# ofsouzap/DistributedMandelbrot

Hardware: AMD Instinct MI355X
Metric: G pixel-iterations/s on 4096^2 tile, max_iter=1000 fp64 (higher is better)
Workload: dtype f64

## Files before the change

distributedmandelbrot_amd/_lib.py:

```python
from __future__ import annotations

import ctypes as C
import importlib.util
import os
import sys

HERE = os.path.dirname(os.path.abspath(__file__))
SO_PATH = os.path.join(HERE, "libmbk_hip.so")

MBK_OK, MBK_ERR_INVALID, MBK_ERR_NO_DEVICE, MBK_ERR_HIP, MBK_ERR_NOMEM, MBK_ERR_NET = range(6)
MBK_WANT_COUNTS = 0x1
MBK_WANT_BYTES = 0x2
MBK_KERNEL_DEFAULT = 0x000
MBK_KERNEL_SIMPLE = 0x100
MBK_KERNEL_ASM = 0x200
MBK_KERNEL_REFILL = 0x300
MBK_KERNEL_GROUP = 0x400
MBK_KERNEL_SCAN = 0x500
KERNELS = {"default": MBK_KERNEL_DEFAULT, "simple": MBK_KERNEL_SIMPLE, "asm": MBK_KERNEL_ASM,
           "refill": MBK_KERNEL_REFILL, "group": MBK_KERNEL_GROUP, "scan": MBK_KERNEL_SCAN}
OPTIONS = {name: i for i, name in enumerate(
    ["order", "waves_per_wg", "group_steps", "exact_steps", "probe_steps", "scan_waves", "scan_xcd_map", "scan_col_period", "heavy_share",
     "rf_livemin", "rf_patience", "rf_batch", "rf_waves", "cycle_detect", "probe_mid", "prepass_overlap", "exact_long", "scan_inline", "wave_limit", "units_min_light", "xcd_balance", "m_late", "h_settled", "classify_wg", "scan_strip", "cycle_window", "spill_first", "spill_lanes", "spill_min_mrd", "spill_min_blocks", "spill_cyc_shift"])}
MBK_PRECISION_F32 = 0x1000
MBK_LAZY_UNIFORM = 0x2000
MBK_DEEP_BLA = 0x8000
MBK_DEEP_XBLA = 0x10000
PRECISIONS = {"f64": 0, "f32": MBK_PRECISION_F32}
MBK_SLOTS = 4
MBK_WORKER_DEPTH = 3
MBK_INFO_SCAN_WG_PER_CU = 100
MBK_INFO_XCD_SHARE = 110
MBK_INFO_SPILL = 130
MBK_CODEC_RAW = 0x00
MBK_CODEC_RLE = 0x01
MBK_CHUNK_DEFINITION = 4096
MBK_CHUNK_BYTES = 4096 * 4096
MBK_ABI_VERSION = 5
MBK_RENDER_BYTES = 0
MBK_RENDER_SMOOTH = 1
MBK_RENDER_DISTANCE = 3
MBK_RENDER_DISTANCE_REL = 4
MBK_RENDER_EQUALIZED = 5
RENDER_SOURCES = {"bytes": MBK_RENDER_BYTES, "smooth": MBK_RENDER_SMOOTH, "distance": MBK_RENDER_DISTANCE,
                  "distance_rel": MBK_RENDER_DISTANCE_REL, "equalized": MBK_RENDER_EQUALIZED}
MBK_HISTOGRAM_MAX_MRD = 1 << 20
RENDER_SUPERSAMPLES = (1, 2, 3, 4, 8)
MBK_RENDER_BAND_BYTES = 256 << 20
MBK_STREAM_OK, MBK_STREAM_BAD_CODEC, MBK_STREAM_BAD_SIZE, MBK_STREAM_ZERO_RUN, MBK_STREAM_TOO_LONG, MBK_STREAM_TOO_SHORT = range(6)
STREAM_REASONS = {MBK_STREAM_OK: "MBK_STREAM_OK", MBK_STREAM_BAD_CODEC: "MBK_STREAM_BAD_CODEC", MBK_STREAM_BAD_SIZE: "MBK_STREAM_BAD_SIZE",
                  MBK_STREAM_ZERO_RUN: "MBK_STREAM_ZERO_RUN", MBK_STREAM_TOO_LONG: "MBK_STREAM_TOO_LONG",
                  MBK_STREAM_TOO_SHORT: "MBK_STREAM_TOO_SHORT"}
CHUNK_SCALES = (1, 2, 4, 8, 16, 32, 64)
MBK_DENSITY_MAX_CELLS = 1 << 28
MBK_DENSITY_LINEAR = 0
MBK_DENSITY_SQRT = 1
DENSITY_MODES = {"linear": MBK_DENSITY_LINEAR, "sqrt": MBK_DENSITY_SQRT}
DENSITY_FACTORS = (1, 2, 4, 8)


class mbk_view(C.Structure):
    _fields_ = [("start_r", C.c_double), ("start_i", C.c_double),
                ("range_r", C.c_double), ("range_i", C.c_double),
                ("width", C.c_uint32), ("height", C.c_uint32),
                ("col0", C.c_uint32), ("row0", C.c_uint32),
                ("ncols", C.c_uint32), ("nrows", C.c_uint32)]


class mbk_deep_view(C.Structure):
    _fields_ = [("range_r", C.c_double), ("range_i", C.c_double),
                ("width", C.c_uint32), ("height", C.c_uint32),
                ("col0", C.c_uint32), ("row0", C.c_uint32),
                ("ncols", C.c_uint32), ("nrows", C.c_uint32)]


class mbk_deep_xview(C.Structure):
    _fields_ = [("range_r", C.c_double), ("range_i", C.c_double), ("exp2", C.c_int32),
                ("width", C.c_uint32), ("height", C.c_uint32),
                ("col0", C.c_uint32), ("row0", C.c_uint32),
                ("ncols", C.c_uint32), ("nrows", C.c_uint32)]


class mbk_render_spec(C.Structure):
    _fields_ = [("source", C.c_uint32), ("supersample", C.c_uint32), ("palette", C.c_void_p),
                ("palette_len", C.c_uint32), ("inside", C.c_uint8 * 4),
                ("scale", C.c_double), ("offset", C.c_double), ("max_band_rows", C.c_uint32)]


class mbk_chunk_spec(C.Structure):
    _fields_ = [("palette", C.c_void_p), ("scale", C.c_uint32)]


class mbk_interior_render_spec(C.Structure):
    _fields_ = [("supersample", C.c_uint32), ("palette", C.c_void_p), ("palette_len", C.c_uint32),
                ("unknown", C.c_uint8 * 4), ("outside", C.c_uint8 * 4), ("scale", C.c_double), ("max_band_rows", C.c_uint32)]


class mbk_density_target(C.Structure):
    _fields_ = [("start_r", C.c_double), ("start_i", C.c_double), ("range_r", C.c_double), ("range_i", C.c_double),
                ("width", C.c_uint32), ("height", C.c_uint32)]


class mbk_density_stats(C.Structure):
    _fields_ = [("deposits", C.c_uint64), ("dropped", C.c_uint64)]


class mbk_density_render_spec(C.Structure):
    _fields_ = [("mode", C.c_uint32), ("factor", C.c_uint32), ("palette", C.c_void_p), ("palette_len", C.c_uint32),
                ("scale", C.c_double), ("offset", C.c_double)]


class mbk_stats(C.Structure):
    _fields_ = [("kernel_ms", C.c_float), ("d2h_ms", C.c_float),
                ("pixel_iterations", C.c_uint64), ("never_pixels", C.c_uint64),
                ("all_bytes_zero", C.c_uint32), ("all_bytes_one", C.c_uint32),
                ("rle_runs", C.c_uint64)]


class mbk_device_info(C.Structure):
    _fields_ = [("name", C.c_char * 128), ("arch", C.c_char * 64),
                ("compute_units", C.c_int), ("clock_mhz", C.c_int),
                ("wavefront_size", C.c_int), ("total_mem", C.c_uint64)]


class mbk_worker_report(C.Structure):
    _fields_ = [("leased", C.c_uint64), ("accepted", C.c_uint64), ("rejected", C.c_uint64), ("resets", C.c_uint64),
                ("uniform_tiles", C.c_uint64), ("pixel_iterations", C.c_uint64),
                ("kernel_ms_sum", C.c_double), ("seconds", C.c_double), ("net_retries", C.c_uint64)]


NET_OPTIONS = {name: i for i, name in enumerate(
    ["max_connections", "connect_timeout_ms", "io_timeout_ms", "retries", "backoff_ms", "stop", "peak_connections", "feeder_slots"])}


FEEDER_SUBMIT = C.CFUNCTYPE(C.c_int, C.c_void_p, C.c_int, C.c_uint32, C.c_uint32, C.c_uint32, C.c_uint32, C.c_void_p)
FEEDER_WAIT = C.CFUNCTYPE(C.c_int, C.c_void_p, C.c_int, C.POINTER(mbk_stats))
FEEDER_ALLOC = C.CFUNCTYPE(C.c_void_p, C.c_void_p, C.c_uint64)
FEEDER_RELEASE = C.CFUNCTYPE(None, C.c_void_p, C.c_void_p)
FEEDER_ON_TILE = C.CFUNCTYPE(None, C.c_void_p, C.POINTER(C.c_uint32 * 4), C.POINTER(mbk_stats), C.c_int)


class mbk_feeder_ops(C.Structure):
    _fields_ = [("user", C.c_void_p), ("submit", FEEDER_SUBMIT), ("wait", FEEDER_WAIT), ("alloc", FEEDER_ALLOC),
                ("release", FEEDER_RELEASE), ("on_tile", FEEDER_ON_TILE)]


SIGNATURES = {
    "mbk_abi_version": (C.c_int, []),
    "mbk_device_count": (C.c_int, [C.POINTER(C.c_int)]),
    "mbk_create": (C.c_int, [C.c_int, C.POINTER(C.c_void_p)]),
    "mbk_destroy": (None, [C.c_void_p]),
    "mbk_last_error": (C.c_char_p, [C.c_void_p]),
    "mbk_get_device_info": (C.c_int, [C.c_void_p, C.POINTER(mbk_device_info)]),
    "mbk_device_pci_bus_id": (C.c_int, [C.c_void_p, C.c_char_p, C.c_int]),
    "mbk_host_alloc": (C.c_int, [C.c_void_p, C.c_uint64, C.POINTER(C.c_void_p)]),
    "mbk_host_free": (C.c_int, [C.c_void_p, C.c_void_p]),
    "mbk_datachunk_geometry": (C.c_int, [C.c_uint32, C.c_uint32, C.c_uint32,
                                         C.POINTER(C.c_double), C.POINTER(C.c_double),
                                         C.POINTER(C.c_double)]),
    "mbk_view_outside_circle": (C.c_int, [C.POINTER(mbk_view), C.c_uint32, C.POINTER(C.c_int)]),
    "mbk_view_needs_literal_doubling": (C.c_int, [C.POINTER(mbk_view), C.c_uint32, C.POINTER(C.c_int)]),
    "mbk_view_launch": (C.c_int, [C.c_void_p, C.POINTER(mbk_view), C.c_uint32, C.c_uint32,
                                  C.c_void_p, C.c_void_p, C.c_void_p]),
    "mbk_view_compute": (C.c_int, [C.c_void_p, C.POINTER(mbk_view), C.c_uint32, C.c_uint32,
                                   C.c_void_p, C.c_void_p, C.POINTER(mbk_stats)]),
    "mbk_datachunk": (C.c_int, [C.c_void_p, C.c_uint32, C.c_uint32, C.c_uint32, C.c_uint32,
                                C.c_void_p, C.c_void_p, C.POINTER(mbk_stats)]),
    "mbk_view_launch_smooth": (C.c_int, [C.c_void_p, C.POINTER(mbk_view), C.c_uint32, C.c_uint32,
                                         C.c_void_p, C.c_void_p, C.c_void_p]),
    "mbk_view_compute_smooth": (C.c_int, [C.c_void_p, C.POINTER(mbk_view), C.c_uint32, C.c_uint32,
                                          C.c_void_p, C.c_void_p, C.POINTER(mbk_stats)]),
    "mbk_view_launch_distance": (C.c_int, [C.c_void_p, C.POINTER(mbk_view), C.c_uint32, C.c_uint32,
                                           C.c_void_p, C.c_void_p, C.c_void_p]),
    "mbk_view_compute_distance": (C.c_int, [C.c_void_p, C.POINTER(mbk_view), C.c_uint32, C.c_uint32,
                                            C.c_void_p, C.c_void_p, C.POINTER(mbk_stats)]),
    "mbk_distance_value_host": (C.c_double, [C.c_double, C.c_double, C.c_int32]),
    "mbk_datachunk_submit": (C.c_int, [C.c_void_p, C.c_int, C.c_uint32, C.c_uint32, C.c_uint32, C.c_uint32,
                                       C.c_void_p, C.c_void_p]),
    "mbk_datachunk_submit_ex": (C.c_int, [C.c_void_p, C.c_int, C.c_uint32, C.c_uint32, C.c_uint32, C.c_uint32,
                                          C.c_void_p, C.c_void_p, C.c_uint32]),
    "mbk_view_submit": (C.c_int, [C.c_void_p, C.c_int, C.POINTER(mbk_view), C.c_uint32, C.c_uint32,
                                  C.c_void_p, C.c_void_p]),
    "mbk_wait": (C.c_int, [C.c_void_p, C.c_int, C.POINTER(mbk_stats)]),
    "mbk_serialize_last": (C.c_int, [C.c_void_p, C.c_void_p, C.c_uint64, C.POINTER(C.c_uint64),
                                     C.POINTER(C.c_uint32)]),
    "mbk_set_option": (C.c_int, [C.c_void_p, C.c_int, C.c_uint32]),
# ... 226 lines not shown
```

distributedmandelbrot_amd/csrc/mbk_api.hip:

```cpp
#include "../../include/mbk.h"

#include <hip/hip_runtime.h>

#include <cmath>
#include <cstdio>
#include <cstdlib>
#include <algorithm>
#include <cstring>
#include <new>
#include <string>
#include <vector>

#include "mbk_kernels.h"
#include "mbk_refill.h"
#include "mbk_persist.h"
#include "mbk_scan.h"
#include "mbk_units.h"
#include "mbk_spill.h"
#include "mbk_feeder.h"
#include "mbk_deep_orbit.h"
#include "mbk_deep.h"
#include "mbk_deep_bla.h"
#include "mbk_deep_wide.h"
#include "mbk_deep_wide_bla.h"
#include "mbk_histogram.h"
#include "mbk_render.h"
#include "mbk_chunks.h"
#include "mbk_distance.h"
#include "mbk_interior.h"
#include "mbk_deep_distance.h"
#include "mbk_deep_distance_bla.h"
#include "mbk_deep_wide_distance.h"
#include "mbk_julia.h"
#include "mbk_density.h"

using mbk::Axis;
using mbk::ReduceOut;
using mbk::ReduceSlot;
using mbk::TileArgs;
using mbk::WorkQueues;

static const int kOrderRing = 3;

struct OrderRing {
    uint32_t *d_order[kOrderRing] = {};
    uint32_t *d_ctl = nullptr;
    bool ctl_dirty = true;
    size_t order_cap = 0;
    unsigned order_turn = 0;
    hipStream_t aux = nullptr;
    uint32_t aux_prio = 0;
    int pp_last = -1;
    hipEvent_t ev_cls[kOrderRing] = {};
    hipEvent_t ev_done[kOrderRing] = {};
    bool done_valid[kOrderRing] = {};

    void drop_lists()
    {
        for (int k = 0; k < kOrderRing; ++k) {
            if (d_order[k]) (void)hipFree(d_order[k]);
            d_order[k] = nullptr;
            done_valid[k] = false;
        }
        order_cap = 0;
    }
    void drop_aux()
    {
        if (aux) (void)hipStreamDestroy(aux);
        aux = nullptr;
        for (int k = 0; k < kOrderRing; ++k) {
            if (ev_cls[k]) (void)hipEventDestroy(ev_cls[k]);
            if (ev_done[k]) (void)hipEventDestroy(ev_done[k]);
            ev_cls[k] = ev_done[k] = nullptr;
            done_valid[k] = false;
        }
    }
    void release()
    {
        if (aux) (void)hipStreamSynchronize(aux);
        drop_lists();
        drop_aux();
        if (d_ctl) (void)hipFree(d_ctl);
        *this = OrderRing();
    }
};

struct SpillBuffers {
    void *d_z = nullptr;
    uint32_t *d_meta = nullptr, *d_cnt = nullptr, *d_chunks = nullptr, *d_src = nullptr;
    unsigned long long *d_total = nullptr;
    size_t cap_slots = 0, cap_blocks = 0;

    void release()
    {
        for (void *q : {d_z, (void *)d_meta, (void *)d_cnt, (void *)d_chunks, (void *)d_src, (void *)d_total})
            if (q) (void)hipFree(q);
        *this = SpillBuffers();
    }
};

struct StreamScratch {
    hipStream_t stream = nullptr;
    OrderRing ring;
    WorkQueues *d_queues = nullptr;
    mbk::ScanCursors *d_cursors = nullptr;
    uint32_t *d_entries = nullptr;
    size_t scan_cap_blocks = 0;
    unsigned scan_turn = 0;
    bool cursors_dirty = false;
    uint32_t *h_hint = nullptr;
    SpillBuffers spill;
    ReduceSlot *d_red = nullptr;
    ReduceSlot *h_red = nullptr;
    unsigned long long *h_stamps = nullptr;
    double xcd_f[8] = {0.125, 0.125, 0.125, 0.125, 0.125, 0.125, 0.125, 0.125};
    uint32_t xcd_issued = 0, xcd_consumed = 0;
    struct SharesUsed { uint32_t seq, switches; float f[8]; } xcd_ring[64] = {};
    void *d_render = nullptr;
    size_t render_cap = 0;
    uint32_t *d_palette = nullptr;
    std::vector<uint32_t> palette;
    uint8_t *d_chunk = nullptr;
    size_t chunk_cap_n = 0;
    uint8_t *d_chunk_bytes = nullptr;
    uint32_t *h_chunk_status = nullptr;
    int32_t *d_dist_counts = nullptr;
    size_t dist_cap_px = 0;
    double *d_lut = nullptr;
    size_t lut_cap = 0;
    std::vector<double> lut;
    uint32_t *d_density_bands = nullptr;
    mbk::DensityMax *d_density_max = nullptr;
};
static const size_t kMaxStreamScratch = 64;
static const uint32_t kStampSlots = 16, kShareRing = 64;

struct Slot {
    hipStream_t stream = nullptr;
    hipEvent_t ev_k0 = nullptr, ev_k1 = nullptr, ev_c0 = nullptr, ev_c1 = nullptr;
    int32_t *d_counts = nullptr;
    uint8_t *d_bytes = nullptr;
    size_t cap_px = 0;
    ReduceSlot *d_red = nullptr;
    ReduceSlot *h_red = nullptr;
    bool busy = false;
    bool with_bytes = false;
    uint8_t *lazy_h_bytes = nullptr;
    size_t lazy_px = 0;
    bool immediate = false;
    mbk_stats imm = {};
};

struct mbk_ctx {
    int device = -1;
    Slot s[MBK_SLOTS];
    std::vector<StreamScratch> scratch;
    size_t last_px = 0;
    double *d_smooth = nullptr;
    size_t smooth_cap_px = 0;
    uint32_t *d_rgba = nullptr;
    size_t rgba_cap_px = 0;
    unsigned long long *d_hist = nullptr;
    size_t hist_cap = 0;
    uint32_t *d_density = nullptr;
    size_t density_cap = 0;
    unsigned long long *d_density_stat = nullptr;
    uint8_t *d_rle = nullptr;
    size_t rle_cap_px = 0;
    uint32_t opt[MBK_OPT_COUNT_];
    hipStream_t last_tile_stream = nullptr;
    uint32_t stream_switches = 0;
    int scan_occ[2][2] = {{0, 0}, {0, 0}};
    int scan_occ_inline[2] = {0, 0};
    uint32_t wave_limit_lds[8] = {0, 0, 0, 0, 0, 0, 0, 0};
    uint32_t spill_launches = 0;
    hipStream_t last_spill_stream = nullptr;
    struct ProbeKey { Axis re, im; uint32_t col0, row0, ncols, nrows; } probe_key = {};
    double probe_share = 0.0;
    bool probe_valid = false;
    struct DeepCopy {
        uint64_t id;
        double4 *d;
        mbk::WideEntry *d_wide;
        bool has_bla;
        uint64_t dcmax_bits;
        double *d_rc;
        double4 *d_ab;
        uint32_t levels;
        uint32_t off[mbk::kBlaMaxLevels];
        bool has_xbla;
        uint64_t xdcmax_bits;
        int32_t xdcmax_exp;
        int32_t *d_xke;
        mbk::WideBlaEntry *d_xab;
        uint32_t xlevels;
        uint32_t xoff[mbk::kBlaMaxLevels];
    };
    std::vector<DeepCopy> deep;
    hipDeviceProp_t prop;
    std::string err;
};

struct mbk_deep_orbit {
    mbk::DeepOrbit o;
};

static thread_local std::string g_err;

static int fail(mbk_ctx *ctx, int code, const std::string &msg)
{
    if (ctx) ctx->err = msg;
    g_err = msg;
    return code;
}

#define MBK_HIP(ctx, call)                                                                  \
    do {                                                                                    \
        hipError_t e_ = (call);                                                             \
        if (e_ != hipSuccess) {                                                             \
            return fail((ctx), MBK_ERR_HIP,                                                 \
                        std::string(#call) + ": " + hipGetErrorString(e_));                 \
        }                                                                                   \
    } while (0)


static Axis make_axis(double start, double range, uint32_t n)
{
    Axis a;
    std::memset(&a, 0, sizeof(a));
    a.start = start;
    a.n = n;
    volatile double stop = start + range;
    if (n <= 1) {
        a.last = start;
        a.div = 1.0;
        return a;
    }
    volatile double delta = stop - start;
    volatile double div = (double)(n - 1);
    volatile double step = delta / div;
    a.last = stop;
    a.delta = delta;
    a.div = div;
    a.step = step;
    a.step_is_zero = (step == 0.0) ? 1u : 0u;
    return a;
}

static double axis_value_host(const Axis &a, uint32_t k)
{
    if (k + 1u == a.n) return a.last;
    volatile double y;
    if (a.step_is_zero) {
        volatile double q = (double)k / a.div;
        y = q * a.delta;
    } else {
        y = (double)k * a.step;
    }
    volatile double v = y + a.start;
    return v;
}

static bool axis_end_is_regular(const Axis &a)
{
    if (a.n <= 1 || a.step_is_zero) return false;
    volatile double y = (double)(a.n - 1u) * a.step;
    volatile double v = y + a.start;
    return v == a.last;
}

static const double kMaxCoord = 0x1p500;
static const double kSafeImagMin = 0x1p-900;

static uint32_t coprime_multiplier(uint32_t n)
{
    if (n < 4) return 1u;
    uint64_t m = (uint64_t)((double)n * 0.6180339887498949);
    if (m < 1) m = 1;
    for (;; ++m) {
        uint64_t a = m, b = n;
        while (b) {
            const uint64_t t = a % b;
            a = b;
            b = t;
        }
        if (a == 1) return (uint32_t)(m % n);
    }
}

static bool axis_has_tiny_nonzero(const Axis &a, uint32_t k0, uint32_t cnt, bool f32)
{
    const double thr = f32 ? 0x1p-100 : kSafeImagMin;
    auto value = [&](uint32_t k) { const double y = axis_value_host(a, k); return f32 ? (double)(float)y : y; };
    auto tiny = [&](double y) { return y != 0.0 && std::fabs(y) < thr; };
    if (cnt == 0) return false;
    uint32_t end = k0 + cnt;
    if (a.n >= 1u && end == a.n) {
        if (tiny(value(a.n - 1u))) return true;
        if (--end == k0) return false;
    }
    const double first = value(k0), last = value(end - 1u);
    if (tiny(first) || tiny(last)) return true;
    if ((first > 0.0 && last > 0.0) || (first < 0.0 && last < 0.0) || first == last) return false;
    const double s = last > first ? 1.0 : -1.0;
    auto lower = [&](bool strict) {
        uint32_t lo = k0, hi = end;
        while (lo < hi) {
            const uint32_t mid = lo + (hi - lo) / 2u;
            const double y = s * value(mid);
            if (strict ? y > 0.0 : y >= 0.0) hi = mid;
            else lo = mid + 1u;
        }
        return lo;
    };
    const uint32_t ge = lower(false), gt = lower(true);
    if (ge > k0 && tiny(value(ge - 1u))) return true;
    if (gt < end && tiny(value(gt))) return true;
    return false;
}

static int validate_view(mbk_ctx *ctx, const mbk_view *v, bool *safe_doubling, bool f32 = false)
{
    if (!v) return fail(ctx, MBK_ERR_INVALID, "view is NULL");
    if (v->width == 0 || v->height == 0) return fail(ctx, MBK_ERR_INVALID, "empty view");
    if (v->ncols == 0 || v->nrows == 0) return fail(ctx, MBK_ERR_INVALID, "empty window");
    if ((uint64_t)v->col0 + v->ncols > v->width || (uint64_t)v->row0 + v->nrows > v->height)
        return fail(ctx, MBK_ERR_INVALID, "window exceeds the view");
    if ((uint64_t)v->ncols * v->nrows > (1ull << 31))
        return fail(ctx, MBK_ERR_INVALID, "window larger than 2^31 pixels");
    const double vals[6] = {v->start_r, v->start_i, v->range_r, v->range_i,
                            v->start_r + v->range_r, v->start_i + v->range_i};
    const double max_coord = f32 ? 0x1p60 : kMaxCoord;
    for (double x : vals)
        if (!std::isfinite(x) || std::fabs(x) > max_coord)
            return fail(ctx, MBK_ERR_INVALID, f32 ? "view coordinates must be finite and |x| <= 2^60 (fp32)"
                                                  : "view coordinates must be finite and |x| <= 2^500");
    *safe_doubling = axis_has_tiny_nonzero(make_axis(v->start_i, v->range_i, v->height), v->row0, v->nrows, f32);
    return MBK_OK;
}

static void free_deep_copy(mbk_ctx::DeepCopy &c)
{
    if (c.d) (void)hipFree(c.d);
    if (c.d_rc) (void)hipFree(c.d_rc);
    if (c.d_ab) (void)hipFree(c.d_ab);
    if (c.d_wide) (void)hipFree(c.d_wide);
    if (c.d_xke) (void)hipFree(c.d_xke);
    if (c.d_xab) (void)hipFree(c.d_xab);
    c = mbk_ctx::DeepCopy();
}

static void free_scratch(StreamScratch &sc)
{
    sc.ring.release();
    sc.spill.release();
    if (sc.d_queues) (void)hipFree(sc.d_queues);
    if (sc.d_cursors) (void)hipFree(sc.d_cursors);
    if (sc.d_entries) (void)hipFree(sc.d_entries);
    if (sc.h_hint) (void)hipHostFree(sc.h_hint);
    if (sc.h_stamps) (void)hipHostFree(sc.h_stamps);
    if (sc.d_red) (void)hipFree(sc.d_red);
    if (sc.h_red) (void)hipHostFree(sc.h_red);
    if (sc.d_render) (void)hipFree(sc.d_render);
    if (sc.d_palette) (void)hipFree(sc.d_palette);
    if (sc.d_chunk) (void)hipFree(sc.d_chunk);
    if (sc.d_chunk_bytes) (void)hipFree(sc.d_chunk_bytes);
    if (sc.h_chunk_status) (void)hipHostFree(sc.h_chunk_status);
    if (sc.d_dist_counts) (void)hipFree(sc.d_dist_counts);
    if (sc.d_lut) (void)hipFree(sc.d_lut);
    if (sc.d_density_bands) (void)hipFree(sc.d_density_bands);
    if (sc.d_density_max) (void)hipFree(sc.d_density_max);
    sc = StreamScratch();
}

static int get_scratch(mbk_ctx *ctx, hipStream_t stream, StreamScratch **out)
{
    for (StreamScratch &sc : ctx->scratch)
        if (sc.stream == stream) {
            *out = &sc;
            return MBK_OK;
        }
    if (ctx->scratch.size() >= kMaxStreamScratch) {
        MBK_HIP(ctx, hipDeviceSynchronize());
        for (StreamScratch &sc : ctx->scratch) free_scratch(sc);
        ctx->scratch.clear();
    }
    ctx->scratch.emplace_back();
    StreamScratch &sc = ctx->scratch.back();
    sc.stream = stream;
    *out = &sc;
    MBK_HIP(ctx, hipHostMalloc((void **)&sc.h_hint, 2 * sizeof(uint32_t), hipHostMallocDefault));
    sc.h_hint[0] = sc.h_hint[1] = 0xffffffffu;
    return MBK_OK;
}

static void set_window_facts(TileArgs &a, bool f32);
static void shares_from_fractions(const double *f, uint32_t *cum);
static double window_heavy_share(const TileArgs &a);
static double window_heavy_share(mbk_ctx *ctx, const TileArgs &a);

static void xcd_shares_update(const mbk_ctx *ctx, StreamScratch &sc)
{
    const unsigned long long kMask = 0xffffffffffffull;
    uint32_t first = sc.xcd_issued >= kStampSlots ? sc.xcd_issued - kStampSlots + 1u : 1u;
    first = std::max(first, sc.xcd_consumed + 1u);
    for (uint32_t c = first; c <= sc.xcd_issued; ++c) {
        const volatile unsigned long long *st = sc.h_stamps + (size_t)(c % kStampSlots) * mbk::kStampWords;
        const StreamScratch::SharesUsed &used = sc.xcd_ring[c % kShareRing];
        if (used.seq != c) continue;
        const StreamScratch::SharesUsed &before = sc.xcd_ring[(c - 1u) % kShareRing], &after = sc.xcd_ring[(c + 1u) % kShareRing];
        const bool alone = c > 1u && before.seq == c - 1u && before.switches == used.switches &&
                           (c == sc.xcd_issued ? ctx->stream_switches == used.switches : after.seq == c + 1u && after.switches == used.switches);
        unsigned long long v[mbk::kStampWords];
        bool whole = true;
        for (uint32_t i = 0; i < mbk::kStampWords; ++i) {
            v[i] = st[i];
            whole = whole && (v[i] >> 48) == (c & 0xffffu);
        }
        if (!whole) continue;
        unsigned long long start = v[0] & kMask;
        for (uint32_t x = 1; x < 8u; ++x)
            if ((((v[x] & kMask) - start) & kMask) >> 47) start = v[x] & kMask;
        double T[8], tmin = 1e300, tmax = 0.0, speed[8], sum = 0.0;
        for (uint32_t x = 0; x < 8u; ++x) {
            unsigned long long last = 0;
            for (uint32_t t = 0; t < mbk::kStampTail; ++t)
                last = std::max(last, ((v[8u + x * mbk::kStampTail + t] & kMask) - start) & kMask);
            T[x] = (double)last;
            tmin = std::min(tmin, T[x]);
            tmax = std::max(tmax, T[x]);
        }
        sc.xcd_consumed = c;
        if (!alone || tmin < 1000.0 || tmax > 1.25 * tmin) continue;
        for (uint32_t x = 0; x < 8u; ++x) {
            speed[x] = (double)used.f[x] / T[x];
            sum += speed[x];
        }
        double fs = 0.0;
        for (uint32_t x = 0; x < 8u; ++x) {
            const double f = 0.7 * sc.xcd_f[x] + 0.3 * speed[x] / sum;
            sc.xcd_f[x] = std::min(0.14, std::max(0.11, f));
            fs += sc.xcd_f[x];
        }
        for (uint32_t x = 0; x < 8u; ++x) sc.xcd_f[x] /= fs;
    }
}

struct FuseStats { ReduceSlot *slots; bool counts_unwanted; bool fused; };

static uint32_t quant_table4(int32_t mrd, bool want_bytes)
{
    uint32_t qtab = 0u;
    if (want_bytes && mrd > 0)
        for (uint32_t c = 1; c <= 4u; ++c)
            qtab |= (uint32_t)(((uint64_t)c * 256u + (uint32_t)mrd - 1u) / (uint32_t)mrd & 0xffu) << (8u * (c - 1u));
    return qtab;
}

struct BlockLaunchPlan {
    uint32_t wpw, by;
    dim3 grid, block;
    uint32_t order_mode, probe_steps;
    bool cyc, units, ordered;
    double unit_share;
};

static BlockLaunchPlan block_launch_plan(mbk_ctx *ctx, TileArgs &a, uint32_t kernel, bool safe, bool f32)
{
    BlockLaunchPlan p;
    p.wpw = ctx->opt[MBK_OPT_WAVES_PER_WG];
    a.blocks_x = (a.ncols + 8u * p.wpw - 1u) / (8u * p.wpw);
    p.by = (a.nrows + 7u) / 8u;
    set_window_facts(a, f32);
    p.cyc = ctx->opt[MBK_OPT_CYCLE_DETECT] != 0u;
    p.grid = dim3(a.blocks_x * p.by);
    p.block = dim3(64u * p.wpw);
    p.order_mode = ctx->opt[MBK_OPT_ORDER];
    p.probe_steps = ctx->opt[MBK_OPT_PROBE_STEPS];
    a.perm_mul = p.order_mode == 1 ? coprime_multiplier(p.grid.x) : 1u;
    a.order = nullptr;
    p.units = p.order_mode == 3 && p.wpw == 1u && kernel == MBK_KERNEL_GROUP && !safe && a.smooth == nullptr &&
              (a.counts || a.bytes) && !(a.bytes && a.quant_wide) && a.blocks_x % 8u == 0u && a.blocks_x <= 2048u &&
              a.fast_bx_end > 0u && a.fast_by_end > 0u && (f32 || ctx->opt[MBK_OPT_GROUP_STEPS] == 16u) &&
              p.grid.x >= 16384u && (uint32_t)a.mrd > 2u * p.probe_steps && p.by <= 0xffffu;
    p.unit_share = 0.0;
    if (p.units) {
        p.unit_share = window_heavy_share(ctx, a);
        p.units = (1.0 - p.unit_share) * 65536.0 >= (double)ctx->opt[MBK_OPT_UNITS_MIN_LIGHT];
    }
    p.ordered = p.order_mode >= 2 && p.grid.x >= 16384u && (uint32_t)a.mrd > 2u * p.probe_steps && a.blocks_x <= 0xffffu && p.by <= 0xffffu;
    return p;
}

struct OrderList {
    StreamScratch *sc = nullptr;
    unsigned k = 0;
    uint32_t *list = nullptr;
    hipStream_t pre = nullptr;
    bool overlap = false;
    bool whole = false;
    ~OrderList() { if (sc && !whole) sc->ring.ctl_dirty = true; }
};

static int acquire_order_list(mbk_ctx *ctx, hipStream_t stream, uint32_t nblocks, OrderList *out)
{
    StreamScratch *sc = nullptr;
    int rc = get_scratch(ctx, stream, &sc);
    if (rc != MBK_OK) return rc;
    OrderRing &ring = sc->ring;
    const uint32_t pp_mode = ctx->opt[MBK_OPT_PREPASS_OVERLAP];
    const bool overlap = pp_mode != 0u;
    const uint32_t want_prio = pp_mode == 2u ? 2u : 1u;
    if (ring.pp_last != (int)pp_mode) {
        if (ring.pp_last >= 0) {
            MBK_HIP(ctx, hipStreamSynchronize(stream));
            if (ring.aux) MBK_HIP(ctx, hipStreamSynchronize(ring.aux));
        }
        for (int k = 0; k < kOrderRing; ++k) ring.done_valid[k] = false;
        ring.pp_last = (int)pp_mode;
    }
    if (overlap && ring.aux && ring.aux_prio != want_prio) {
        MBK_HIP(ctx, hipStreamSynchronize(stream));
        MBK_HIP(ctx, hipStreamSynchronize(ring.aux));
        ring.drop_aux();
    }
    if (overlap && !ring.aux) {
        if (want_prio == 2u) {
            int least = 0, greatest = 0;
            MBK_HIP(ctx, hipDeviceGetStreamPriorityRange(&least, &greatest));
            MBK_HIP(ctx, hipStreamCreateWithPriority(&ring.aux, hipStreamNonBlocking, greatest));
        } else {
            MBK_HIP(ctx, hipStreamCreateWithFlags(&ring.aux, hipStreamNonBlocking));
        }
        ring.aux_prio = want_prio;
        for (int k = 0; k < kOrderRing; ++k) {
            MBK_HIP(ctx, hipEventCreateWithFlags(&ring.ev_cls[k], hipEventDisableTiming));
            MBK_HIP(ctx, hipEventCreateWithFlags(&ring.ev_done[k], hipEventDisableTiming));
        }
    }
    if (nblocks > ring.order_cap) {
        MBK_HIP(ctx, hipStreamSynchronize(stream));
        if (ring.aux) MBK_HIP(ctx, hipStreamSynchronize(ring.aux));
        ring.drop_lists();
        for (int k = 0; k < kOrderRing; ++k)
            MBK_HIP(ctx, hipMalloc((void **)&ring.d_order[k], mbk::units_list_words(nblocks) * sizeof(uint32_t)));
        ring.order_cap = nblocks;
    }
    const unsigned k = ring.order_turn++ % (unsigned)kOrderRing;
    if (overlap && ring.done_valid[k]) MBK_HIP(ctx, hipStreamWaitEvent(ring.aux, ring.ev_done[k], 0));
    out->k = k;
    out->list = ring.d_order[k];
    out->pre = overlap ? ring.aux : stream;
    out->overlap = overlap;
    out->sc = sc;
    return MBK_OK;
}

static int enqueue_units_prepass(mbk_ctx *ctx, TileArgs &a, const BlockLaunchPlan &p, const OrderList &ol, hipStream_t stream)
{
    StreamScratch *sc = ol.sc;
    OrderRing &ring = sc->ring;
    const uint32_t hs = p.cyc ? ctx->opt[MBK_OPT_H_SETTLED] : 0u;
    const double settle_thr = hs ? std::pow(10.0, -(double)hs) : 0.0;
    if (!ring.d_ctl) {
        MBK_HIP(ctx, hipMalloc((void **)&ring.d_ctl, (size_t)kOrderRing * 8u * sizeof(uint32_t)));
        ring.ctl_dirty = true;
    }
    if (ring.ctl_dirty) {
        if (ring.aux) MBK_HIP(ctx, hipStreamSynchronize(ring.aux));
        MBK_HIP(ctx, hipStreamSynchronize(stream));
        MBK_HIP(ctx, hipMemsetAsync(ring.d_ctl, 0, (size_t)kOrderRing * 8u * sizeof(uint32_t), ol.pre));
        ring.ctl_dirty = false;
    }
    uint32_t *ctl = ring.d_ctl + 8u * ol.k;
    const uint32_t balance = ctx->opt[MBK_OPT_XCD_BALANCE] == 1u && (p.cyc || ctx->prop.multiProcessorCount != 256)
                                 ? 0u : ctx->opt[MBK_OPT_XCD_BALANCE];
    static const double kUneven[8] = {0.110, 0.140, 0.125, 0.120, 0.130, 0.125, 0.115, 0.135};
    if (balance == 1u && !sc->h_stamps) {
        MBK_HIP(ctx, hipHostMalloc((void **)&sc->h_stamps, (size_t)kStampSlots * mbk::kStampWords * sizeof(unsigned long long),
                                   hipHostMallocDefault));
        std::memset(sc->h_stamps, 0xff, (size_t)kStampSlots * mbk::kStampWords * sizeof(unsigned long long));
    }
    if (balance == 1u) xcd_shares_update(ctx, *sc);
    mbk::XcdShares w;
    double f[8];
    const uint32_t seq = ++sc->xcd_issued;
    StreamScratch::SharesUsed &used = sc->xcd_ring[seq % kShareRing];
    used.seq = seq;
    used.switches = ctx->stream_switches;
    for (uint32_t x = 0; x < 8u; ++x) {
        f[x] = balance == 1u ? sc->xcd_f[x] : (balance == 2u ? kUneven[x] : 0.125);
        used.f[x] = (float)f[x];
    }
    shares_from_fractions(f, w.cum);
    a.plan = ol.list + ((2u * (size_t)p.grid.x + 5u + 15u) & ~(size_t)15u);
    a.stamps = balance == 1u ? sc->h_stamps + (size_t)(seq % kStampSlots) * mbk::kStampWords : nullptr;
    a.stamp_tag = seq & 0xffffu;
    const uint32_t cwg = ctx->opt[MBK_OPT_CLASSIFY_WG];
    hipLaunchKernelGGL(mbk::classify_units_kernel, dim3((p.grid.x + cwg - 1u) / cwg), dim3(cwg), 0, ol.pre, a, p.grid.x,
                       (int32_t)p.probe_steps, ol.list, ctl, (int32_t)ctx->opt[MBK_OPT_M_LATE], settle_thr, ctl + 3, (uint32_t *)a.plan, w,
                       a.stamps ? 1u : 0u);
    return MBK_OK;
}

static int enqueue_classify_prepass(mbk_ctx *ctx, const TileArgs &a, const BlockLaunchPlan &p, const OrderList &ol, bool *mid_first)
{
    const uint32_t nblocks = p.grid.x;
    uint32_t *cursors = ol.list + nblocks;
    MBK_HIP(ctx, hipMemsetAsync(cursors, 0, 3 * sizeof(uint32_t), ol.pre));
    *mid_first = p.order_mode == 3 && ctx->opt[MBK_OPT_PROBE_MID] > p.probe_steps && ctx->opt[MBK_OPT_M_LATE] >= 2u &&
                 ctx->opt[MBK_OPT_M_LATE] <= p.probe_steps;
    hipLaunchKernelGGL(mbk::classify_blocks_kernel, dim3((nblocks + 1023u) / 1024u), dim3(1024), 0, ol.pre, a,
                       nblocks, 8u * p.wpw, (int32_t)p.probe_steps, (int32_t)(*mid_first ? ctx->opt[MBK_OPT_M_LATE] : ctx->opt[MBK_OPT_PROBE_MID]),
                       ol.list, cursors);
    return MBK_OK;
}

static bool spill_wanted(const mbk_ctx *ctx, const TileArgs &a, const BlockLaunchPlan &p, uint32_t kernel, bool safe, bool f32)
{
    const uint32_t spill_first = ctx->opt[MBK_OPT_SPILL_FIRST], spill_lanes = ctx->opt[MBK_OPT_SPILL_LANES];
    return !p.units && a.order != nullptr && p.order_mode >= 2u && kernel == MBK_KERNEL_GROUP && !safe && a.smooth == nullptr && p.wpw == 1u &&
           (a.counts || a.bytes) && spill_first != 0u && (f32 || ctx->opt[MBK_OPT_GROUP_STEPS] == 16u) &&
           (uint32_t)a.mrd >= ctx->opt[MBK_OPT_SPILL_MIN_MRD] && (uint32_t)a.mrd < (1u << 26) &&
           ((uint64_t)p.grid.x >> ctx->opt[MBK_OPT_SPILL_MIN_BLOCKS]) != 0ull &&
           (uint64_t)a.mrd > (uint64_t)ctx->opt[MBK_OPT_EXACT_STEPS] + spill_first + 66u &&
           (uint64_t)p.grid.x * spill_lanes < (1ull << 32) && a.fast_bx_end > 0u && a.fast_by_end > 0u;
}

static int acquire_spill(mbk_ctx *ctx, StreamScratch *sc, hipStream_t stream, TileArgs &a, uint32_t nblocks, SpillBuffers **out)
{
    SpillBuffers &sp = sc->spill;
    const uint32_t spill_lanes = ctx->opt[MBK_OPT_SPILL_LANES];
    const size_t slots = (size_t)nblocks * spill_lanes, nchunks = (nblocks + mbk::kSpillChunk - 1u) / mbk::kSpillChunk;
    *out = nullptr;
    if (slots > sp.cap_slots || nblocks > sp.cap_blocks) {
        MBK_HIP(ctx, hipStreamSynchronize(stream));
        sp.release();
        const bool got = hipMalloc(&sp.d_z, slots * 16u) == hipSuccess &&
                         hipMalloc((void **)&sp.d_meta, slots * sizeof(uint32_t)) == hipSuccess &&
                         hipMalloc((void **)&sp.d_src, slots * sizeof(uint32_t)) == hipSuccess &&
                         hipMalloc((void **)&sp.d_cnt, (size_t)nblocks * sizeof(uint32_t)) == hipSuccess &&
                         hipMalloc((void **)&sp.d_chunks, (nchunks * mbk::kSpillLevels + 1u) * sizeof(uint32_t)) == hipSuccess &&
                         hipMalloc((void **)&sp.d_total, sizeof(unsigned long long)) == hipSuccess;
        if (got) {
            sp.cap_slots = slots;
            sp.cap_blocks = nblocks;
        } else {
            (void)hipGetLastError();
            sp.release();
        }
    }
    if (sp.cap_slots >= slots && sp.cap_blocks >= nblocks && sp.d_z) {
        a.spill_first = ctx->opt[MBK_OPT_SPILL_FIRST];
        a.spill_lanes = spill_lanes;
        a.spill_win_shift = ctx->opt[MBK_OPT_SPILL_CYC_SHIFT];
        a.spill_z = sp.d_z;
        a.spill_meta = sp.d_meta;
        a.spill_cnt = sp.d_cnt;
        MBK_HIP(ctx, hipMemsetAsync(sp.d_cnt, 0, (size_t)nblocks * sizeof(uint32_t), stream));
        *out = &sp;
    }
    return MBK_OK;
}

typedef void (*UnitsKernel)(TileArgs, uint32_t);
typedef void (*BlockKernel)(TileArgs);
typedef void (*SpillKernel)(TileArgs, const uint32_t *, const unsigned long long *, uint32_t);

static UnitsKernel pick_units_kernel(bool f32, bool cyc, bool stats, bool counts, bool bytes)
{
    static const UnitsKernel forms[4][4] = {
        {mbk::tile_units_kernel<float, 8, true, false, true, true>, mbk::tile_units_kernel<float, 8, true, true, true>,
         mbk::tile_units_kernel<float, 8, true, false, true>, mbk::tile_units_kernel<float, 8, true, true, false>},
        {mbk::tile_units_kernel<float, 8, false, false, true, true>, mbk::tile_units_kernel<float, 8, false, true, true>,
         mbk::tile_units_kernel<float, 8, false, false, true>, mbk::tile_units_kernel<float, 8, false, true, false>},
        {mbk::tile_units_kernel<double, 16, true, false, true, true>, mbk::tile_units_kernel<double, 16, true, true, true>,
         mbk::tile_units_kernel<double, 16, true, false, true>, mbk::tile_units_kernel<double, 16, true, true, false>},
        {mbk::tile_units_kernel<double, 16, false, false, true, true>, mbk::tile_units_kernel<double, 16, false, true, true>,
         mbk::tile_units_kernel<double, 16, false, false, true>, mbk::tile_units_kernel<double, 16, false, true, false>},
    };
    return forms[(f32 ? 0 : 2) + (cyc ? 0 : 1)][stats ? 0 : (counts && bytes) ? 1 : bytes ? 2 : 3];
}

static BlockKernel pick_block_kernel(uint32_t kernel, bool safe, bool f32, bool cyc, uint32_t group_steps, bool spill)
{
    if (spill && f32 && cyc) return mbk::tile_asm_kernel<float, true, 8, true, true>;
    if (spill && f32) return mbk::tile_asm_kernel<float, true, 8, false, true>;
    if (spill && cyc) return mbk::tile_asm_kernel<double, true, 16, true, true>;
    if (spill) return mbk::tile_asm_kernel<double, true, 16, false, true>;
    if (f32 && safe) return mbk::tile_asm_kernel<float, false, 0>;
    if (f32 && kernel == MBK_KERNEL_ASM) return mbk::tile_asm_kernel<float, true, 0>;
    if (f32 && cyc) return mbk::tile_asm_kernel<float, true, 8, true>;
    if (f32) return mbk::tile_asm_kernel<float, true, 8>;
    if (safe) return mbk::tile_asm_kernel<double, false, 0>;
    if (kernel == MBK_KERNEL_ASM) return mbk::tile_asm_kernel<double, true, 0>;
    if (group_steps == 32 && !cyc) return mbk::tile_asm_kernel<double, true, 32>;
    if (group_steps >= 16 && cyc) return mbk::tile_asm_kernel<double, true, 16, true>;
    if (group_steps >= 16) return mbk::tile_asm_kernel<double, true, 16>;
    if (group_steps == 8 && cyc) return mbk::tile_asm_kernel<double, true, 8, true>;
    if (group_steps == 8) return mbk::tile_asm_kernel<double, true, 8>;
    return mbk::tile_asm_kernel<double, true, 4>;
}

static SpillKernel pick_spill_kernels(bool f32, bool cyc)
{
    if (f32 && cyc) return mbk::tile_spill_kernel<float, true>;
    if (f32) return mbk::tile_spill_kernel<float, false>;
    if (cyc) return mbk::tile_spill_kernel<double, true>;
    return mbk::tile_spill_kernel<double, false>;
}

static void enqueue_units_tile(mbk_ctx *ctx, TileArgs &a, const BlockLaunchPlan &p, bool f32, uint32_t lds, hipStream_t stream, FuseStats *fuse)
{
    const double est = (double)p.grid.x * (p.unit_share + (1.0 - p.unit_share) / 8.0);
    const uint32_t cus = (uint32_t)ctx->prop.multiProcessorCount;
    uint32_t g = (uint32_t)std::min<double>((double)p.grid.x, est * 1.15 + 2048.0);
    g = (std::max(std::max(g, std::min(p.grid.x, cus * 64u)), 16384u) + 7u) & ~7u;
    a.unit_stride = g;
    const bool stats = fuse != nullptr && fuse->slots != nullptr && fuse->counts_unwanted && a.bytes != nullptr;
    if (stats) {
        a.stats = fuse->slots;
        a.counts = nullptr;
        fuse->fused = true;
    }
    hipLaunchKernelGGL(pick_units_kernel(f32, p.cyc, stats, a.counts != nullptr, a.bytes != nullptr), dim3(g), dim3(64), lds, stream, a,
                       quant_table4(a.mrd, a.bytes != nullptr));
}

static int enqueue_spill_second_pass(mbk_ctx *ctx, const TileArgs &a, const SpillBuffers &sp, uint32_t nblocks, bool f32, bool cyc, hipStream_t stream)
{
    const uint32_t nchunks = (nblocks + mbk::kSpillChunk - 1u) / mbk::kSpillChunk;
    hipLaunchKernelGGL(mbk::spill_count_kernel, dim3(nchunks), dim3(mbk::kSpillChunk), 0, stream, sp.d_cnt, nblocks, nchunks, sp.d_chunks);
    hipLaunchKernelGGL(mbk::rle_scan_kernel, dim3(1), dim3(1024), 0, stream, sp.d_chunks, nchunks * mbk::kSpillLevels, sp.d_total);
    hipLaunchKernelGGL(mbk::spill_expand_kernel, dim3(nchunks), dim3(mbk::kSpillChunk), 0, stream, sp.d_cnt, nblocks, nchunks,
                       sp.d_chunks, a.spill_lanes, sp.d_src);
    const uint32_t nwg = (uint32_t)std::min<uint64_t>(((uint64_t)nblocks * a.spill_lanes + 63u) / 64u, 16384u);
    const uint32_t lds2 = 0u;
    hipLaunchKernelGGL(pick_spill_kernels(f32, cyc), dim3(nwg), dim3(64), lds2, stream, a, sp.d_src, sp.d_total, nwg);
    MBK_HIP(ctx, hipGetLastError());
    ++ctx->spill_launches;
    ctx->last_spill_stream = stream;
    return MBK_OK;
}

static int launch_blocks(mbk_ctx *ctx, TileArgs a, uint32_t kernel, bool safe, bool f32, hipStream_t stream, FuseStats *fuse = nullptr)
{
    const BlockLaunchPlan p = block_launch_plan(ctx, a, kernel, safe, f32);
    OrderList ol;
    if (p.ordered) {
        int rc = acquire_order_list(ctx, stream, p.grid.x, &ol);
        if (rc != MBK_OK) return rc;
        OrderRing &ring = ol.sc->ring;
        bool mid_first = false;
        rc = p.units ? enqueue_units_prepass(ctx, a, p, ol, stream) : enqueue_classify_prepass(ctx, a, p, ol, &mid_first);
        if (rc != MBK_OK) return rc;
        if (ol.overlap) {
            MBK_HIP(ctx, hipEventRecord(ring.ev_cls[ol.k], ring.aux));
            MBK_HIP(ctx, hipStreamWaitEvent(stream, ring.ev_cls[ol.k], 0));
        }
        a.order = ol.list;
        a.ngrid = p.grid.x;
        a.order_mid = mid_first ? 2u : (ctx->opt[MBK_OPT_PROBE_MID] <= p.probe_steps ? 1u : 0u);
    }
    SpillBuffers *spill = nullptr;
    if (spill_wanted(ctx, a, p, kernel, safe, f32)) {
        const int rc = acquire_spill(ctx, ol.sc, stream, a, p.grid.x, &spill);
        if (rc != MBK_OK) return rc;
    }
    const uint32_t lds = p.wpw == 1u ? ctx->wave_limit_lds[ctx->opt[MBK_OPT_WAVE_LIMIT] & 7u] : 0u;
    if (p.units && a.order)
        enqueue_units_tile(ctx, a, p, f32, lds, stream, fuse);
    else
        hipLaunchKernelGGL(pick_block_kernel(kernel, safe, f32, p.cyc, ctx->opt[MBK_OPT_GROUP_STEPS], spill != nullptr), p.grid, p.block, lds, stream, a);
    const hipError_t e = hipGetLastError();
    if (e != hipSuccess) return fail(ctx, MBK_ERR_HIP, std::string("tile launch: ") + hipGetErrorString(e));
    if (ol.overlap) {
        MBK_HIP(ctx, hipEventRecord(ol.sc->ring.ev_done[ol.k], stream));
        ol.sc->ring.done_valid[ol.k] = true;
    }
    if (spill) {
        const int rc = enqueue_spill_second_pass(ctx, a, *spill, p.grid.x, f32, p.cyc, stream);
        if (rc != MBK_OK) return rc;
    }
    ol.whole = true;
    return MBK_OK;
}

static bool window_may_touch_ring(const TileArgs &a, double margin = 1e-6)
{
    const double x0 = axis_value_host(a.re, a.col0), x1 = axis_value_host(a.re, a.col0 + a.ncols - 1u);
    const double y0 = axis_value_host(a.im, a.row0), y1 = axis_value_host(a.im, a.row0 + a.nrows - 1u);
    const double xlo = std::fmin(x0, x1), xhi = std::fmax(x0, x1), ylo = std::fmin(y0, y1), yhi = std::fmax(y0, y1);
    const double dx = (xlo <= 0.0 && 0.0 <= xhi) ? 0.0 : std::fmin(std::fabs(xlo), std::fabs(xhi));
    const double dy = (ylo <= 0.0 && 0.0 <= yhi) ? 0.0 : std::fmin(std::fabs(ylo), std::fabs(yhi));
    const double fx = std::fmax(std::fabs(xlo), std::fabs(xhi)), fy = std::fmax(std::fabs(ylo), std::fabs(yhi));
    const double rmin2 = dx * dx + dy * dy, rmax2 = fx * fx + fy * fy;
    return !(rmax2 < 4.0 - margin || rmin2 > 4.0 + margin);
}

static void set_window_facts(TileArgs &a, bool f32)
{
    a.ring_possible = window_may_touch_ring(a, f32 ? 2e-3 : 1e-6) ? 1u : 0u;
    a.fast_bx_end = a.fast_by_end = 0u;
    if (a.re.step_is_zero || a.im.step_is_zero) return;
    const uint64_t re_n = (uint64_t)a.re.n - (axis_end_is_regular(a.re) ? 0u : 1u), im_n = (uint64_t)a.im.n - (axis_end_is_regular(a.im) ? 0u : 1u);
    const uint64_t cols_ok = std::min<uint64_t>(a.ncols, re_n - std::min<uint64_t>(a.col0, re_n));
    const uint64_t rows_ok = std::min<uint64_t>(a.nrows, im_n - std::min<uint64_t>(a.row0, im_n));
    a.fast_bx_end = (uint32_t)(cols_ok / 8u);
    a.fast_by_end = (uint32_t)(rows_ok / 8u);
}

static int launch_refill(mbk_ctx *ctx, const TileArgs &a, bool safe, hipStream_t stream)
{
    const bool eligible = !safe && a.mrd >= 2 && a.counts != nullptr && !a.re.step_is_zero &&
                          !a.im.step_is_zero && !window_may_touch_ring(a, 1e-6);
    const uint32_t cols_ok = a.re.n > 0 ? std::min<uint64_t>(a.ncols, (uint64_t)(a.re.n - 1u) - std::min<uint64_t>(a.col0, a.re.n - 1u)) : 0u;
    const uint32_t rows_ok = a.im.n > 0 ? std::min<uint64_t>(a.nrows, (uint64_t)(a.im.n - 1u) - std::min<uint64_t>(a.row0, a.im.n - 1u)) : 0u;
    const uint32_t icols = eligible ? (cols_ok / 8u) * 8u : 0u, irows = eligible ? (rows_ok / 8u) * 8u : 0u;
    if (icols == 0 || irows == 0) return launch_blocks(ctx, a, MBK_KERNEL_GROUP, safe, false, stream);

    mbk::PersistArgs q;
    std::memset(&q, 0, sizeof(q));
    q.re_start = a.re.start;
    q.re_step = a.re.step;
    q.im_start = a.im.start;
    q.im_step = a.im.step;
    q.col0 = a.col0;
    q.row0 = a.row0;
    q.pitch = a.out_pitch;
    q.bxn = icols / 8u;
    q.nblocks = q.bxn * (irows / 8u);
    q.total = (uint32_t)a.mrd - 1u;
    q.livemin = ctx->opt[MBK_OPT_RF_LIVEMIN];
    q.patience = ctx->opt[MBK_OPT_RF_PATIENCE];
    q.batch = ctx->opt[MBK_OPT_RF_BATCH];
    q.counts = a.counts;
    StreamScratch *sc = nullptr;
    int rcs = get_scratch(ctx, stream, &sc);
    if (rcs != MBK_OK) return rcs;
    if (!sc->d_queues) MBK_HIP(ctx, hipMalloc((void **)&sc->d_queues, sizeof(WorkQueues)));
    WorkQueues *wq = sc->d_queues;
    hipLaunchKernelGGL(mbk::init_queues_kernel, dim3(1), dim3(64), 0, stream, wq, q.nblocks);
    uint32_t waves = (uint32_t)ctx->prop.multiProcessorCount * 4u * ctx->opt[MBK_OPT_RF_WAVES];
    if (waves > q.nblocks) waves = q.nblocks;
    hipLaunchKernelGGL(mbk::tile_persist_kernel, dim3((waves + 3u) / 4u), dim3(256), 0, stream, q, wq);
    MBK_HIP(ctx, hipGetLastError());
    TileArgs e = a;
    e.bytes = nullptr;
    if (icols < a.ncols) {
        e.col0 = a.col0 + icols;
        e.ncols = a.ncols - icols;
        e.out_col0 = a.out_col0 + icols;
        int rc = launch_blocks(ctx, e, MBK_KERNEL_GROUP, safe, false, stream);
        if (rc != MBK_OK) return rc;
    }
    if (irows < a.nrows) {
        e = a;
        e.bytes = nullptr;
        e.ncols = icols;
        e.row0 = a.row0 + irows;
        e.nrows = a.nrows - irows;
        e.out_row0 = a.out_row0 + irows;
        int rc = launch_blocks(ctx, e, MBK_KERNEL_GROUP, safe, false, stream);
        if (rc != MBK_OK) return rc;
    }
    if (a.bytes) {
        const uint64_t npx = (uint64_t)a.ncols * a.nrows;
        hipLaunchKernelGGL(mbk::quantise_kernel, dim3(2048), dim3(256), 0, stream, a.counts, a.bytes, npx, a.mrd,
                           a.quant_wide, a.quant_rcp);
        MBK_HIP(ctx, hipGetLastError());
    }
    return MBK_OK;
}

static double window_heavy_share(const TileArgs &a)
{
    const uint32_t k = 16;
    uint32_t inside = 0;
    for (uint32_t j = 0; j < k; ++j) {
        const double ci = axis_value_host(a.im, a.row0 + (uint32_t)(((uint64_t)(2u * j + 1u) * a.nrows) / (2u * k)));
        for (uint32_t i = 0; i < k; ++i) {
            const double cr = axis_value_host(a.re, a.col0 + (uint32_t)(((uint64_t)(2u * i + 1u) * a.ncols) / (2u * k)));
            double zr = cr, zi = ci;
            bool in = true;
            for (int n = 0; n < 4 && in; ++n) {
                const double t = zr * zr - zi * zi + cr;
                zi = 2.0 * zr * zi + ci;
                zr = t;
                in = zr * zr + zi * zi < 4.0;
            }
            inside += in ? 1u : 0u;
        }
    }
    return (double)inside / (double)(k * k);
}

static double window_heavy_share(mbk_ctx *ctx, const TileArgs &a)
{
    mbk_ctx::ProbeKey k;
    std::memset(&k, 0, sizeof(k));
    k.re = a.re;
// ... 473 lines not shown
        case Target::kDeep: set_geometry(p.deep, p.g); break;
        case Target::kJulia:
        case Target::kPlain: set_geometry(p.view, p.g); break;
    }
    return p;
}

struct BandPlan {
    uint32_t ncols, nrows, tile_cols, band_rows;
    size_t cap_px() const { return (size_t)tile_cols * band_rows; }
};

static BandPlan band_plan(uint32_t ncols, uint32_t nrows, uint64_t bytes_per_px, uint32_t max_rows = 0u)
{
    const uint64_t budget = MBK_RENDER_BAND_BYTES - 1024u;
    BandPlan p = {ncols, nrows, ncols, 1u};
    if ((uint64_t)ncols * bytes_per_px <= budget)
        p.band_rows = (uint32_t)std::min<uint64_t>(nrows, budget / ((uint64_t)ncols * bytes_per_px));
    else
        p.tile_cols = (uint32_t)(budget / bytes_per_px);
    if (max_rows) p.band_rows = std::min(p.band_rows, max_rows);
    return p;
}

template <typename Piece>
static int for_each_band(mbk_ctx *ctx, const BandPlan &p, const int32_t *d_counts, uint64_t samples_per_px, uint32_t mrd,
                         hipStream_t stream, Slot *stat, Piece piece)
{
    for (uint32_t r = 0; r < p.nrows; r += p.band_rows) {
        const uint32_t nr = std::min(p.band_rows, p.nrows - r);
        for (uint32_t c = 0; c < p.ncols; c += p.tile_cols) {
            const uint32_t nc = std::min(p.tile_cols, p.ncols - c);
            const bool is_last = r + nr == p.nrows && c + nc == p.ncols;
            int rc = piece(r, c, nr, nc, is_last);
            if (rc != MBK_OK) return rc;
            if (stat) {
                if (is_last) MBK_HIP(ctx, hipEventRecord(stat->ev_k1, stream));
                rc = launch_reduce(ctx, stat->d_red, stat->h_red, d_counts, nullptr, (uint64_t)nc * nr * samples_per_px, mrd, stream, false);
                if (rc != MBK_OK) return rc;
            }
        }
    }
    return MBK_OK;
}


static double deep_step(double range, uint32_t n)
{
    if (n <= 1u) return 0.0;
    volatile double s = range / (double)(n - 1u);
    return s;
}

static double deep_dc(uint32_t k, uint32_t n, double range)
{
    volatile double dc = ((double)k - (double)(n - 1u) * 0.5) * deep_step(range, n);
    return dc;
}

template <typename V>
static bool deep_ranges_within(const V *v, double lo)
{
    for (double r : {v->range_r, v->range_i})
        if (!std::isfinite(r) || !(r >= lo) || !(r <= 4.0)) return false;
    return true;
}

template <typename V, typename FlagRules, typename RangeRules>
static int validate_deep_view(mbk_ctx *ctx, const mbk_deep_orbit *orbit, const V *v, uint32_t mrd, uint32_t flags, FlagRules flag_rules,
                              RangeRules range_rules)
{
    if (!orbit) return fail(ctx, MBK_ERR_INVALID, "orbit is NULL");
    if (!v) return fail(ctx, MBK_ERR_INVALID, "view is NULL");
    int rc = flag_rules();
    if (rc != MBK_OK) return rc;
    if (v->width == 0 || v->height == 0) return fail(ctx, MBK_ERR_INVALID, "empty view");
    if (v->ncols == 0 || v->nrows == 0) return fail(ctx, MBK_ERR_INVALID, "empty window");
    if ((uint64_t)v->col0 + v->ncols > v->width || (uint64_t)v->row0 + v->nrows > v->height)
        return fail(ctx, MBK_ERR_INVALID, "window exceeds the view");
    if ((uint64_t)v->ncols * v->nrows > (1ull << 31)) return fail(ctx, MBK_ERR_INVALID, "window larger than 2^31 pixels");
    rc = range_rules();
    if (rc != MBK_OK) return rc;
    if (mrd > orbit->o.mrd) return fail(ctx, MBK_ERR_INVALID, "mrd exceeds the mrd the reference orbit was computed for");
    if ((flags & MBK_WANT_BYTES) && mrd == 0) return fail(ctx, MBK_ERR_INVALID, "mrd == 0 has no quantised form (division by zero)");
    return MBK_OK;
}

template <typename Args, typename V>
static void fill_deep_window(Args &a, const V *v, uint32_t mrd)
{
    a.half_r = (double)(v->width - 1u) * 0.5;
    a.half_i = (double)(v->height - 1u) * 0.5;
    a.step_r = deep_step(v->range_r, v->width);
    a.step_i = deep_step(v->range_i, v->height);
    a.col0 = v->col0;
    a.row0 = v->row0;
    a.ncols = v->ncols;
    a.nrows = v->nrows;
    a.blocks_x = (v->ncols + 7u) / 8u;
    a.mrd = (int32_t)mrd;
}

template <typename Args>
static void fill_outputs(Args &a, uint32_t mrd, int32_t *d_counts, uint8_t *d_bytes, double *d_smooth)
{
    a.quant_wide = (mrd >= (1u << 23)) ? 1u : 0u;
    a.quant_rcp = mrd ? 1.0 / (double)mrd : 0.0;
    a.counts = d_counts;
    a.bytes = d_bytes;
    a.smooth = d_smooth;
}

template <typename Args>
static dim3 block_grid(const Args &a) { return dim3(a.blocks_x * ((a.nrows + 7u) / 8u)); }


extern "C" {

int mbk_abi_version(void) { return MBK_ABI_VERSION; }

int mbk_device_count(int *count)
{
    if (!count) return fail(nullptr, MBK_ERR_INVALID, "count is NULL");
    int n = 0;
    hipError_t e = hipGetDeviceCount(&n);
    if (e != hipSuccess) {
        *count = 0;
        return fail(nullptr, MBK_ERR_NO_DEVICE, std::string("hipGetDeviceCount: ") + hipGetErrorString(e));
    }
    *count = n;
    return MBK_OK;
}

int mbk_create(int device, mbk_ctx **out)
{
    if (!out) return fail(nullptr, MBK_ERR_INVALID, "out is NULL");
    *out = nullptr;
    int n = 0;
    hipError_t e = hipGetDeviceCount(&n);
    if (e != hipSuccess || n <= 0)
        return fail(nullptr, MBK_ERR_NO_DEVICE,
                    std::string("no HIP device visible (") + hipGetErrorString(e) +
                        "); libmbk_hip has no CPU fallback");
    if (device < 0 || device >= n) return fail(nullptr, MBK_ERR_NO_DEVICE, "device index out of range");
    mbk_ctx *ctx = new (std::nothrow) mbk_ctx();
    if (!ctx) return fail(nullptr, MBK_ERR_NOMEM, "out of host memory");
    ctx->device = device;
    static const uint32_t kDefaults[MBK_OPT_COUNT_] = {
         3u,  1u,  16u,  8u,  32u,
         8u,  1u,  4u,  655u,
         48u,  256u,  1u,  8u,  1u,
         65537u,  1u,  0u,  1u,  0u,
         32768u,  0u,  8u,  6u,  1024u,
         1u,  32u,  256u,  16u,  2048u,  19u,  5u};
    std::memcpy(ctx->opt, kDefaults, sizeof(kDefaults));
#define MBK_CREATE_HIP(call)                                                        \
    do {                                                                            \
        hipError_t e2_ = (call);                                                    \
        if (e2_ != hipSuccess) {                                                    \
            fail(nullptr, MBK_ERR_HIP, std::string(#call) + ": " + hipGetErrorString(e2_)); \
            mbk_destroy(ctx);                                                       \
            return MBK_ERR_HIP;                                                     \
        }                                                                           \
    } while (0)
    MBK_CREATE_HIP(hipSetDevice(device));
    MBK_CREATE_HIP(hipGetDeviceProperties(&ctx->prop, device));
    if (std::strncmp(ctx->prop.gcnArchName, "gfx950", 6) != 0) {
        fail(nullptr, MBK_ERR_NO_DEVICE,
             std::string("device is ") + ctx->prop.gcnArchName + ", this library is built for gfx950 only");
        mbk_destroy(ctx);
        return MBK_ERR_NO_DEVICE;
    }
    for (Slot &sl : ctx->s) {
        MBK_CREATE_HIP(hipStreamCreateWithFlags(&sl.stream, hipStreamNonBlocking));
        MBK_CREATE_HIP(hipEventCreate(&sl.ev_k0));
        MBK_CREATE_HIP(hipEventCreate(&sl.ev_k1));
        MBK_CREATE_HIP(hipEventCreate(&sl.ev_c0));
        MBK_CREATE_HIP(hipEventCreate(&sl.ev_c1));
        MBK_CREATE_HIP(hipMalloc((void **)&sl.d_red, sizeof(ReduceSlot) * mbk::kReduceSlots));
        MBK_CREATE_HIP(hipHostMalloc((void **)&sl.h_red, sizeof(ReduceSlot) * mbk::kReduceSlots, hipHostMallocDefault));
    }
    {
        const void *fns[2][2] = {{(const void *)mbk::tile_light_kernel<double, true, true>, (const void *)mbk::tile_todo_kernel<double>},
                                 {(const void *)mbk::tile_light_kernel<float, true, true>, (const void *)mbk::tile_todo_kernel<float>}};
        for (int f = 0; f < 2; ++f)
            for (int k = 0; k < 2; ++k) {
                int n = 0;
                MBK_CREATE_HIP(hipOccupancyMaxActiveBlocksPerMultiprocessor(&n, fns[f][k], 64, 0));
                ctx->scan_occ[f][k] = n > 0 ? n : 1;
            }
        const void *fi[2][6] = {{(const void *)mbk::tile_light_kernel<double, true, true, 2>, (const void *)mbk::tile_light_kernel<double, true, true, 1>,
                                 (const void *)mbk::tile_light_kernel<double, true, true, 2, true>, (const void *)mbk::tile_light_kernel<double, false, true, 2, true>,
                                 (const void *)mbk::tile_light_kernel<double, true, false, 2, true>, (const void *)mbk::tile_light_kernel<double, true, false, 1>},
                                {(const void *)mbk::tile_light_kernel<float, true, true, 2>, (const void *)mbk::tile_light_kernel<float, true, true, 1>,
                                 (const void *)mbk::tile_light_kernel<float, true, true, 2, true>, (const void *)mbk::tile_light_kernel<float, false, true, 2, true>,
                                 (const void *)mbk::tile_light_kernel<float, true, false, 2, true>, (const void *)mbk::tile_light_kernel<float, true, false, 1>}};
        for (int f = 0; f < 2; ++f) {
            int least = 0;
            for (int k = 0; k < 6; ++k) {
                int n = 0;
                MBK_CREATE_HIP(hipOccupancyMaxActiveBlocksPerMultiprocessor(&n, fi[f][k], 64, 0));
                n = n > 0 ? n : 1;
                least = (k == 0 || n < least) ? n : least;
            }
            ctx->scan_occ_inline[f] = least;
        }
    }
    {
        const void *fn = (const void *)mbk::tile_asm_kernel<double, true, 16, false>;
        for (int k = 1; k <= 7; ++k) {
            uint32_t lo = 0, hi = 65536;
            int n = 0;
            MBK_CREATE_HIP(hipOccupancyMaxActiveBlocksPerMultiprocessor(&n, fn, 64, hi));
            if (n > 4 * k) {
                ctx->wave_limit_lds[k] = hi;
                continue;
            }
            while (hi - lo > 64) {
                const uint32_t mid = (lo + hi) / 2;
                MBK_CREATE_HIP(hipOccupancyMaxActiveBlocksPerMultiprocessor(&n, fn, 64, mid));
                if (n > 4 * k) lo = mid;
                else hi = mid;
            }
            ctx->wave_limit_lds[k] = hi;
        }
    }
#undef MBK_CREATE_HIP
    *out = ctx;
    return MBK_OK;
}

void mbk_destroy(mbk_ctx *ctx)
{
    if (!ctx) return;
    if (ctx->device >= 0) (void)hipSetDevice(ctx->device);
    for (Slot &sl : ctx->s) {
        if (sl.stream) (void)hipStreamSynchronize(sl.stream);
        if (sl.d_counts) (void)hipFree(sl.d_counts);
        if (sl.d_bytes) (void)hipFree(sl.d_bytes);
        if (sl.d_red) (void)hipFree(sl.d_red);
        if (sl.h_red) (void)hipHostFree(sl.h_red);
        if (sl.ev_k0) (void)hipEventDestroy(sl.ev_k0);
        if (sl.ev_k1) (void)hipEventDestroy(sl.ev_k1);
        if (sl.ev_c0) (void)hipEventDestroy(sl.ev_c0);
        if (sl.ev_c1) (void)hipEventDestroy(sl.ev_c1);
        if (sl.stream) (void)hipStreamDestroy(sl.stream);
    }
    if (!ctx->scratch.empty() || !ctx->deep.empty()) (void)hipDeviceSynchronize();
    for (StreamScratch &sc : ctx->scratch) free_scratch(sc);
    for (mbk_ctx::DeepCopy &c : ctx->deep) free_deep_copy(c);
    if (ctx->d_rle) (void)hipFree(ctx->d_rle);
    if (ctx->d_smooth) (void)hipFree(ctx->d_smooth);
    if (ctx->d_rgba) (void)hipFree(ctx->d_rgba);
    if (ctx->d_hist) (void)hipFree(ctx->d_hist);
    if (ctx->d_density) (void)hipFree(ctx->d_density);
    if (ctx->d_density_stat) (void)hipFree(ctx->d_density_stat);
    delete ctx;
}

const char *mbk_last_error(const mbk_ctx *ctx) { return ctx ? ctx->err.c_str() : g_err.c_str(); }

int mbk_get_device_info(mbk_ctx *ctx, mbk_device_info *info)
{
    if (!ctx || !info) return fail(ctx, MBK_ERR_INVALID, "NULL argument");
    std::memset(info, 0, sizeof(*info));
    std::snprintf(info->name, sizeof(info->name), "%s", ctx->prop.name);
    std::snprintf(info->arch, sizeof(info->arch), "%s", ctx->prop.gcnArchName);
    info->compute_units = ctx->prop.multiProcessorCount;
    info->clock_mhz = ctx->prop.clockRate / 1000;
    info->wavefront_size = ctx->prop.warpSize;
    info->total_mem = ctx->prop.totalGlobalMem;
    return MBK_OK;
}

int mbk_device_pci_bus_id(mbk_ctx *ctx, char *buf, int len)
{
    if (!ctx || !buf || len < 16) return fail(ctx, MBK_ERR_INVALID, "buffer of at least 16 bytes needed");
    MBK_HIP(ctx, hipDeviceGetPCIBusId(buf, len, ctx->device));
    return MBK_OK;
}

int mbk_host_alloc(mbk_ctx *ctx, uint64_t bytes, void **out)
{
    if (!ctx || !out || bytes == 0) return fail(ctx, MBK_ERR_INVALID, "bad argument");
    MBK_HIP(ctx, hipSetDevice(ctx->device));
    MBK_HIP(ctx, hipHostMalloc(out, bytes, hipHostMallocDefault));
    return MBK_OK;
}

int mbk_host_free(mbk_ctx *ctx, void *ptr)
{
    if (!ctx) return fail(ctx, MBK_ERR_INVALID, "ctx is NULL");
    if (!ptr) return MBK_OK;
    MBK_HIP(ctx, hipSetDevice(ctx->device));
    MBK_HIP(ctx, hipHostFree(ptr));
    return MBK_OK;
}

int mbk_datachunk_geometry(uint32_t level, uint32_t index_real, uint32_t index_imag,
                           double *start_r, double *start_i, double *range)
{
    if (!start_r || !start_i || !range) return fail(nullptr, MBK_ERR_INVALID, "NULL output pointer");
    if (level == 0) return fail(nullptr, MBK_ERR_INVALID, "level must be > 0 (DataChunk.cs:99-100)");
    if (index_real >= level || index_imag >= level)
        return fail(nullptr, MBK_ERR_INVALID, "chunk index must be < level (DataChunk.cs:102-106)");
    volatile double chunk_range = (2.0 - (-2.0)) / (double)level;
    volatile double pr = chunk_range * (double)index_real;
// ... 328 lines not shown
static int launch_interior(mbk_ctx *ctx, const mbk_view *v, uint32_t mrd, uint32_t flags, bool safe, int32_t *d_counts,
                           int32_t *d_period, double *d_distance, hipStream_t stream)
{
    const size_t px = (size_t)v->ncols * v->nrows;
    if (!d_counts) {
        StreamScratch *sc = nullptr;
        int rc = get_scratch(ctx, stream, &sc);
        if (rc == MBK_OK) rc = grow(ctx, sc->d_dist_counts, sc->dist_cap_px, px, px * sizeof(int32_t));
        if (rc != MBK_OK) return rc;
        d_counts = sc->d_dist_counts;
    }
    int rc = launch_tile(ctx, v, mrd, (flags & MBK_KERNEL_MASK) | MBK_WANT_COUNTS, d_counts, nullptr, stream);
    if (rc != MBK_OK) return rc;
    mbk::InteriorArgs a;
    std::memset(&a, 0, sizeof(a));
    fill_window(a, v);
    a.blocks_x = (v->ncols + 7u) / 8u;
    a.mrd = (int32_t)mrd;
    a.counts_in = d_counts;
    a.period = d_period;
    a.distance = d_distance;
    const dim3 grid(a.blocks_x * ((v->nrows + 7u) / 8u)), block(64);
    if (safe) hipLaunchKernelGGL(mbk::interior_kernel<false>, grid, block, 0, stream, a);
    else hipLaunchKernelGGL(mbk::interior_kernel<true>, grid, block, 0, stream, a);
    MBK_HIP(ctx, hipGetLastError());
    return MBK_OK;
}

int mbk_view_interior_launch(mbk_ctx *ctx, const mbk_view *view, uint32_t mrd, uint32_t flags, int32_t *d_counts,
                             int32_t *d_period, double *d_distance, void *hip_stream)
{
    if (!ctx || (!d_period && !d_distance)) return fail(ctx, MBK_ERR_INVALID, "NULL argument");
    bool safe = false;
    int rc = interior_check(ctx, view, mrd, flags, &safe);
    if (rc != MBK_OK) return rc;
    MBK_HIP(ctx, hipSetDevice(ctx->device));
    return launch_interior(ctx, view, mrd, flags, safe, d_counts, d_period, d_distance, (hipStream_t)hip_stream);
}

int mbk_view_interior_compute(mbk_ctx *ctx, const mbk_view *view, uint32_t mrd, uint32_t flags, int32_t *h_counts,
                              int32_t *h_period, double *h_distance, mbk_stats *stats)
{
    if (!ctx || !view || (!h_period && !h_distance)) return fail(ctx, MBK_ERR_INVALID, "NULL argument");
    bool safe = false;
    int rc = interior_check(ctx, view, mrd, flags, &safe);
    if (rc != MBK_OK) return rc;
    rc = sync_begin(ctx);
    if (rc != MBK_OK) return rc;
    const size_t px = (size_t)view->ncols * view->nrows;
    return compute_values(ctx, px, mrd, h_counts, h_distance, stats,
                          [&](int32_t *d_counts, double *d_distance, hipStream_t stream) {
                              return launch_interior(ctx, view, mrd, flags, safe, d_counts, h_period ? (int32_t *)(d_distance + px) : nullptr,
                                                     h_distance ? d_distance : nullptr, stream);
                          },
                          true, h_period);
}

int mbk_interior_host(double c_r, double c_i, uint32_t mrd, int32_t *count, int32_t *period, int32_t *cycle_len, double *de)
{
    if (!count) return fail(nullptr, MBK_ERR_INVALID, "count is NULL");
    if (mrd > 0x7fffffffu) return fail(nullptr, MBK_ERR_INVALID, "mrd must fit int32 (calc_mb_value returns int32)");
    double mag = 0.0, d = 0.0;
    int32_t L = 0, p = 0;
    *count = mbk::julia_count<false>(c_r, c_i, c_r, c_i, (int32_t)mrd, &mag);
    mbk::interior_pixel<false>(c_r, c_i, (int32_t)mrd, *count, L, p, d);
    if (period) *period = p;
    if (cycle_len) *cycle_len = L;
    if (de) *de = d;
    return MBK_OK;
}

int mbk_serialize_last(mbk_ctx *ctx, uint8_t *h_out, uint64_t cap, uint64_t *size, uint32_t *codec)
{
    if (!ctx || !h_out || !size || !codec) return fail(ctx, MBK_ERR_INVALID, "NULL argument");
    int rc = sync_begin(ctx);
    if (rc != MBK_OK) return rc;
    const size_t n = ctx->last_px;
    if (n == 0) return fail(ctx, MBK_ERR_INVALID, "no tile with quantised bytes has been computed on this ctx");
    const uint32_t nblocks = (uint32_t)((n + mbk::kRleBlock - 1) / mbk::kRleBlock);
    auto align = [](size_t x) { return (x + 255) & ~(size_t)255; };
    const size_t max_runs = n / 5 + 1;
    const size_t off_cnt = 0, off_tot = align(off_cnt + (size_t)nblocks * 4), off_start = align(off_tot + 8),
                 off_val = align(off_start + max_runs * 4), off_out = align(off_val + max_runs),
                 total_bytes = off_out + 1 + n;
    rc = grow(ctx, ctx->d_rle, ctx->rle_cap_px, n, total_bytes);
    if (rc != MBK_OK) return rc;
    uint32_t *d_cnt = (uint32_t *)(ctx->d_rle + off_cnt);
    unsigned long long *d_tot = (unsigned long long *)(ctx->d_rle + off_tot);
    uint32_t *d_start = (uint32_t *)(ctx->d_rle + off_start);
    uint8_t *d_val = ctx->d_rle + off_val, *d_out = ctx->d_rle + off_out;
    hipStream_t s = ctx->s[0].stream;
    hipLaunchKernelGGL(mbk::rle_count_kernel, dim3(nblocks), dim3(mbk::kRleBlock), 0, s, ctx->s[0].d_bytes, (uint64_t)n, d_cnt);
    hipLaunchKernelGGL(mbk::rle_scan_kernel, dim3(1), dim3(1024), 0, s, d_cnt, nblocks, d_tot);
    MBK_HIP(ctx, hipGetLastError());
    unsigned long long runs = 0;
    MBK_HIP(ctx, hipMemcpyAsync(&runs, d_tot, sizeof(runs), hipMemcpyDeviceToHost, s));
    MBK_HIP(ctx, hipStreamSynchronize(s));
    const uint64_t raw_size = 1 + (uint64_t)n, rle_size = 1 + 5 * (uint64_t)runs;
    const bool use_rle = rle_size < raw_size;
    *codec = use_rle ? MBK_CODEC_RLE : MBK_CODEC_RAW;
    *size = use_rle ? rle_size : raw_size;
    if (cap < *size) return fail(ctx, MBK_ERR_INVALID, "output buffer too small for the serialised chunk");
    if (use_rle) {
        hipLaunchKernelGGL(mbk::rle_scatter_kernel, dim3(nblocks), dim3(mbk::kRleBlock), 0, s, ctx->s[0].d_bytes,
                           (uint64_t)n, d_cnt, d_start, d_val);
        hipLaunchKernelGGL(mbk::rle_emit_kernel, dim3((uint32_t)((runs + 255) / 256)), dim3(256), 0, s, d_start,
                           d_val, (uint64_t)runs, (uint64_t)n, d_out);
        MBK_HIP(ctx, hipGetLastError());
        MBK_HIP(ctx, hipMemcpyAsync(h_out, d_out, rle_size, hipMemcpyDeviceToHost, s));
    } else {
        h_out[0] = MBK_CODEC_RAW;
        MBK_HIP(ctx, hipMemcpyAsync(h_out + 1, ctx->s[0].d_bytes, n, hipMemcpyDeviceToHost, s));
    }
    MBK_HIP(ctx, hipStreamSynchronize(s));
    return MBK_OK;
}

int mbk_set_option(mbk_ctx *ctx, int option, uint32_t value)
{
    if (!ctx) return fail(ctx, MBK_ERR_INVALID, "ctx is NULL");
    bool ok = false;
    switch (option) {
        case MBK_OPT_ORDER: ok = value <= 3u; break;
        case MBK_OPT_WAVES_PER_WG: ok = value == 1u || value == 2u || value == 4u; break;
        case MBK_OPT_GROUP_STEPS: ok = value == 4u || value == 8u || value == 16u || value == 32u; break;
        case MBK_OPT_EXACT_STEPS: ok = value <= 4096u; break;
        case MBK_OPT_PROBE_STEPS: ok = value >= 2u && value <= 65536u; break;
        case MBK_OPT_SCAN_WAVES: ok = value >= 1u && value <= 8u; break;
        case MBK_OPT_SCAN_XCD_MAP: ok = value <= 1u; break;
        case MBK_OPT_SCAN_COL_PERIOD: ok = value <= 65536u; break;
        case MBK_OPT_HEAVY_SHARE: ok = value <= 65536u; break;
        case MBK_OPT_RF_LIVEMIN: ok = value <= 63u; break;
        case MBK_OPT_RF_PATIENCE: ok = value >= 16u && value <= (1u << 20); break;
        case MBK_OPT_RF_BATCH: ok = value >= 1u && value <= 64u; break;
        case MBK_OPT_RF_WAVES: ok = value >= 1u && value <= 8u; break;
        case MBK_OPT_CYCLE_DETECT: ok = value <= 1u; break;
        case MBK_OPT_PROBE_MID: ok = value >= 2u && value <= 65537u; break;
        case MBK_OPT_PREPASS_OVERLAP: ok = value <= 2u; break;
        case MBK_OPT_CLASSIFY_WG: ok = value >= 64u && value <= 1024u && value % 64u == 0u; break;
        case MBK_OPT_SCAN_STRIP: ok = value <= 1u; break;
        case MBK_OPT_CYCLE_WINDOW: ok = value <= 65536u; break;
        case MBK_OPT_EXACT_LONG: ok = value <= 4096u; break;
        case MBK_OPT_SCAN_INLINE: ok = value <= 1u; break;
        case MBK_OPT_WAVE_LIMIT: ok = value <= 7u; break;
        case MBK_OPT_UNITS_MIN_LIGHT: ok = value <= 65536u; break;
        case MBK_OPT_XCD_BALANCE: ok = value <= 2u; break;
        case MBK_OPT_M_LATE: ok = value <= 65536u; break;
        case MBK_OPT_H_SETTLED: ok = value <= 30u; break;
        case MBK_OPT_SPILL_FIRST: ok = value <= 65536u && value % 32u == 0u; break;
        case MBK_OPT_SPILL_LANES: ok = value >= 1u && value <= 32u; break;
        case MBK_OPT_SPILL_MIN_MRD: ok = true; break;
        case MBK_OPT_SPILL_MIN_BLOCKS: ok = value <= 31u; break;
        case MBK_OPT_SPILL_CYC_SHIFT: ok = value <= 31u; break;
        default: return fail(ctx, MBK_ERR_INVALID, "unknown MBK_OPT_* selector");
    }
    if (!ok) return fail(ctx, MBK_ERR_INVALID, "option value out of range");
    ctx->opt[option] = value;
    return MBK_OK;
}

int mbk_get_option(mbk_ctx *ctx, int option, uint32_t *value)
{
    if (!ctx || !value) return fail(ctx, MBK_ERR_INVALID, "NULL argument");
    if (option >= MBK_INFO_SCAN_WG_PER_CU && option < MBK_INFO_SCAN_WG_PER_CU + 4) {
        const int k = option - MBK_INFO_SCAN_WG_PER_CU;
        *value = (uint32_t)ctx->scan_occ[k >> 1][k & 1];
        return MBK_OK;
    }
    if (option >= MBK_INFO_XCD_SHARE && option < MBK_INFO_XCD_SHARE + 10) {
        const StreamScratch *best = nullptr;
        for (const StreamScratch &sc : ctx->scratch)
            if (!best || sc.xcd_consumed > best->xcd_consumed) best = &sc;
        const int k = option - MBK_INFO_XCD_SHARE;
        *value = !best ? 0u : k < 8 ? (uint32_t)std::lround(best->xcd_f[k] * 1048576.0) : k == 8 ? best->xcd_consumed : best->xcd_issued;
        return MBK_OK;
    }
    if (option == MBK_INFO_SPILL || option == MBK_INFO_SPILL + 1) {
        *value = ctx->spill_launches;
        if (option == MBK_INFO_SPILL) {
            *value = 0u;
            for (const StreamScratch &sc : ctx->scratch)
                if (sc.stream == ctx->last_spill_stream && sc.spill.d_total && ctx->spill_launches) {
                    unsigned long long t = 0;
                    MBK_HIP(ctx, hipSetDevice(ctx->device));
                    MBK_HIP(ctx, hipStreamSynchronize(sc.stream));
                    MBK_HIP(ctx, hipMemcpy(&t, sc.spill.d_total, sizeof(t), hipMemcpyDeviceToHost));
                    *value = (uint32_t)std::min<unsigned long long>(t, 0xffffffffull);
                }
        }
        return MBK_OK;
    }
    if (option < 0 || option >= MBK_OPT_COUNT_) return fail(ctx, MBK_ERR_INVALID, "unknown MBK_OPT_* selector");
    *value = ctx->opt[option];
    return MBK_OK;
}

static void shares_from_fractions(const double *f, uint32_t *cum)
{
    double c = 0.0;
    for (uint32_t x = 0; x < 8u; ++x) {
        c += f[x];
        cum[x] = x == 7u ? (1u << 24) : (uint32_t)std::lround(std::min(1.0, std::max(0.0, c)) * (double)(1u << 24));
    }
}

int mbk_units_plan(uint32_t n_h, uint32_t n_v, uint32_t n_m, const double *fractions, uint32_t *plan)
{
    if (!fractions || !plan) return MBK_ERR_INVALID;
    if ((uint64_t)n_h + n_v + n_m > 0x7fffffffull) return MBK_ERR_INVALID;
    uint32_t cum[8];
    shares_from_fractions(fractions, cum);
    mbk::units_plan(n_h, n_v, n_m, cum, 0u, plan, 0u, 0u);
    return MBK_OK;
}

int mbk_units_lookup(const uint32_t *plan, uint32_t id, uint32_t *list, uint32_t *index)
{
    if (!plan || !list || !index) return MBK_ERR_INVALID;
    const uint32_t x = id & 7u;
    bool is_h = false;
    uint32_t i = 0;
    *list = 0u;
    *index = 0u;
    if (id >= plan[2] || !mbk::units_lookup(id, plan[3], plan[4], plan[8u + x], plan[16u + x], plan[24u + x], plan[32u + x], is_h, i))
        return MBK_OK;
    *list = is_h ? 1u : (i < plan[1] ? 2u : 3u);
    *index = is_h ? i : (i < plan[1] ? i : i - plan[1]);
    return MBK_OK;
}

int mbk_quantise_counts(mbk_ctx *ctx, const int32_t *h_counts, uint64_t n, uint32_t mrd, uint8_t *h_bytes)
{
    if (!ctx || !h_counts || !h_bytes) return fail(ctx, MBK_ERR_INVALID, "NULL argument");
    if (mrd == 0 || mrd > 0x7fffffffu) return fail(ctx, MBK_ERR_INVALID, "mrd must be in [1, 2^31)");
    if (n == 0) return MBK_OK;
    if (n > (1ull << 31)) return fail(ctx, MBK_ERR_INVALID, "more than 2^31 counts");
    int rc = sync_begin(ctx);
    if (rc != MBK_OK) return rc;
    Slot &sl = ctx->s[0];
    rc = ensure_buffers(ctx, sl, (size_t)n);
    if (rc != MBK_OK) return rc;
    MBK_HIP(ctx, hipMemcpyAsync(sl.d_counts, h_counts, n * sizeof(int32_t), hipMemcpyHostToDevice, sl.stream));
    hipLaunchKernelGGL(mbk::quantise_kernel, dim3(2048), dim3(256), 0, sl.stream, sl.d_counts, sl.d_bytes, n,
                       (int32_t)mrd, mrd >= (1u << 23) ? 1u : 0u, 1.0 / (double)mrd);
    MBK_HIP(ctx, hipGetLastError());
    MBK_HIP(ctx, hipMemcpyAsync(h_bytes, sl.d_bytes, n, hipMemcpyDeviceToHost, sl.stream));
    MBK_HIP(ctx, hipStreamSynchronize(sl.stream));
    ctx->last_px = 0;
    return MBK_OK;
}

int mbk_reduce_counts(mbk_ctx *ctx, const int32_t *d_counts, uint64_t n, uint32_t mrd,
                      void *hip_stream, mbk_stats *stats)
{
    if (!ctx || !d_counts || !stats) return fail(ctx, MBK_ERR_INVALID, "NULL argument");
    MBK_HIP(ctx, hipSetDevice(ctx->device));
    hipStream_t s = (hipStream_t)hip_stream;
    StreamScratch *sc = nullptr;
    int rc = get_scratch(ctx, s, &sc);
    if (rc != MBK_OK) return rc;
    if (!sc->d_red) {
        MBK_HIP(ctx, hipMalloc((void **)&sc->d_red, sizeof(ReduceSlot) * mbk::kReduceSlots));
        MBK_HIP(ctx, hipHostMalloc((void **)&sc->h_red, sizeof(ReduceSlot) * mbk::kReduceSlots, hipHostMallocDefault));
    }
    rc = launch_reduce(ctx, sc->d_red, sc->h_red, d_counts, nullptr, n, mrd, s);
    if (rc != MBK_OK) return rc;
    MBK_HIP(ctx, hipStreamSynchronize(s));
    std::memset(stats, 0, sizeof(*stats));
    fill_stats_from_reduce(sc->h_red, stats, false);
    return MBK_OK;
}


int mbk_deep_orbit_create(const char *center_r, const char *center_i, uint32_t precision_bits, uint32_t mrd,
                          mbk_deep_orbit **out)
{
    if (!out) return fail(nullptr, MBK_ERR_INVALID, "out is NULL");
    *out = nullptr;
    mbk_deep_orbit *o = new (std::nothrow) mbk_deep_orbit();
    if (!o) return fail(nullptr, MBK_ERR_NOMEM, "out of host memory");
    std::string why;
    bool ok = false;
    try {
        ok = mbk::build_deep_orbit(center_r, center_i, precision_bits, mrd, &o->o, &why);
    } catch (const std::bad_alloc &) {
        delete o;
        return fail(nullptr, MBK_ERR_NOMEM, "out of host memory for the reference orbit");
    }
    if (!ok) {
        delete o;
        return fail(nullptr, MBK_ERR_INVALID, why);
    }
    *out = o;
    return MBK_OK;
}

void mbk_deep_orbit_destroy(mbk_deep_orbit *orbit) { delete orbit; }

int mbk_deep_orbit_info(const mbk_deep_orbit *orbit, uint32_t *length, uint32_t *escaped, uint32_t *precision_bits,
                        uint32_t *mrd)
{
    if (!orbit) return fail(nullptr, MBK_ERR_INVALID, "orbit is NULL");
    if (length) *length = orbit->o.length;
    if (escaped) *escaped = orbit->o.escaped;
    if (precision_bits) *precision_bits = orbit->o.precision_bits;
    if (mrd) *mrd = orbit->o.mrd;
    return MBK_OK;
}

int mbk_deep_orbit_read(const mbk_deep_orbit *orbit, double *zr, double *zi, uint64_t n)
{
    if (!orbit || !zr || !zi) return fail(nullptr, MBK_ERR_INVALID, "NULL argument");
    const uint64_t entries = (uint64_t)orbit->o.length + 1u;
    if (n < entries) return fail(nullptr, MBK_ERR_INVALID, "the output holds fewer than length + 1 entries");
    for (uint64_t k = 0; k < entries; ++k) {
        zr[k] = orbit->o.table[4 * k];
        zi[k] = orbit->o.table[4 * k + 1];
    }
    return MBK_OK;
}

int mbk_deep_orbit_read_wide(const mbk_deep_orbit *orbit, double *xr, double *xi, int32_t *xe, uint64_t n)
{
    if (!orbit || !xr || !xi || !xe) return fail(nullptr, MBK_ERR_INVALID, "NULL argument");
    const uint64_t entries = (uint64_t)orbit->o.length + 1u;
    if (n < entries) return fail(nullptr, MBK_ERR_INVALID, "the output holds fewer than length + 1 entries");
    for (uint64_t k = 0; k < entries; ++k) {
        xr[k] = orbit->o.wide[k].xr;
        xi[k] = orbit->o.wide[k].xi;
        xe[k] = orbit->o.wide[k].xe;
    }
    return MBK_OK;
}

static const size_t kMaxDeepCopies = 8;

static int deep_copy(mbk_ctx *ctx, const mbk_deep_orbit *orbit, mbk_ctx::DeepCopy **out)
{
    for (mbk_ctx::DeepCopy &c : ctx->deep)
        if (c.id == orbit->o.id) {
            *out = &c;
// ... 2287 lines not shown
```

distributedmandelbrot_amd/csrc/mbk_kernels.h:

```cpp
#pragma once

#include <hip/hip_runtime.h>
#include <stdint.h>

namespace mbk {

struct Axis {
    double start;
    double step;
    double last;
    double delta;
    double div;
    uint32_t n;
    uint32_t step_is_zero;
};

struct ReduceSlot;

constexpr uint32_t kSpillLevels = 12;

struct TileArgs {
    Axis re, im;
    uint32_t col0, row0, ncols, nrows;
    uint32_t blocks_x;
// ... 28 lines not shown

__device__ __forceinline__ double axis_value(const Axis &a, uint32_t k)
{
    double y;
    if (a.step_is_zero) {
        double q = (double)k / a.div;
        y = q * a.delta;
    } else {
        y = (double)k * a.step;
    }
    double v = y + a.start;
    return (k + 1u == a.n) ? a.last : v;
}

__device__ __forceinline__ uint8_t quantise(int32_t count, int32_t mrd, uint32_t wide, double rcp)
{
    if (wide) {
        uint64_t x = (uint64_t)(uint32_t)count * 256ull + (uint64_t)(uint32_t)mrd - 1ull;
        return (uint8_t)(x / (uint64_t)(uint32_t)mrd);
    }
    const uint32_t x = (uint32_t)count * 256u + (uint32_t)mrd - 1u;
    return (uint8_t)(uint32_t)__builtin_fma((double)x, rcp, 0x1p-30);
}
__device__ __forceinline__ uint8_t quantise(int32_t count, const TileArgs &p)
{
    return quantise(count, p.mrd, p.quant_wide, p.quant_rcp);
}

__device__ __forceinline__ double smooth_value(int32_t count, double m)
{
    return count > 0 ? (double)count + 1.0 - log2(0.5 * log(m)) : 0.0;
}

template <bool kFmaDouble>
__device__ __forceinline__ int32_t escape_count(double cr, double ci, int32_t mrd)
{
    double zr = cr, zi = ci;
    double a = zr * zr, b = zi * zi;
    int32_t result = 0;
    for (int32_t n = 1; n < mrd; ++n) {
        double t = a - b;
        double zi_new;
        if (kFmaDouble) {
            double p = zr * zi;
            zi_new = __builtin_fma(2.0, p, ci);
        } else {
            double w = 2.0 * zr;
            double u = w * zi;
            zi_new = u + ci;
        }
        zr = t + cr;
        zi = zi_new;
        a = zr * zr;
        b = zi * zi;
        double m = a + b;
        if (m >= 4.0) {
            result = n;
            break;
        }
    }
    return result;
}

template <bool kFmaDouble>
__global__ __launch_bounds__(256) void tile_simple_kernel(TileArgs p)
{
    const uint32_t lane = threadIdx.x & 63u;
    const uint32_t wave = threadIdx.x >> 6;
    const uint32_t by = blockIdx.x / p.blocks_x, bx = blockIdx.x - by * p.blocks_x;
    const uint32_t lc = bx * 32u + wave * 8u + (lane & 7u);
    const uint32_t lr = by * 8u + (lane >> 3);
    if (lc >= p.ncols || lr >= p.nrows) return;
    const double cr = axis_value(p.re, p.col0 + lc);
    const double ci = axis_value(p.im, p.row0 + lr);
    const int32_t count = escape_count<kFmaDouble>(cr, ci, p.mrd);
    const size_t o = (size_t)lr * p.ncols + lc;
    if (p.counts) p.counts[o] = count;
    if (p.bytes) p.bytes[o] = quantise(count, p);
}

#define MBK_T double
#define MBK_F "f64"
#define MBK_CI_FROM_T64 "v_add_f64 %[ci], %[t64], %[start]\n"
#define MBK_CR_FROM_T64 "v_add_f64 %[cr], %[t64], %[start]\n"
#define MBK_CYC_BITS "u64"
#define MBK_CYC_MOV "b64"
#include "mbk_loops.inc"
#undef MBK_T
#undef MBK_F
#undef MBK_CI_FROM_T64
#undef MBK_CR_FROM_T64
#undef MBK_CYC_BITS
#undef MBK_CYC_MOV
#define MBK_T float
#define MBK_F "f32"
#define MBK_CI_FROM_T64 "v_add_f64 %[t64], %[t64], %[start]\nv_cvt_f32_f64 %[ci], %[t64]\n"
#define MBK_CR_FROM_T64 "v_add_f64 %[t64], %[t64], %[start]\nv_cvt_f32_f64 %[cr], %[t64]\n"
#define MBK_CYC_BITS "u32"
#define MBK_CYC_MOV "b32"
#include "mbk_loops.inc"
#undef MBK_T
#undef MBK_F
#undef MBK_CI_FROM_T64
#undef MBK_CR_FROM_T64
#undef MBK_CYC_BITS
#undef MBK_CYC_MOV


template <typename T, bool kFmaDouble, int kGroup, bool kCycle = false>
__device__ __forceinline__ int32_t block_pixel(const TileArgs &p, uint32_t ucol, uint32_t urow, uint32_t lx, uint32_t ly,
                                               bool long_groups, bool interior = false)
{
    const uint32_t lc = ucol + lx, lr = urow + ly;
    T cr, ci;
    bool ring_test = kGroup != 0 && kFmaDouble;
    if (interior) {
        cr = (T)((double)(p.col0 + lc) * p.re.step + p.re.start);
        ci = (T)((double)(p.row0 + lr) * p.im.step + p.im.start);
        ring_test = ring_test && p.ring_possible != 0u;
    } else {
        if (lc >= p.ncols || lr >= p.nrows) return -1;
        cr = (T)axis_value(p.re, p.col0 + lc);
        ci = (T)axis_value(p.im, p.row0 + lr);
    }
    int32_t count;
    T m = 0;
    if (kGroup != 0 && kFmaDouble) {
        bool risky = false;
        if (ring_test) {
            const T c2 = cr * cr + ci * ci;
            const T margin = sizeof(T) == 8 ? (T)1e-9 : (T)1e-3;
            risky = __ballot(__builtin_fabs((double)(c2 - (T)4)) < (double)margin) != 0ull;
        }
        if (risky) {
            count = escape_count_asm<true>(cr, ci, p.mrd, &m);
        } else if (kGroup == 32) {
            count = long_groups ? escape_count_group<32, false>(cr, ci, p.mrd, &m, p.exact_steps_long)
                                : escape_count_group<8, false>(cr, ci, p.mrd, &m, p.exact_steps);
        } else if (kGroup == 16) {
            count = long_groups ? escape_count_group<16, kCycle>(cr, ci, p.mrd, &m, p.exact_steps_long, p.cyc_window)
                                : escape_count_group<8, kCycle>(cr, ci, p.mrd, &m, p.exact_steps, p.cyc_window);
        } else {
            count = escape_count_group<kGroup == 8 ? 8 : 4, kCycle>(cr, ci, p.mrd, &m, p.exact_steps, p.cyc_window);
        }
    } else {
        count = escape_count_asm<kFmaDouble>(cr, ci, p.mrd, &m);
    }
    const size_t ubase = (size_t)(urow + p.out_row0) * p.out_pitch + ucol + p.out_col0;
    const uint32_t loff = ly * p.out_pitch + lx;
    if (p.counts) (p.counts + ubase)[loff] = count;
    if (p.bytes) (p.bytes + ubase)[loff] = quantise(count, p);
    if (p.smooth) (p.smooth + ubase)[loff] = smooth_value(count, (double)m);
    return count;
}

template <typename T> struct SpillPair;
template <> struct SpillPair<double> { using type = double2; };
template <> struct SpillPair<float> { using type = float2; };
constexpr int32_t kSpilled = -2;

template <typename T, int kGroup, bool kCycle>
__device__ __forceinline__ void block_pixel_spill(const TileArgs &p, uint32_t ucol, uint32_t urow, uint32_t lx, uint32_t ly,
                                                  bool long_groups, uint32_t block_index)
{
    const uint32_t lc = ucol + lx, lr = urow + ly;
    const T cr = (T)((double)(p.col0 + lc) * p.re.step + p.re.start);
    const T ci = (T)((double)(p.row0 + lr) * p.im.step + p.im.start);
    bool risky = false;
    if (p.ring_possible != 0u) {
        const T c2 = cr * cr + ci * ci;
        const T margin = sizeof(T) == 8 ? (T)1e-9 : (T)1e-3;
        risky = __ballot(__builtin_fabs((double)(c2 - (T)4)) < (double)margin) != 0ull;
    }
    int32_t count;
    if (risky) {
        count = escape_count_asm<true>(cr, ci, p.mrd);
    } else {
        T zr = cr, zi = ci, a = zr * zr, b = zi * zi, m = 0;
        int32_t cnt = 0;
        const uint32_t total = p.mrd > 1 ? (uint32_t)p.mrd - 1u : 0u;
        const uint32_t ex = (kGroup >= 16 && long_groups) ? p.exact_steps_long : p.exact_steps;
        const uint32_t first = total < ex ? total : ex;
        escape_steps_asm<true>(cr, ci, zr, zi, a, b, m, cnt, 0u, first);
        uint32_t n = first, seg = p.spill_first, level = 0u;
        bool spilled = false;
        T szr = zr, szi = zi;
        uint32_t cyc_tc = 0u, cyc_win = 1u;
        while (n < total) {
            if (__ballot(cnt == 0) == 0ull) break;
            const uint32_t stop = (total - n > seg + 64u) ? n + seg : total;
            if (cnt == 0) {
                if (kCycle) {
                    if (kGroup >= 16 && long_groups) escape_steps_carry<16>(cr, ci, zr, zi, a, b, m, cnt, n, stop, p.cyc_window, szr, szi, cyc_tc, cyc_win);
                    else escape_steps_carry<8>(cr, ci, zr, zi, a, b, m, cnt, n, stop, p.cyc_window, szr, szi, cyc_tc, cyc_win);
                } else {
                    if (kGroup >= 16 && long_groups) escape_steps_tail<16, false, false>(cr, ci, zr, zi, a, b, m, cnt, n, stop);
                    else escape_steps_tail<8, false, false>(cr, ci, zr, zi, a, b, m, cnt, n, stop);
                }
            }
            if (kCycle) {
                cyc_tc = (uint32_t)__builtin_amdgcn_readfirstlane((int)cyc_tc);
                cyc_win = (uint32_t)__builtin_amdgcn_readfirstlane((int)cyc_win);
            }
            n = stop;
            if (n >= total) break;
            const unsigned long long alive = __ballot(cnt == 0);
            const uint32_t k = (uint32_t)__popcll(alive);
            if (k == 0u) break;
            if (k <= p.spill_lanes) {
                if (cnt == 0) {
                    const uint32_t rank = __builtin_amdgcn_mbcnt_hi((uint32_t)(alive >> 32), __builtin_amdgcn_mbcnt_lo((uint32_t)alive, 0u));
                    const size_t slot = (size_t)block_index * p.spill_lanes + rank;
                    typename SpillPair<T>::type z;
                    z.x = zr;
                    z.y = zi;
                    reinterpret_cast<typename SpillPair<T>::type *>(p.spill_z)[slot] = z;
                    p.spill_meta[slot] = (ly * 8u + lx) | (n << 6);
                    if (rank == 0u) p.spill_cnt[block_index] = k | ((level < kSpillLevels - 1u ? level : kSpillLevels - 1u) << 8);
                    spilled = true;
                }
                break;
            }
            seg = n - first;
            ++level;
        }
        escape_fixup(cr, ci, zr, zi, a, b, m, cnt);
        count = spilled ? kSpilled : ((kCycle && cnt == -1) ? 0 : cnt);
    }
    if (count != kSpilled) {
        const size_t ubase = (size_t)(urow + p.out_row0) * p.out_pitch + ucol + p.out_col0;
        const uint32_t loff = ly * p.out_pitch + lx;
        if (p.counts) (p.counts + ubase)[loff] = count;
        if (p.bytes) (p.bytes + ubase)[loff] = quantise(count, p);
    }
}

template <typename T, bool kFmaDouble, int kGroup = 0, bool kCycle = false, bool kSpill = false>
__global__ __launch_bounds__(256) void tile_asm_kernel(TileArgs p)
{
    const uint32_t lane = threadIdx.x & 63u;
    const uint32_t wave = (uint32_t)__builtin_amdgcn_readfirstlane((int)(threadIdx.x >> 6));
    uint32_t bx, by;
    uint32_t n_heavy = 0u, heavy_lo = 0u;
    if (p.order) {
        const uint32_t j = blockIdx.x;
        uint32_t e;
        if (p.order_mid == 2u) {
            n_heavy = p.order[p.ngrid];
            const uint32_t n_mid = p.order[p.ngrid + 2u];
            e = j < n_mid ? p.order[p.ngrid + 3u + j] : (j < n_mid + n_heavy ? p.order[j - n_mid] : p.order[j]);
            heavy_lo = n_mid;
        } else if (p.order_mid) {
            n_heavy = p.order[p.ngrid];
            const uint32_t n_mid = p.order[p.ngrid + 2u];
            e = (j >= n_heavy && j < n_heavy + n_mid) ? p.order[p.ngrid + 3u + (j - n_heavy)] : p.order[j];
        } else {
            e = p.order[j];
            n_heavy = p.order[p.ngrid];
        }
        by = e >> 16;
        bx = e & 0xffffu;
    } else {
        const uint32_t blk = (uint32_t)(((uint64_t)blockIdx.x * p.perm_mul) % gridDim.x);
        by = blk / p.blocks_x;
        bx = blk - by * p.blocks_x;
    }
    const uint32_t wcol = bx * (blockDim.x >> 6) + wave;
    const bool long_groups = kGroup >= 16 && (!p.order || (blockIdx.x >= heavy_lo && blockIdx.x < heavy_lo + n_heavy));
    const bool interior = wcol < p.fast_bx_end && by < p.fast_by_end;
    if (kSpill && kFmaDouble && kGroup >= 8 && interior)
        block_pixel_spill<T, kGroup, kCycle>(p, wcol * 8u, by * 8u, lane & 7u, lane >> 3, long_groups, by * p.blocks_x + wcol);
    else
    block_pixel<T, kFmaDouble, kGroup, kCycle>(p, wcol * 8u, by * 8u, lane & 7u, lane >> 3, long_groups, interior);
}

__global__ __launch_bounds__(1024) void classify_blocks_kernel(TileArgs p, uint32_t nregions,
                                                                uint32_t region_w, int32_t probe_steps, int32_t mid_min,
                                                                uint32_t *order, uint32_t *counters)
{
    __shared__ uint32_t s_cnt[3][16], s_base[3];
    const uint32_t r = blockIdx.x * blockDim.x + threadIdx.x;
    const uint32_t lane = threadIdx.x & 63u, wave = threadIdx.x >> 6;
    const bool valid = r < nregions;
    uint32_t cls = 1u;
    uint32_t packed = 0;
    if (valid) {
        const uint32_t by = r / p.blocks_x, bx = r - by * p.blocks_x;
        packed = (by << 16) | bx;
        uint32_t lc = bx * region_w + region_w / 2u, lr = by * 8u + 4u;
        lc = lc < p.ncols ? lc : p.ncols - 1u;
        lr = lr < p.nrows ? lr : p.nrows - 1u;
        const double cr = axis_value(p.re, p.col0 + lc), ci = axis_value(p.im, p.row0 + lr);
        const int32_t cap = p.mrd < probe_steps ? p.mrd : probe_steps;
        const int32_t cnt = cap > 1 ? escape_count<true>(cr, ci, cap) : 1;
        cls = cnt == 0 ? 0u : (cnt >= mid_min ? 2u : 1u);
    }
    unsigned long long m[3];
#pragma unroll
    for (uint32_t k = 0; k < 3u; ++k) {
        m[k] = __ballot(valid && cls == k);
        if (lane == 0) s_cnt[k][wave] = (uint32_t)__popcll(m[k]);
    }
    __syncthreads();
    if (threadIdx.x < 3u) {
        const uint32_t k = threadIdx.x, nw = (blockDim.x + 63u) >> 6;
        uint32_t t = 0;
// ... 237 lines not shown
```

distributedmandelbrot_amd/csrc/mbk_loops.inc:

```
#ifndef MBK_T
#error "define MBK_T and MBK_F before including mbk_loops.inc"
#endif
#define MBK_STEP_HEAD_FMA                                  \
    "v_add_" MBK_F " %[t], %[a], -%[b]\n"                        \
    "v_mul_" MBK_F " %[p], %[zr], %[zi]\n"                       \
    "v_add_" MBK_F " %[zr], %[t], %[cr]\n"                       \
    "v_fma_" MBK_F " %[zi], %[p], 2.0, %[ci]\n"
#define MBK_STEP_HEAD_SAFE                                 \
    "v_add_" MBK_F " %[t], %[a], -%[b]\n"                        \
    "v_add_" MBK_F " %[p], %[zr], %[zr]\n"                       \
    "v_mul_" MBK_F " %[p], %[p], %[zi]\n"                        \
    "v_add_" MBK_F " %[zr], %[t], %[cr]\n"                       \
    "v_add_" MBK_F " %[zi], %[p], %[ci]\n"
#define MBK_STEP_TAIL(ID)                                  \
    "v_mul_" MBK_F " %[a], %[zr], %[zr]\n"                       \
    "v_mul_" MBK_F " %[b], %[zi], %[zi]\n"                       \
    "v_add_" MBK_F " %[m], %[a], %[b]\n"                         \
    "v_cmp_le_" MBK_F " vcc, 4.0, %[m]\n"                        \
    "s_cbranch_vccnz .Lesc" ID "_%=\n"                     \
    ".Lcont" ID "_%=:\n"
#define MBK_ESCAPE(ID, INC)                                \
    ".Lesc" ID "_%=:\n"                                    \
    "s_add_u32 %[k], %[n], " INC "\n"                      \
    "s_and_saveexec_b64 %[tmp], vcc\n"                     \
// ... 134 lines not shown
    MBK_G_GROUP(MBK_G_B2T, MBK_G_T2A, "%[a]", "%[b]", "2")    \
    "s_add_u32 %[n], %[n], 8\n"                            \
    "s_cmp_lt_u32 %[n], %[limit8]\n"                       \
    "s_cbranch_scc1 .Lgmain_%=\n"                          \
    ".Lgtail_%=:\n"                                        \
    "s_cmp_ge_u32 %[n], %[total]\n"                        \
    "s_cbranch_scc1 .Lgdone_%=\n"                          \
    ".Lgtloop_%=:\n"                                       \
    MBK_STEP_HEAD_FMA MBK_STEP_TAIL("GT")                  \
    "s_add_u32 %[n], %[n], 1\n"                            \
    "s_cmp_lt_u32 %[n], %[total]\n"                        \
    "s_cbranch_scc1 .Lgtloop_%=\n"                         \
    "s_branch .Lgdone_%=\n"                                \
    MBK_G_TRIP_A("1", "0")                                 \
    MBK_G_TRIP_B("2", "4")                                 \
    MBK_ESCAPE("GT", "1")                                  \
    ".Ldone_%=:\n"                                         \
    ".Lgdone_%=:\n"                                        \
    "s_mov_b64 exec, %[save]\n"                            \
    MBK_G_FIXUP("4")                                       \
    "s_mov_b64 exec, %[save]\n"

#define MBK_G_GROUP8(FIRST, LAST, AD, BD, ID)              \
    FIRST MBK_G_T2T MBK_G_T2T MBK_G_T2T MBK_G_T2T MBK_G_T2T MBK_G_T2T LAST \
    "v_add_" MBK_F " %[m], " AD ", " BD "\n"                     \
    "v_cmp_ngt_" MBK_F " vcc, 4.0, %[m]\n"                       \
    "s_cbranch_vccnz .Lgrep" ID "_%=\n"                    \
    ".Lgcont" ID "_%=:\n"
#define MBK_G_LOOP8X(INIT, CYC1, CYC2, OOL, FIX)                             \
    "s_mov_b64 %[save], exec\n"                            \
    "s_mov_b32 %[n], %[n0]\n"                              \
    INIT                                                   \
    "s_cmp_ge_u32 %[n], %[limit8]\n"                          \
    "s_cbranch_scc1 .Lgtail_%=\n"                          \
    ".Lgmain_%=:\n"                                        \
    MBK_G_GROUP8(MBK_G_A2T, MBK_G_T2B, "%[a2]", "%[b2]", "1") \
    CYC1                                                   \
    MBK_G_GROUP8(MBK_G_B2T, MBK_G_T2A, "%[a]", "%[b]", "2")   \
    CYC2                                                   \
    "s_add_u32 %[n], %[n], 16\n"                           \
    "s_cmp_lt_u32 %[n], %[limit8]\n"                       \
    "s_cbranch_scc1 .Lgmain_%=\n"                          \
    ".Lgtail_%=:\n"                                        \
    "s_cmp_ge_u32 %[n], %[total]\n"                        \
    "s_cbranch_scc1 .Lgdone_%=\n"                          \
    ".Lgtloop_%=:\n"                                       \
    MBK_STEP_HEAD_FMA MBK_STEP_TAIL("GT")                  \
    "s_add_u32 %[n], %[n], 1\n"                            \
    "s_cmp_lt_u32 %[n], %[total]\n"                        \
    "s_cbranch_scc1 .Lgtloop_%=\n"                         \
    "s_branch .Lgdone_%=\n"                                \
    MBK_G_TRIP_A("1", "0")                                 \
    MBK_G_TRIP_B("2", "8")                                 \
    MBK_ESCAPE("GT", "1")                                  \
    OOL                                                    \
    ".Ldone_%=:\n"                                         \
    ".Lgdone_%=:\n"                                        \
    "s_mov_b64 exec, %[save]\n"                            \
    FIX                                                    \
    "s_mov_b64 exec, %[save]\n"
#define MBK_G_LOOP8 MBK_G_LOOP8X("", "", "", "", MBK_G_FIXUP("8"))
#define MBK_G_LOOP8_NF MBK_G_LOOP8X("", "", "", "", "")

#define MBK_G_T2T4 MBK_G_T2T MBK_G_T2T MBK_G_T2T MBK_G_T2T
#define MBK_G_GROUP16(FIRST, MID, LAST, AD, BD, ID)        \
    FIRST MBK_G_T2T4 MBK_G_T2T MBK_G_T2T MBK_G_T2T MID MBK_G_T2T4 MBK_G_T2T MBK_G_T2T MBK_G_T2T LAST \
    "v_add_" MBK_F " %[m], " AD ", " BD "\n"                     \
    "v_cmp_ngt_" MBK_F " vcc, 4.0, %[m]\n"                       \
    "s_cbranch_vccnz .Lgrep" ID "_%=\n"                    \
    ".Lgcont" ID "_%=:\n"
#define MBK_G_LOOP16X(INIT, MID1, CYC1, MID2, CYC2, OOL, FIX)                      \
    "s_mov_b64 %[save], exec\n"                            \
    "s_mov_b32 %[n], %[n0]\n"                              \
    INIT                                                   \
    "s_cmp_ge_u32 %[n], %[limit8]\n"                       \
    "s_cbranch_scc1 .Lgtail_%=\n"                          \
    ".Lgmain_%=:\n"                                        \
    MBK_G_GROUP16(MBK_G_A2T, MID1, MBK_G_T2B, "%[a2]", "%[b2]", "1") \
    CYC1                                                   \
    MBK_G_GROUP16(MBK_G_B2T, MID2, MBK_G_T2A, "%[a]", "%[b]", "2")   \
    CYC2                                                   \
    "s_add_u32 %[n], %[n], 32\n"                           \
    "s_cmp_lt_u32 %[n], %[limit8]\n"                       \
    "s_cbranch_scc1 .Lgmain_%=\n"                          \
    ".Lgtail_%=:\n"                                        \
    "s_cmp_ge_u32 %[n], %[total]\n"                        \
    "s_cbranch_scc1 .Lgdone_%=\n"                          \
    ".Lgtloop_%=:\n"                                       \
    MBK_STEP_HEAD_FMA MBK_STEP_TAIL("GT")                  \
    "s_add_u32 %[n], %[n], 1\n"                            \
    "s_cmp_lt_u32 %[n], %[total]\n"                        \
    "s_cbranch_scc1 .Lgtloop_%=\n"                         \
    "s_branch .Lgdone_%=\n"                                \
    MBK_G_TRIP_A("1", "0")                                 \
    MBK_G_TRIP_B("2", "16")                                \
    MBK_ESCAPE("GT", "1")                                  \
    OOL                                                    \
    ".Ldone_%=:\n"                                         \
    ".Lgdone_%=:\n"                                        \
    "s_mov_b64 exec, %[save]\n"                            \
    FIX                                                    \
    "s_mov_b64 exec, %[save]\n"
#define MBK_G_LOOP16 MBK_G_LOOP16X("", "", "", "", "", "", MBK_G_FIXUP("16"))
#define MBK_G_LOOP16_NF MBK_G_LOOP16X("", "", "", "", "", "", "")

#define MBK_G_T2T7 MBK_G_T2T4 MBK_G_T2T MBK_G_T2T MBK_G_T2T
#define MBK_G_GROUP32(FIRST, LAST, AD, BD, ID)             \
    FIRST MBK_G_T2T7 MBK_G_T2T4 MBK_G_T2T4 MBK_G_T2T4 MBK_G_T2T4 MBK_G_T2T7 LAST \
    "v_add_" MBK_F " %[m], " AD ", " BD "\n"                     \
    "v_cmp_ngt_" MBK_F " vcc, 4.0, %[m]\n"                       \
    "s_cbranch_vccnz .Lgrep" ID "_%=\n"                    \
    ".Lgcont" ID "_%=:\n"
#define MBK_G_LOOP32                                       \
    "s_mov_b64 %[save], exec\n"                            \
    "s_mov_b32 %[n], %[n0]\n"                              \
    "s_cmp_ge_u32 %[n], %[limit8]\n"                       \
    "s_cbranch_scc1 .Lgtail_%=\n"                          \
    ".Lgmain_%=:\n"                                        \
    MBK_G_GROUP32(MBK_G_A2T, MBK_G_T2B, "%[a2]", "%[b2]", "1") \
    MBK_G_GROUP32(MBK_G_B2T, MBK_G_T2A, "%[a]", "%[b]", "2")   \
    "s_add_u32 %[n], %[n], 64\n"                           \
    "s_cmp_lt_u32 %[n], %[limit8]\n"                       \
    "s_cbranch_scc1 .Lgmain_%=\n"                          \
    ".Lgtail_%=:\n"                                        \
    "s_cmp_ge_u32 %[n], %[total]\n"                        \
    "s_cbranch_scc1 .Lgdone_%=\n"                          \
    ".Lgtloop_%=:\n"                                       \
    MBK_STEP_HEAD_FMA MBK_STEP_TAIL("GT")                  \
    "s_add_u32 %[n], %[n], 1\n"                            \
    "s_cmp_lt_u32 %[n], %[total]\n"                        \
    "s_cbranch_scc1 .Lgtloop_%=\n"                         \
    "s_branch .Lgdone_%=\n"                                \
    MBK_G_TRIP_A("1", "0")                                 \
    MBK_G_TRIP_B("2", "32")                                \
    MBK_ESCAPE("GT", "1")                                  \
    ".Ldone_%=:\n"                                         \
    ".Lgdone_%=:\n"                                        \
    "s_mov_b64 exec, %[save]\n"                            \
    MBK_G_FIXUP("32")                                      \
    "s_mov_b64 exec, %[save]\n"

#define MBK_G_CYC_INIT                                     \
    "v_mov_" MBK_CYC_MOV " %[szr], %[zr]\n"                \
    "v_mov_" MBK_CYC_MOV " %[szi], %[zi]\n"                \
    "s_mov_b32 %[tc], 0\n"                                 \
    "s_mov_b32 %[win], 1\n"
#define MBK_G_CYC_INIT_W                                   \
    "v_mov_" MBK_CYC_MOV " %[szr], %[zr]\n"                \
    "v_mov_" MBK_CYC_MOV " %[szi], %[zi]\n"                \
    "s_mov_b32 %[tc], 0\n"                                 \
    "s_mov_b32 %[win], %[win0]\n"
#define MBK_G_CYC(ZR, ZI, ID)                              \
    "v_cmp_eq_" MBK_CYC_BITS " vcc, " ZR ", %[szr]\n"      \
    "v_cmp_eq_" MBK_CYC_BITS "_e64 %[tmp2], " ZI ", %[szi]\n" \
    "s_and_b64 vcc, vcc, %[tmp2]\n"                        \
    "s_cbranch_vccnz .Lcyc" ID "_%=\n"                     \
    ".Lcyccont" ID "_%=:\n"                                \
    "s_add_u32 %[tc], %[tc], 1\n"                          \
    "s_cmp_ge_u32 %[tc], %[win]\n"                         \
    "s_cbranch_scc1 .Lcycsave" ID "_%=\n"                  \
    ".Lcycsaved" ID "_%=:\n"
#define MBK_G_CYC_OOL(ZR, ZI, ID)                          \
    ".Lcyc" ID "_%=:\n"                                    \
    "s_and_saveexec_b64 %[tmp], vcc\n"                     \
    "v_mov_b32 %[cnt], -1\n"                               \
    "s_andn2_b64 exec, %[tmp], vcc\n"                      \
    "s_cbranch_scc1 .Lcyccont" ID "_%=\n"                  \
    "s_branch .Lgdone_%=\n"                                \
    ".Lcycsave" ID "_%=:\n"                                \
    "v_mov_" MBK_CYC_MOV " %[szr], " ZR "\n"               \
    "v_mov_" MBK_CYC_MOV " %[szi], " ZI "\n"               \
    "s_mov_b32 %[tc], 0\n"                                 \
    "s_lshr_b32 %[k], %[win], 2\n"                         \
    "s_add_u32 %[k], %[k], 1\n"                            \
    "s_cmp_lt_u32 %[win], %[wcap]\n"                       \
    "s_cselect_b32 %[k], %[k], %[win]\n"                   \
    "s_add_u32 %[win], %[win], %[k]\n"                     \
    "s_branch .Lcycsaved" ID "_%=\n"
#define MBK_G_LOOP8CXI(INIT, FIX) MBK_G_LOOP8X(INIT, MBK_G_CYC("%[zr2]", "%[zi2]", "1"), MBK_G_CYC("%[zr]", "%[zi]", "2"), \
                                               MBK_G_CYC_OOL("%[zr2]", "%[zi2]", "1") MBK_G_CYC_OOL("%[zr]", "%[zi]", "2"), FIX)
#define MBK_G_LOOP8CX(FIX) MBK_G_LOOP8CXI(MBK_G_CYC_INIT, FIX)
#define MBK_G_LOOP8C_W MBK_G_LOOP8CXI(MBK_G_CYC_INIT_W, MBK_G_FIXUP("8"))
#define MBK_G_LOOP16CX(FIX) MBK_G_LOOP16X(MBK_G_CYC_INIT, MBK_G_CYC("%[zrt]", "%[zit]", "M1"), MBK_G_CYC("%[zr2]", "%[zi2]", "1"), \
                                          MBK_G_CYC("%[zrt]", "%[zit]", "M2"), MBK_G_CYC("%[zr]", "%[zi]", "2"), \
                                          MBK_G_CYC_OOL("%[zrt]", "%[zit]", "M1") MBK_G_CYC_OOL("%[zr2]", "%[zi2]", "1") \
                                          MBK_G_CYC_OOL("%[zrt]", "%[zit]", "M2") MBK_G_CYC_OOL("%[zr]", "%[zi]", "2"), FIX)
#define MBK_G_LOOP8C MBK_G_LOOP8CX(MBK_G_FIXUP("8"))
#define MBK_G_LOOP16C MBK_G_LOOP16CX(MBK_G_FIXUP("16"))
#define MBK_G_LOOP8C_NF MBK_G_LOOP8CX("")
#define MBK_G_LOOP16C_NF MBK_G_LOOP16CX("")
#define MBK_G_LOOP8C_R MBK_G_LOOP8CXI("", "")
#define MBK_G_LOOP16C_R MBK_G_LOOP16X("", MBK_G_CYC("%[zrt]", "%[zit]", "M1"), MBK_G_CYC("%[zr2]", "%[zi2]", "1"), \
                                      MBK_G_CYC("%[zrt]", "%[zit]", "M2"), MBK_G_CYC("%[zr]", "%[zi]", "2"), \
                                      MBK_G_CYC_OOL("%[zrt]", "%[zit]", "M1") MBK_G_CYC_OOL("%[zr2]", "%[zi2]", "1") \
                                      MBK_G_CYC_OOL("%[zrt]", "%[zit]", "M2") MBK_G_CYC_OOL("%[zr]", "%[zi]", "2"), "")

template <int kGroup = 4, bool kCycle = false, bool kFixup = true, bool kWin0 = false>
__device__ __forceinline__ void escape_steps_group(MBK_T cr, MBK_T ci, MBK_T &zr, MBK_T &zi, MBK_T &a,
                                                   MBK_T &b, MBK_T &m, int32_t &cnt, uint32_t n0, uint32_t total,
                                                   uint32_t cyc_wcap = 32u, uint32_t cyc_win0 = 1u)
{
    static_assert(kFixup || kGroup == 8 || kGroup == 16, "the form without the fix-up exists for 8- and 16-step groups");
    static_assert(!kWin0 || (kGroup == 8 && kCycle && kFixup), "a starting window exists for the 8-step cycle-test loop");
    MBK_T zr2, zi2, a2, b2, zrt, zit, at, bt, t, p;
    const uint32_t limit8 = n0 + ((total - n0) & (kGroup == 32 ? ~63u : kGroup == 16 ? ~31u : kGroup == 8 ? ~15u : ~7u));
    uint32_t n, k;
    unsigned long long save, tmp, tmp2;
#define MBK_G_OUTPUTS                                                                           \
                   [zr] "+&v"(zr), [zi] "+&v"(zi), [a] "+&v"(a), [b] "+&v"(b), [cnt] "+&v"(cnt),  \
                   [zr2] "=&v"(zr2), [zi2] "=&v"(zi2), [a2] "=&v"(a2), [b2] "=&v"(b2),            \
                   [zrt] "=&v"(zrt), [zit] "=&v"(zit), [at] "=&v"(at), [bt] "=&v"(bt),            \
                   [m] "+&v"(m), [t] "=&v"(t), [p] "=&v"(p), [n] "=&s"(n), [k] "=&s"(k),           \
                   [save] "=&s"(save), [tmp] "=&s"(tmp), [tmp2] "=&s"(tmp2)
#define MBK_G_INPUTS [cr] "v"(cr), [ci] "v"(ci), [total] "s"(total), [limit8] "s"(limit8), [n0] "s"(n0)
    if (kCycle && kGroup >= 8) {
        MBK_T szr, szi;
        uint32_t tc, win;
        if (kGroup == 16 && kFixup) {
            asm volatile(MBK_G_LOOP16C
                         : MBK_G_OUTPUTS, [szr] "=&v"(szr), [szi] "=&v"(szi), [tc] "=&s"(tc), [win] "=&s"(win)
                         : MBK_G_INPUTS, [wcap] "s"(cyc_wcap)
                         : "vcc", "scc");
        } else if (kGroup == 16) {
            asm volatile(MBK_G_LOOP16C_NF
                         : MBK_G_OUTPUTS, [szr] "=&v"(szr), [szi] "=&v"(szi), [tc] "=&s"(tc), [win] "=&s"(win)
                         : MBK_G_INPUTS, [wcap] "s"(cyc_wcap)
                         : "vcc", "scc");
        } else if (kWin0) {
            asm volatile(MBK_G_LOOP8C_W
                         : MBK_G_OUTPUTS, [szr] "=&v"(szr), [szi] "=&v"(szi), [tc] "=&s"(tc), [win] "=&s"(win)
                         : MBK_G_INPUTS, [wcap] "s"(cyc_wcap), [win0] "s"(cyc_win0)
                         : "vcc", "scc");
        } else if (kFixup) {
            asm volatile(MBK_G_LOOP8C
                         : MBK_G_OUTPUTS, [szr] "=&v"(szr), [szi] "=&v"(szi), [tc] "=&s"(tc), [win] "=&s"(win)
                         : MBK_G_INPUTS, [wcap] "s"(cyc_wcap)
                         : "vcc", "scc");
        } else {
            asm volatile(MBK_G_LOOP8C_NF
                         : MBK_G_OUTPUTS, [szr] "=&v"(szr), [szi] "=&v"(szi), [tc] "=&s"(tc), [win] "=&s"(win)
                         : MBK_G_INPUTS, [wcap] "s"(cyc_wcap)
                         : "vcc", "scc");
        }
    } else if (kGroup == 32) {
        asm volatile(MBK_G_LOOP32 : MBK_G_OUTPUTS : MBK_G_INPUTS : "vcc", "scc");
    } else if (kGroup == 16 && kFixup) {
        asm volatile(MBK_G_LOOP16 : MBK_G_OUTPUTS : MBK_G_INPUTS : "vcc", "scc");
    } else if (kGroup == 16) {
        asm volatile(MBK_G_LOOP16_NF : MBK_G_OUTPUTS : MBK_G_INPUTS : "vcc", "scc");
    } else if (kGroup == 8 && kFixup) {
        asm volatile(MBK_G_LOOP8 : MBK_G_OUTPUTS : MBK_G_INPUTS : "vcc", "scc");
    } else if (kGroup == 8) {
        asm volatile(MBK_G_LOOP8_NF : MBK_G_OUTPUTS : MBK_G_INPUTS : "vcc", "scc");
    } else {
        asm volatile(MBK_G_LOOP : MBK_G_OUTPUTS : MBK_G_INPUTS : "vcc", "scc");
    }
#undef MBK_G_OUTPUTS
#undef MBK_G_INPUTS
}

template <int kGroup>
__device__ __forceinline__ void escape_steps_carry(MBK_T cr, MBK_T ci, MBK_T &zr, MBK_T &zi, MBK_T &a, MBK_T &b, MBK_T &m, int32_t &cnt,
                                                   uint32_t n0, uint32_t total, uint32_t cyc_wcap, MBK_T &szr, MBK_T &szi, uint32_t &tc, uint32_t &win)
{
    static_assert(kGroup == 8 || kGroup == 16, "8- or 16-step groups");
    MBK_T zr2, zi2, a2, b2, zrt, zit, at, bt, t, p;
    uint32_t n, k;
    unsigned long long save, tmp, tmp2;
#define MBK_G_CARRY_OPERANDS                                                                       \
                 : [zr] "+&v"(zr), [zi] "+&v"(zi), [a] "+&v"(a), [b] "+&v"(b), [cnt] "+&v"(cnt),    \
                   [zr2] "=&v"(zr2), [zi2] "=&v"(zi2), [a2] "=&v"(a2), [b2] "=&v"(b2),              \
                   [zrt] "=&v"(zrt), [zit] "=&v"(zit), [at] "=&v"(at), [bt] "=&v"(bt),              \
                   [m] "+&v"(m), [t] "=&v"(t), [p] "=&v"(p), [n] "=&s"(n), [k] "=&s"(k),             \
                   [save] "=&s"(save), [tmp] "=&s"(tmp), [tmp2] "=&s"(tmp2),                        \
                   [szr] "+&v"(szr), [szi] "+&v"(szi), [tc] "+&s"(tc), [win] "+&s"(win)              \
                 : [cr] "v"(cr), [ci] "v"(ci), [total] "s"(stop), [limit8] "s"(limit8), [n0] "s"(start), [wcap] "s"(cyc_wcap) \
                 : "vcc", "scc"
    uint32_t start = n0;
    if (kGroup == 16) {
        const uint32_t stop = n0 + ((total - n0) & ~31u), limit8 = stop;
        if (stop > start) {
            asm volatile(MBK_G_LOOP16C_R MBK_G_CARRY_OPERANDS);
            tc = (uint32_t)__builtin_amdgcn_readfirstlane((int)tc);
            win = (uint32_t)__builtin_amdgcn_readfirstlane((int)win);
        }
        start = stop;
    }
    if (total > start) {
        const uint32_t stop = total, limit8 = start + ((total - start) & ~15u);
        if (cnt == 0) {
            asm volatile(MBK_G_LOOP8C_R MBK_G_CARRY_OPERANDS);
        }
        tc = (uint32_t)__builtin_amdgcn_readfirstlane((int)tc);
        win = (uint32_t)__builtin_amdgcn_readfirstlane((int)win);
    }
#undef MBK_G_CARRY_OPERANDS
}

__device__ __forceinline__ void escape_fixup(MBK_T cr, MBK_T ci, MBK_T &zr, MBK_T &zi, MBK_T &a, MBK_T &b, MBK_T &m, int32_t &cnt)
{
    MBK_T t, p;
    uint32_t k;
    unsigned long long save, tmp2;
    asm volatile("s_mov_b64 %[save], exec\n"
                 MBK_G_FIXUP("16")
                 "s_mov_b64 exec, %[save]\n"
                 : [zr] "+&v"(zr), [zi] "+&v"(zi), [a] "+&v"(a), [b] "+&v"(b), [cnt] "+&v"(cnt), [m] "+&v"(m), [t] "=&v"(t), [p] "=&v"(p),
                   [k] "=&s"(k), [save] "=&s"(save), [tmp2] "=&s"(tmp2)
                 : [cr] "v"(cr), [ci] "v"(ci)
                 : "vcc", "scc");
}

template <int kGroup, bool kCycle = false, bool kFixup = true>
__device__ __forceinline__ void escape_steps_tail(MBK_T cr, MBK_T ci, MBK_T &zr, MBK_T &zi, MBK_T &a, MBK_T &b,
                                                  MBK_T &m, int32_t &cnt, uint32_t n0, uint32_t total, uint32_t cyc_wcap = 32u)
{
    if (kGroup == 32) {
        static_assert(kGroup != 32 || !kCycle, "32-step groups have no cycle test");
        const uint32_t t64 = n0 + ((total - n0) & ~63u);
        if (t64 > n0) escape_steps_group<32, false>(cr, ci, zr, zi, a, b, m, cnt, n0, t64);
        if (cnt == 0 && total > t64) escape_steps_tail<16, false>(cr, ci, zr, zi, a, b, m, cnt, t64, total);
    } else if (kGroup == 16) {
        const uint32_t t32 = n0 + ((total - n0) & ~31u);
        if (t32 > n0) escape_steps_group<16, kCycle, kFixup>(cr, ci, zr, zi, a, b, m, cnt, n0, t32, cyc_wcap);
        if (cnt == 0 && total > t32) escape_steps_group<8, kCycle, kFixup>(cr, ci, zr, zi, a, b, m, cnt, t32, total, cyc_wcap);
    } else {
        escape_steps_group<kGroup, kCycle, kFixup>(cr, ci, zr, zi, a, b, m, cnt, n0, total, cyc_wcap);
    }
}

template <int kGroup = 4, bool kCycle = false>
__device__ __forceinline__ int32_t escape_count_group(MBK_T cr, MBK_T ci, int32_t mrd, MBK_T *m_out = nullptr,
                                                      uint32_t kExactSteps = 8, uint32_t cyc_wcap = 32u)
{
    MBK_T zr = cr, zi = ci;
    MBK_T a = zr * zr, b = zi * zi, m = 0;
    int32_t cnt = 0;
    const uint32_t total = mrd > 1 ? (uint32_t)mrd - 1u : 0u;
    const uint32_t first = total < kExactSteps ? total : kExactSteps;
    escape_steps_asm<true>(cr, ci, zr, zi, a, b, m, cnt, 0u, first);
    if (cnt == 0 && total > first) escape_steps_tail<kGroup, kCycle>(cr, ci, zr, zi, a, b, m, cnt, first, total, cyc_wcap);
    if (m_out) *m_out = m;
    return kCycle && cnt < 0 ? 0 : cnt;
}

template <bool kFmaDouble>
__device__ __forceinline__ int32_t escape_count_asm_from(MBK_T z0r, MBK_T z0i, MBK_T cr, MBK_T ci, int32_t mrd, MBK_T *m_out = nullptr)
{
    MBK_T zr = z0r, zi = z0i;
    MBK_T a = zr * zr, b = zi * zi, m = 0;
    int32_t cnt = 0;
    escape_steps_asm<kFmaDouble>(cr, ci, zr, zi, a, b, m, cnt, 0u, mrd > 1 ? (uint32_t)mrd - 1u : 0u);
    if (m_out) *m_out = m;
    return cnt;
}

template <int kGroup = 8, bool kCycle = false>
__device__ __forceinline__ int32_t escape_count_group_from(MBK_T z0r, MBK_T z0i, MBK_T cr, MBK_T ci, int32_t mrd, MBK_T *m_out = nullptr,
                                                           uint32_t kExactSteps = 8, uint32_t cyc_wcap = 32u)
{
    MBK_T zr = z0r, zi = z0i;
    MBK_T a = zr * zr, b = zi * zi, m = 0;
    int32_t cnt = 0;
    const uint32_t total = mrd > 1 ? (uint32_t)mrd - 1u : 0u;
    const uint32_t first = total < kExactSteps ? total : kExactSteps;
    escape_steps_asm<true>(cr, ci, zr, zi, a, b, m, cnt, 0u, first);
    if (cnt == 0 && total > first) escape_steps_tail<kGroup, kCycle>(cr, ci, zr, zi, a, b, m, cnt, first, total, cyc_wcap);
    if (m_out) *m_out = m;
    return kCycle && cnt < 0 ? 0 : cnt;
}

#define MBK_LR_TEST                                        \
    "v_mul_" MBK_F " %[a], %[zr], %[zr]\n"                 \
    "v_mul_" MBK_F " %[b], %[zi], %[zi]\n"                 \
    "v_add_" MBK_F " %[m], %[a], %[b]\n"                   \
    "v_cmp_gt_" MBK_F " vcc, 4.0, %[m]\n"                  \
    "v_addc_co_u32_e64 %[cnt], %[tmp], %[cnt], 0, vcc\n"   \
    "s_mov_b64 exec, vcc\n"                                \
    "s_cbranch_execz .Llrdone_%=\n"
#define MBK_LR_BODY(STORES)                                \
    "s_mov_b64 %[save], exec\n"                            \
    ".Llrblk_%=:\n"                                        \
    "v_cvt_f64_u32 %[t64], %[row]\n"                       \
    "v_mul_f64 %[t64], %[t64], %[step]\n"                  \
    MBK_CI_FROM_T64                                        \
    "v_mov_b32 %[cnt], 1\n"                                \
    "v_mul_" MBK_F " %[b], %[ci], %[ci]\n"                 \
    "v_add_" MBK_F " %[t], %[a0], -%[b]\n"                 \
    "v_mul_" MBK_F " %[p], %[cr], %[ci]\n"                 \
    "v_add_" MBK_F " %[zr], %[t], %[cr]\n"                 \
    "v_fma_" MBK_F " %[zi], %[p], 2.0, %[ci]\n"            \
    MBK_LR_TEST                                            \
    MBK_STEP_HEAD_FMA MBK_LR_TEST                          \
    MBK_STEP_HEAD_FMA MBK_LR_TEST                          \
    MBK_STEP_HEAD_FMA MBK_LR_TEST                          \
    "s_mov_b64 exec, %[save]\n"                            \
    "s_mov_b32 %[flag], 1\n"                               \
    "s_branch .Llrend_%=\n"                                \
    ".Llrdone_%=:\n"                                       \
    "s_mov_b64 exec, %[save]\n"                            \
    STORES                                                 \
    "v_add_u32 %[row], %[rowinc], %[row]\n"                \
    "v_add_u32 %[off], %[einc], %[off]\n"                  \
    "s_sub_u32 %[n], %[n], 1\n"                            \
    "s_cmp_lg_u32 %[n], 0\n"                               \
    "s_cbranch_scc1 .Llrblk_%=\n"                          \
    "s_mov_b32 %[flag], 0\n"                               \
    ".Llrend_%=:\n"
#define MBK_LR_ST_COUNTS "global_store_dword %[off], %[cnt], %[cbase]\n"
#define MBK_LR_ST_BYTES_Q                                  \
    "v_lshl_add_u32 %[q], %[cnt], 3, -8\n"                 \
    "v_lshrrev_b32_e64 %[q], %[q], %[qtab]\n"
#define MBK_LR_ST_BYTES_ONLY MBK_LR_ST_BYTES_Q "global_store_byte %[off], %[q], %[bbase]\n"
#define MBK_LR_ST_BOTH MBK_LR_ST_COUNTS MBK_LR_ST_BYTES_Q "v_lshrrev_b32 %[o2], 2, %[off]\nglobal_store_byte %[o2], %[q], %[bbase]\n"
template <bool kCounts, bool kBytes, bool kAcc = false>
__device__ __forceinline__ uint32_t escape_light_run(MBK_T cr, MBK_T a0, uint32_t &row, uint32_t rowinc, double im_step,
                                                     double im_start, int32_t &cnt, int32_t *cbase, uint8_t *bbase,
                                                     uint32_t &off, uint32_t einc, uint32_t qtab, uint32_t &n,
                                                     uint32_t *acc_io = nullptr)
{
    MBK_T ci, zr, zi, a, b, t, p, m;
    double t64;
    uint32_t q, o2, flag;
    unsigned long long tmp, save;
    const unsigned long long step_bits = (unsigned long long)__double_as_longlong(im_step);
    const unsigned long long start_bits = (unsigned long long)__double_as_longlong(im_start);
    uint32_t acc = kAcc ? *acc_io : 0u;
#define MBK_LR_OPERANDS                                                                                    \
        : [row] "+v"(row), [off] "+v"(off), [cnt] "=&v"(cnt), [n] "+s"(n), [acc] "+v"(acc), [ci] "=&v"(ci), [zr] "=&v"(zr), \
          [zi] "=&v"(zi), [a] "=&v"(a), [b] "=&v"(b), [m] "=&v"(m), [t] "=&v"(t), [p] "=&v"(p),            \
          [t64] "=&v"(t64), [q] "=&v"(q), [o2] "=&v"(o2), [tmp] "=&s"(tmp), [save] "=&s"(save),            \
          [flag] "=&s"(flag)                                                                               \
        : [cr] "v"(cr), [a0] "v"(a0), [step] "s"(step_bits), [start] "s"(start_bits), [cbase] "s"(cbase),  \
          [bbase] "s"(bbase), [qtab] "s"(qtab), [rowinc] "s"(rowinc), [einc] "s"(einc)                     \
        : "vcc", "scc", "memory"
#define MBK_LR_ACC "v_add_u32 %[acc], %[acc], %[cnt]\n"
    if (kAcc) {
        if (kCounts && kBytes) {
            asm volatile(MBK_LR_BODY(MBK_LR_ACC MBK_LR_ST_BOTH) MBK_LR_OPERANDS);
        } else if (kCounts) {
            asm volatile(MBK_LR_BODY(MBK_LR_ACC MBK_LR_ST_COUNTS) MBK_LR_OPERANDS);
        } else {
            asm volatile(MBK_LR_BODY(MBK_LR_ACC MBK_LR_ST_BYTES_ONLY) MBK_LR_OPERANDS);
        }
        *acc_io = acc;
    } else if (kCounts && kBytes) {
        asm volatile(MBK_LR_BODY(MBK_LR_ST_BOTH) MBK_LR_OPERANDS);
    } else if (kCounts) {
        asm volatile(MBK_LR_BODY(MBK_LR_ST_COUNTS) MBK_LR_OPERANDS);
    } else {
        asm volatile(MBK_LR_BODY(MBK_LR_ST_BYTES_ONLY) MBK_LR_OPERANDS);
    }
#undef MBK_LR_ACC
#undef MBK_LR_OPERANDS
    n = (uint32_t)__builtin_amdgcn_readfirstlane((int)n);
    return (uint32_t)__builtin_amdgcn_readfirstlane((int)flag);
}
#define MBK_LW_TEST                                        \
    "v_mul_" MBK_F " %[a], %[zr], %[zr]\n"                 \
    "v_mul_" MBK_F " %[b], %[zi], %[zi]\n"                 \
    "v_add_" MBK_F " %[m], %[a], %[b]\n"                   \
    "v_cmp_gt_" MBK_F " vcc, 4.0, %[m]\n"                  \
    "v_addc_co_u32_e64 %[cnt], %[tmp], %[cnt], 0, vcc\n"   \
    "s_mov_b64 exec, vcc\n"                                \
    "s_cbranch_execz .Llwdone_%=\n"
#define MBK_LW_BODY(STORES)                                \
    "s_mov_b64 %[save], exec\n"                            \
    ".Llwblk_%=:\n"                                        \
    "s_bitcmp1_b32 %[mask], %[k]\n"                        \
    "s_cbranch_scc0 .Llwnext_%=\n"                         \
    "s_lshl_b32 %[kk], %[k], 3\n"                          \
    "v_add_u32 %[c], %[kk], %[col]\n"                      \
    "v_cvt_f64_u32 %[t64], %[c]\n"                         \
    "v_mul_f64 %[t64], %[t64], %[step]\n"                  \
    MBK_CR_FROM_T64                                        \
    "v_mov_b32 %[cnt], 1\n"                                \
    "v_mul_" MBK_F " %[a], %[cr], %[cr]\n"                 \
    "v_add_" MBK_F " %[t], %[a], -%[b0]\n"                 \
    "v_mul_" MBK_F " %[p], %[cr], %[ci]\n"                 \
    "v_add_" MBK_F " %[zr], %[t], %[cr]\n"                 \
    "v_fma_" MBK_F " %[zi], %[p], 2.0, %[ci]\n"            \
    MBK_LW_TEST                                            \
    MBK_STEP_HEAD_FMA MBK_LW_TEST                          \
    MBK_STEP_HEAD_FMA MBK_LW_TEST                          \
    MBK_STEP_HEAD_FMA MBK_LW_TEST                          \
    "s_mov_b64 exec, %[save]\n"                            \
    "s_mov_b32 %[flag], 1\n"                               \
    "s_branch .Llwend_%=\n"                                \
    ".Llwdone_%=:\n"                                       \
    "s_mov_b64 exec, %[save]\n"                            \
    "s_mul_i32 %[kk], %[k], %[einc]\n"                     \
    "v_add_u32 %[o], %[kk], %[off]\n"                      \
    STORES                                                 \
    ".Llwnext_%=:\n"                                       \
    "s_add_u32 %[k], %[k], 1\n"                            \
    "s_cmp_lt_u32 %[k], 8\n"                               \
    "s_cbranch_scc1 .Llwblk_%=\n"                          \
    "s_mov_b32 %[flag], 0\n"                               \
// ... 94 lines not shown
```

distributedmandelbrot_amd/csrc/mbk_units.h:

```cpp
#pragma once

#include "mbk_refill.h"

namespace mbk {

__host__ __device__ inline size_t units_settled_base(size_t n) { return 2u * n + 64u; }
__host__ __device__ inline size_t units_list_words(size_t n) { return 3u * n + 64u; }

struct XcdShares { uint32_t cum[8]; };
__host__ __device__ inline void units_plan(uint32_t n_h, uint32_t n_v, uint32_t n_m, const uint32_t *cum, uint32_t stamps, uint32_t *plan,
                                           uint32_t n_ml, uint32_t n_hs);

__device__ __forceinline__ int32_t probe_settling(double cr, double ci, int32_t cap, double *delta)
{
    double zr = cr, zi = ci;
    int32_t n = 1;
    for (; n < cap - 9; ++n) {
        const double t = zr * zr - zi * zi;
        zi = __builtin_fma(2.0, zr * zi, ci);
        zr = t + cr;
        if (zr * zr + zi * zi >= 4.0) { *delta = 1e300; return n; }
    }
    double hr[9], hi[9];
#pragma unroll
    for (int k = 0; k < 9; ++k) hr[k] = hi[k] = 1e150;
    for (; n < cap; ++n) {
        const double t = zr * zr - zi * zi;
        zi = __builtin_fma(2.0, zr * zi, ci);
        zr = t + cr;
        if (zr * zr + zi * zi >= 4.0) { *delta = 1e300; return n; }
#pragma unroll
        for (int k = 8; k > 0; --k) { hr[k] = hr[k - 1]; hi[k] = hi[k - 1]; }
        hr[0] = zr;
        hi[0] = zi;
    }
    double d = 1e300;
#pragma unroll
    for (int k = 1; k <= 8; ++k) {
        if (k == 7) continue;
        const double dr = hr[0] - hr[k], di = hi[0] - hi[k], q = dr * dr + di * di;
        d = q < d ? q : d;
    }
    *delta = d;
    return 0;
}

__global__ __launch_bounds__(1024) void classify_units_kernel(TileArgs p, uint32_t nregions, int32_t probe_steps,
                                                              uint32_t *order, uint32_t *counters, int32_t m_late, double settle_thr,
                                                              uint32_t *extra, uint32_t *plan, XcdShares shares, uint32_t stamps)
{
    __shared__ uint32_t s_last;
    __shared__ uint32_t s_cnt[5][16], s_base[5];
    const uint32_t r = blockIdx.x * blockDim.x + threadIdx.x;
    const uint32_t lane = threadIdx.x & 63u, wave = threadIdx.x >> 6;
    const bool valid = r < nregions;
    uint32_t cls = 5u;
    uint32_t by = 0, bx = 0;
    if (valid) {
        by = r / p.blocks_x;
        bx = r - by * p.blocks_x;
        uint32_t lc = bx * 8u + 4u, lr = by * 8u + 4u;
        lc = lc < p.ncols ? lc : p.ncols - 1u;
        lr = lr < p.nrows ? lr : p.nrows - 1u;
        const double cr = axis_value(p.re, p.col0 + lc), ci = axis_value(p.im, p.row0 + lr);
        const int32_t cap = p.mrd < probe_steps ? p.mrd : probe_steps;
        double delta = 1e300;
        const int32_t cnt = cap > 1 ? (settle_thr > 0.0 ? probe_settling(cr, ci, cap, &delta) : escape_count<true>(cr, ci, cap)) : 1;
        const bool regular = bx < p.fast_bx_end && by < p.fast_by_end;
        cls = cnt == 0 ? (delta <= settle_thr ? 4u : 0u) : (cnt <= 3 && regular ? 1u : (m_late > 0 && cnt >= m_late ? 3u : 2u));
    }
    const unsigned long long vmask = __ballot(cls == 1u);
    const uint32_t seg = (uint32_t)(vmask >> (lane & ~7u)) & 0xffu;
    const bool emit[5] = {cls == 0u, (lane & 7u) == 0u && seg != 0u, cls == 2u, cls == 3u, cls == 4u};
    unsigned long long m[5];
#pragma unroll
    for (uint32_t k = 0; k < 5u; ++k) {
        m[k] = __ballot(emit[k]);
        if (lane == 0) s_cnt[k][wave] = (uint32_t)__popcll(m[k]);
    }
    __syncthreads();
    if (threadIdx.x < 5u) {
        const uint32_t k = threadIdx.x, nw = (blockDim.x + 63u) >> 6;
        uint32_t t = 0;
        for (uint32_t w = 0; w < nw; ++w) {
            const uint32_t c = s_cnt[k][w];
            s_cnt[k][w] = t;
            t += c;
        }
        s_base[k] = t ? atomicAdd(k < 3u ? &counters[k] : &extra[k - 3u], t) : 0u;
    }
    __syncthreads();
    const unsigned long long below = (1ull << lane) - 1ull;
    if (emit[0]) order[s_base[0] + s_cnt[0][wave] + (uint32_t)__popcll(m[0] & below)] = (by << 16) | bx;
    if (emit[1]) order[nregions - 1u - (s_base[1] + s_cnt[1][wave] + (uint32_t)__popcll(m[1] & below))] = (by << 16) | ((bx >> 3) << 8) | seg;
    if (emit[2]) order[nregions + 3u + s_base[2] + s_cnt[2][wave] + (uint32_t)__popcll(m[2] & below)] = (by << 16) | bx;
    if (emit[3]) order[2u * nregions + 2u - (s_base[3] + s_cnt[3][wave] + (uint32_t)__popcll(m[3] & below))] = (by << 16) | bx;
    if (emit[4]) order[units_settled_base(nregions) + s_base[4] + s_cnt[4][wave] + (uint32_t)__popcll(m[4] & below)] = (by << 16) | bx;
    if (plan == nullptr) return;
    __syncthreads();
    if (threadIdx.x == 0) {
        __threadfence();
        s_last = atomicAdd(&extra[2], 1u) == gridDim.x - 1u ? 1u : 0u;
    }
    __syncthreads();
    if (s_last != 0u && threadIdx.x == 0) {
        __threadfence();
        const uint32_t n_h = atomicExch(&counters[0], 0u), n_v = atomicExch(&counters[1], 0u), n_m = atomicExch(&counters[2], 0u);
        const uint32_t n_ml = atomicExch(&extra[0], 0u), n_hs = atomicExch(&extra[1], 0u);
        atomicExch(&extra[2], 0u);
        units_plan(n_h + n_ml + n_hs, n_v, n_m, shares.cum, stamps, plan, n_ml, n_hs);
    }
}

constexpr uint32_t kStampTail = 8;
constexpr uint32_t kStampWords = 8u + 8u * kStampTail;
constexpr uint32_t kPlanWords = 40;

__host__ __device__ inline void units_plan(uint32_t n_h, uint32_t n_v, uint32_t n_m, const uint32_t *cum, uint32_t stamps, uint32_t *plan,
                                           uint32_t n_ml, uint32_t n_hs)
{
    const uint32_t n_l = n_m + n_v, total = n_h + n_l;
    uint32_t h[8], l[8], prev = 0, slots = (total + 7u) >> 3;
    for (uint32_t x = 0; x < 8u; ++x) {
        uint32_t c = x == 7u ? n_h : (uint32_t)(((unsigned long long)n_h * cum[x]) >> 24);
        c = c < prev ? prev : (c > n_h ? n_h : c);
        h[x] = c - prev;
        prev = c;
        slots = slots > h[x] ? slots : h[x];
    }
    uint32_t left = n_l, hmin = 0xffffffffu, lmin = 0xffffffffu;
    for (uint32_t x = 0; x < 8u; ++x) {
        const uint32_t room = slots - h[x];
        l[x] = room < left ? room : left;
        left -= l[x];
        hmin = hmin < h[x] ? hmin : h[x];
        lmin = lmin < l[x] ? lmin : l[x];
    }
    plan[0] = n_h; plan[1] = n_m; plan[2] = slots * 8u; plan[3] = hmin; plan[4] = lmin; plan[5] = stamps; plan[6] = n_ml < n_h ? n_ml : n_h; plan[7] = n_hs < n_h ? n_h - n_hs : 0u;
    uint32_t hb = 8u * hmin, lb = 8u * lmin;
    for (uint32_t x = 0; x < 8u; ++x) {
        plan[8u + x] = h[x];
        plan[16u + x] = l[x];
        plan[24u + x] = hb - hmin;
        plan[32u + x] = lb - lmin;
        hb += h[x] - hmin;
        lb += l[x] - lmin;
    }
}

__host__ __device__ __forceinline__ bool units_lookup(uint32_t u, uint32_t hmin, uint32_t lmin, uint32_t h_x, uint32_t l_x,
                                                      uint32_t hbase_x, uint32_t lbase_x, bool &is_h, uint32_t &i)
{
    const uint32_t x = u & 7u, j = u >> 3, k = j - h_x;
    is_h = j < h_x;
    if (!is_h && k >= l_x) return false;
    i = is_h ? (j < hmin ? u : hbase_x + j) : (k < lmin ? 8u * k + x : lbase_x + k);
    return true;
}

__device__ __forceinline__ void load_shares(const uint32_t *plan, uint32_t x, uint32_t &n_m, uint32_t &total, uint32_t &hmin,
                                            uint32_t &lmin, uint32_t &stamps, uint32_t &n_ml, uint32_t &hs0, uint32_t &h_x, uint32_t &l_x,
                                            uint32_t &hbase_x, uint32_t &lbase_x)
{
    const uint32_t *pl = plan, *px = plan + x;
    asm volatile("s_load_dword %0, %11, 0x4\n\t"
                 "s_load_dword %1, %11, 0x8\n\t"
                 "s_load_dword %2, %11, 0xc\n\t"
                 "s_load_dword %3, %11, 0x10\n\t"
                 "s_load_dword %4, %11, 0x14\n\t"
                 "s_load_dword %5, %11, 0x18\n\t"
                 "s_load_dword %6, %11, 0x1c\n\t"
                 "s_load_dword %7, %12, 0x20\n\t"
                 "s_load_dword %8, %12, 0x40\n\t"
                 "s_load_dword %9, %12, 0x60\n\t"
                 "s_load_dword %10, %12, 0x80\n\t"
                 "s_waitcnt lgkmcnt(0)"
                 : "=&s"(n_m), "=&s"(total), "=&s"(hmin), "=&s"(lmin), "=&s"(stamps), "=&s"(n_ml), "=&s"(hs0), "=&s"(h_x), "=&s"(l_x),
                   "=&s"(hbase_x), "=&s"(lbase_x)
                 : "s"(pl), "s"(px)
                 : "memory");
}

__device__ __forceinline__ void leave_stamp(uint32_t slot)
{
    unsigned long long base;
    uint32_t tag;
    asm volatile("s_load_dwordx2 %0, %2, %3\n\t"
                 "s_load_dword %1, %2, %4\n\t"
                 "s_waitcnt lgkmcnt(0)"
                 : "=&s"(base), "=&s"(tag)
                 : "s"(__builtin_amdgcn_kernarg_segment_ptr()), "n"(offsetof(TileArgs, stamps)), "n"(offsetof(TileArgs, stamp_tag))
                 : "memory");
    if (__lane_id() == 0)
        reinterpret_cast<unsigned long long *>(base)[slot] = (wall_clock64() & 0xffffffffffffull) | ((unsigned long long)tag << 48);
}

template <typename T, int kGroup, bool kCycle, bool kCounts, bool kBytes, bool kStats = false>
__global__ __launch_bounds__(64) __attribute__((amdgpu_waves_per_eu(8, 8))) void tile_units_kernel(TileArgs args, uint32_t qtab)
{
    static_assert(!kStats || (!kCounts && kBytes), "fused statistics exist for the bytes-only instantiation");
    unsigned long long heavy = 0;
    uint32_t acc = 0;
    const uint32_t never_cap = args.mrd > 1 ? (uint32_t)args.mrd - 1u : 0u;
    TileArgs p = args;
    p.smooth = nullptr;
    p.stats = nullptr;
    p.quant_wide = 0u;
    p.re.step_is_zero = p.im.step_is_zero = 0u;
    if (!kCounts) p.counts = nullptr;
    if (!kBytes) p.bytes = nullptr;
    const uint32_t lane = threadIdx.x;
    const uint32_t lx = lane & 7u, ly = lane >> 3;
    const uint32_t n = p.ngrid;
    const uint32_t x = blockIdx.x & 7u;
    const uint32_t oscale = kCounts ? 4u : 1u;
    for (uint32_t u = blockIdx.x;; u += p.unit_stride) {
        uint32_t n_m, total, hmin, lmin, stamps, n_ml, hs0, h_x, l_x, hbase_x, lbase_x;
        load_shares(args.plan, x, n_m, total, hmin, lmin, stamps, n_ml, hs0, h_x, l_x, hbase_x, lbase_x);
        if (stamps && u < p.unit_stride) {
            const uint32_t j0 = u >> 3, slots = total >> 3;
            if (j0 == 0u) leave_stamp(x);
            if (j0 < slots && j0 + kStampTail >= slots) leave_stamp(8u + x * kStampTail + (j0 + kStampTail - slots));
        }
        if (u >= total) break;
        bool is_h;
        uint32_t i;
        if (!units_lookup(u, hmin, lmin, h_x, l_x, hbase_x, lbase_x, is_h, i)) break;
        if (is_h || i < n_m) {
            const bool late = is_h && i < n_ml;
            const uint32_t e = scalar_load_u32(p.order, is_h ? (late ? 2u * n + 2u - i : (i < hs0 ? i - n_ml : (uint32_t)units_settled_base(n) + (i - hs0)))
                                                              : n + 3u + i);
            const uint32_t by = e >> 16, bx = e & 0xffffu;
            const int32_t c = block_pixel<T, true, kGroup, kCycle>(p, bx * 8u, by * 8u, lx, ly, kGroup >= 16 && is_h && !late,
                                                                   bx < p.fast_bx_end && by < p.fast_by_end);
            if (kStats && c >= 0) heavy += c > 0 ? (unsigned long long)(uint32_t)c : (1ull << 47) + never_cap;
        } else {
            const uint32_t v = scalar_load_u32(p.order, n - 1u - (i - n_m));
            const uint32_t by = v >> 16, bx0 = ((v >> 8) & 0xffu) << 3, mask = v & 0xffu;
            const T ci = (T)((double)(p.row0 + by * 8u + ly) * p.im.step + p.im.start);
            const T b0 = ci * ci;
            const size_t elem0 = (size_t)(by * 8u + p.out_row0) * p.out_pitch + bx0 * 8u + p.out_col0;
            int32_t *cb = reinterpret_cast<int32_t *>(uniform_u64(reinterpret_cast<unsigned long long>(kCounts ? p.counts + elem0 : nullptr)));
            uint8_t *bb = reinterpret_cast<uint8_t *>(uniform_u64(reinterpret_cast<unsigned long long>(kBytes ? p.bytes + elem0 : nullptr)));
            const uint32_t col = p.col0 + bx0 * 8u + lx, off = (ly * p.out_pitch + lx) * oscale;
            uint32_t k = 0;
            int32_t cnt;
            while (escape_light_row<kCounts, kBytes, kStats>(ci, b0, col, p.re.step, p.re.start, cnt, cb, bb, off, 8u * oscale, qtab, mask, k, &acc) != 0u) {
                const int32_t c = block_pixel<T, true, kGroup, kCycle>(p, (bx0 + k) * 8u, by * 8u, lx, ly, false, true);
                if (kStats && c >= 0) heavy += c > 0 ? (unsigned long long)(uint32_t)c : (1ull << 47) + never_cap;
                if (++k >= 8u) break;
            }
        }
    }
    if (kStats) {
        const unsigned long long iters = wave_sum_u64((heavy & ((1ull << 47) - 1ull)) + acc), never = wave_sum_u64(heavy >> 47);
        ReduceOut *out = &args.stats[blockIdx.x % kReduceSlots].r;
        if (lane == 0) {
            if (iters) atomicAdd(&out->pixel_iterations, iters);
            if (never) atomicAdd(&out->never_pixels, never);
        }
    }
}

}
```

distributedmandelbrot_amd/device.py:

```python
from __future__ import annotations

import ctypes as C
import math
from dataclasses import dataclass
from decimal import Decimal
from fractions import Fraction
from typing import Optional, Tuple, Union

import numpy as np

from . import _lib as L


class MbkError(RuntimeError):
    def __init__(self, status: int, message: str):
        super().__init__(f"libmbk_hip status {status}: {message}")
        self.status = status


def _error_text(lib, ctx=None) -> str:
    return (lib.mbk_last_error(ctx) or b"").decode()


def _check(lib, st: int, ctx=None) -> None:
# ... 330 lines not shown
                                              out.ctypes.data if out.size else None))
    return out


def density_cell_host(target: DensityTarget, z) -> Optional[Tuple[int, int]]:
    lib = L.load()
    ct = target.ctarget()
    cx, cy, inside = C.c_uint32(0), C.c_uint32(0), C.c_int(0)
    _check(lib, lib.mbk_density_cell_host(C.byref(ct), float(z[0]), float(z[1]), C.byref(cx), C.byref(cy), C.byref(inside)))
    return (int(cx.value), int(cy.value)) if inside.value else None


def density_host(view: View, target: DensityTarget, mrd: int, *, min_count: int = 1, max_count: int = 0, window=None,
                 out: Optional[np.ndarray] = None):
    lib = L.load()
    cv = MandelbrotDevice._cview(view, window)
    ct = target.ctarget()
    shape = (max(int(target.height), 0), max(int(target.width), 0))
    table = np.zeros(shape, np.uint32) if out is None else _out_array(out, shape, np.uint32)
    ds = L.mbk_density_stats()
    _check(lib, lib.mbk_density_accumulate_host(C.byref(cv), C.byref(ct), mrd, min_count, max_count,
                                                table.ctypes.data if table.size else None, C.byref(ds)))
    return table.reshape(shape), DensityStats(int(ds.deposits), int(ds.dropped))


def _stream_array(stream) -> np.ndarray:
    if isinstance(stream, np.ndarray):
        a = np.ascontiguousarray(stream, dtype=np.uint8).ravel()
    else:
        a = np.frombuffer(stream, np.uint8)
    return a


_EMPTY_STREAM = (C.c_uint8 * 1)()


def _stream_ptr(a: np.ndarray) -> int:
    return a.ctypes.data if a.size else C.addressof(_EMPTY_STREAM)


class ChunkStreamError(MbkError):

    def __init__(self, reason: int, message: str):
        super().__init__(L.MBK_ERR_INVALID, message)
        self.reason = reason


def chunk_stream_check(stream, n: int = L.MBK_CHUNK_BYTES) -> Tuple[int, int]:
    lib = L.load()
    a = _stream_array(stream)
    codec, runs, reason = C.c_uint32(0), C.c_uint64(0), C.c_uint32(0)
    st = lib.mbk_chunk_stream_check(_stream_ptr(a), a.size, n, C.byref(codec), C.byref(runs), C.byref(reason))
    if st != L.MBK_OK:
        raise ChunkStreamError(int(reason.value), _error_text(lib))
    return int(codec.value), int(runs.value)


def decode_chunk_host(stream, n: int = L.MBK_CHUNK_BYTES, out: Optional[np.ndarray] = None) -> np.ndarray:
    lib = L.load()
    a = _stream_array(stream)
    out = _out_array(out, n, np.uint8)
    _check(lib, lib.mbk_chunk_decode_host(_stream_ptr(a), a.size, n, out.ctypes.data))
    return out


class MandelbrotDevice:

    SLOTS = L.MBK_SLOTS
    WORKER_DEPTH = L.MBK_WORKER_DEPTH

    def __init__(self, device: int = 0):
        self._lib = L.load()
        h = C.c_void_p()
        _check(self._lib, self._lib.mbk_create(device, C.byref(h)))
        self._h = h
        self.device = device
        self._pinned = []
        self._ser_buf = np.empty(1 + L.MBK_CHUNK_BYTES, np.uint8)

    def close(self) -> None:
        if getattr(self, "_h", None):
            for p in self._pinned:
                self._lib.mbk_host_free(self._h, p)
            self._pinned = []
            self._lib.mbk_destroy(self._h)
            self._h = None

    def __enter__(self):
        return self

    def __exit__(self, *exc):
        self.close()

    def __del__(self):
        try:
            self.close()
        except Exception:
            pass

    def _check(self, st: int) -> None:
        _check(self._lib, st, self._h)

    def info(self) -> dict:
        inf = L.mbk_device_info()
        self._check(self._lib.mbk_get_device_info(self._h, C.byref(inf)))
        return {"name": inf.name.decode(), "arch": inf.arch.decode(),
                "compute_units": inf.compute_units, "clock_mhz": inf.clock_mhz,
                "wavefront_size": inf.wavefront_size, "total_mem": inf.total_mem}

    def pci_bus_id(self) -> str:
        buf = C.create_string_buffer(32)
        self._check(self._lib.mbk_device_pci_bus_id(self._h, buf, 32))
        return buf.value.decode()

    def pinned_empty(self, shape, dtype) -> np.ndarray:
        dtype = np.dtype(dtype)
        n = int(np.prod(shape)) * dtype.itemsize
        p = C.c_void_p()
        self._check(self._lib.mbk_host_alloc(self._h, max(n, 1), C.byref(p)))
        self._pinned.append(p)
        buf = (C.c_uint8 * max(n, 1)).from_address(p.value)
        return np.frombuffer(buf, dtype=dtype, count=int(np.prod(shape))).reshape(shape)

    def set_option(self, name: str, value: int) -> None:
        self._check(self._lib.mbk_set_option(self._h, L.OPTIONS[name], int(value)))

    def get_option(self, name: str) -> int:
        v = C.c_uint32(0)
        self._check(self._lib.mbk_get_option(self._h, L.OPTIONS[name], C.byref(v)))
        return int(v.value)

    def scan_occupancy(self) -> dict:
        out = {}
        for k, name in enumerate(["f64_scan", "f64_heavy", "f32_scan", "f32_heavy"]):
            v = C.c_uint32(0)
            self._check(self._lib.mbk_get_option(self._h, L.MBK_INFO_SCAN_WG_PER_CU + k, C.byref(v)))
            out[name] = int(v.value)
        return out

    def xcd_shares(self) -> dict:
        vals = []
        for k in range(10):
            v = C.c_uint32(0)
            self._check(self._lib.mbk_get_option(self._h, L.MBK_INFO_XCD_SHARE + k, C.byref(v)))
            vals.append(int(v.value))
        return {"shares": [round(v / 1048576.0, 5) for v in vals[:8]], "last_launch_read": vals[8], "units_launches": vals[9]}

    def spill_info(self) -> dict:
        a, b = C.c_uint32(0), C.c_uint32(0)
        self._check(self._lib.mbk_get_option(self._h, L.MBK_INFO_SPILL, C.byref(a)))
        self._check(self._lib.mbk_get_option(self._h, L.MBK_INFO_SPILL + 1, C.byref(b)))
        return {"lanes_last_launch": int(a.value), "launches": int(b.value)}

    def quantise_counts(self, counts: np.ndarray, mrd: int) -> np.ndarray:
        counts = np.ascontiguousarray(counts, dtype=np.int32)
        out = np.empty(counts.shape, np.uint8)
        self._check(self._lib.mbk_quantise_counts(self._h, counts.ctypes.data, counts.size, mrd, out.ctypes.data))
        return out

    @staticmethod
    def _cview(view: View, window) -> L.mbk_view:
        col0, row0, ncols, nrows = window if window is not None else (0, 0, view.width, view.height)
        return L.mbk_view(view.start_r, view.start_i, view.range_r, view.range_i,
                          view.width, view.height, col0, row0, ncols, nrows)

    def compute_view(self, view: View, mrd: int, *, window=None, want_counts: bool = True,
                     want_bytes: bool = True, kernel: str = "default", precision: str = "f64",
                     out_counts: Optional[np.ndarray] = None, out_bytes: Optional[np.ndarray] = None):
        cv = self._cview(view, window)
        shape = (cv.nrows, cv.ncols)
        counts = _out_array(out_counts, shape, np.int32) if want_counts else None
        byts = _out_array(out_bytes, shape, np.uint8) if want_bytes else None
        flags, p_counts, p_bytes = _wanted(shape, counts, byts)
        st = L.mbk_stats()
        self._check(self._lib.mbk_view_compute(self._h, C.byref(cv), mrd, L.KERNELS[kernel] | L.PRECISIONS[precision] | flags,
                                               p_counts, p_bytes, C.byref(st)))
        return counts, byts, _stats(st)

    def datachunk(self, level: int, mrd: int, index_real: int, index_imag: int, *,
                  want_counts: bool = False, out_bytes: Optional[np.ndarray] = None):
        byts = _out_array(out_bytes, L.MBK_CHUNK_BYTES, np.uint8)
        counts = np.empty(L.MBK_CHUNK_BYTES, np.int32) if want_counts else None
        st = L.mbk_stats()
        self._check(self._lib.mbk_datachunk(
            self._h, level, mrd, index_real, index_imag, byts.ctypes.data,
            counts.ctypes.data if counts is not None else None, C.byref(st)))
        return byts, counts, _stats(st)

    def compute_view_smooth(self, view: View, mrd: int, *, window=None, kernel: str = "default"):
        cv = self._cview(view, window)
        shape = (cv.nrows, cv.ncols)
        smooth = np.empty(shape, np.float64)
        counts = np.empty(shape, np.int32)
        st = L.mbk_stats()
        self._check(self._lib.mbk_view_compute_smooth(self._h, C.byref(cv), mrd, L.KERNELS[kernel],
                                                      counts.ctypes.data, smooth.ctypes.data, C.byref(st)))
        return smooth, counts, _stats(st)

    def launch_view_smooth(self, view: View, mrd: int, *, d_smooth: int, d_counts: int = 0, stream: int = 0,
                           window=None, kernel: str = "default") -> None:
        cv = self._cview(view, window)
        self._check(self._lib.mbk_view_launch_smooth(self._h, C.byref(cv), mrd, L.KERNELS[kernel],
                                                     d_counts or None, d_smooth, stream or None))

    def compute_view_distance(self, view: View, mrd: int, *, window=None, kernel: str = "default"):
        cv = self._cview(view, window)
        shape = (cv.nrows, cv.ncols)
        dist = np.empty(shape, np.float64)
        counts = np.empty(shape, np.int32)
        st = L.mbk_stats()
        self._check(self._lib.mbk_view_compute_distance(self._h, C.byref(cv), mrd, L.KERNELS[kernel],
                                                        counts.ctypes.data, dist.ctypes.data, C.byref(st)))
        return dist, counts, _stats(st)

    def launch_view_distance(self, view: View, mrd: int, *, d_distance: int, d_counts: int = 0, stream: int = 0,
                             window=None, kernel: str = "default") -> None:
        cv = self._cview(view, window)
        self._check(self._lib.mbk_view_launch_distance(self._h, C.byref(cv), mrd, L.KERNELS[kernel],
                                                       d_counts or None, d_distance, stream or None))

    def compute_view_interior(self, view: View, mrd: int, *, window=None, kernel: str = "default", want_counts: bool = True,
                              want_period: bool = True, want_distance: bool = True):
        cv = self._cview(view, window)
        shape = (cv.nrows, cv.ncols)
        period = np.empty(shape, np.int32) if want_period else None
        dist = np.empty(shape, np.float64) if want_distance else None
        counts = np.empty(shape, np.int32) if want_counts else None
        st = L.mbk_stats()
        ptr = lambda a: a.ctypes.data if a is not None else None
        self._check(self._lib.mbk_view_interior_compute(self._h, C.byref(cv), mrd, L.KERNELS[kernel], ptr(counts), ptr(period),
                                                        ptr(dist), C.byref(st)))
        return period, dist, counts, _stats(st)

    def launch_view_interior(self, view: View, mrd: int, *, d_period: int = 0, d_distance: int = 0, d_counts: int = 0,
                             stream: int = 0, window=None, kernel: str = "default") -> None:
        cv = self._cview(view, window)
        self._check(self._lib.mbk_view_interior_launch(self._h, C.byref(cv), mrd, L.KERNELS[kernel], d_counts or None,
                                                       d_period or None, d_distance or None, stream or None))

    def render_view_interior(self, view: View, mrd: int, *, palette, scale: float = 2.0 ** 80, supersample: int = 1,
                             unknown=(0, 0, 0, 255), outside=(255, 255, 255, 255), window=None, kernel: str = "default",
                             max_band_rows: int = 0, out: Optional[np.ndarray] = None):
        cv = self._cview(view, window)
        spec, pal = _interior_spec(palette, supersample, unknown, outside, scale, max_band_rows)
        img = self._render_out(cv, out)
        st = L.mbk_stats()
        self._check(self._lib.mbk_view_interior_render_compute(self._h, C.byref(cv), mrd, L.KERNELS[kernel], C.byref(spec),
                                                               img.ctypes.data, C.byref(st)))
        return img, _stats(st)

    def launch_render_view_interior(self, view: View, mrd: int, *, palette, d_rgba: int, scale: float = 2.0 ** 80,
                                    supersample: int = 1, unknown=(0, 0, 0, 255), outside=(255, 255, 255, 255), stream: int = 0,
                                    window=None, kernel: str = "default", max_band_rows: int = 0) -> None:
        cv = self._cview(view, window)
        spec, pal = _interior_spec(palette, supersample, unknown, outside, scale, max_band_rows)
        self._check(self._lib.mbk_view_interior_render_launch(self._h, C.byref(cv), mrd, L.KERNELS[kernel], C.byref(spec),
                                                              d_rgba or None, stream or None))

    def serialize_last(self) -> Tuple[bytes, int]:
        cap = len(self._ser_buf)
        size, codec = C.c_uint64(0), C.c_uint32(0)
        st = self._lib.mbk_serialize_last(self._h, self._ser_buf.ctypes.data, cap, C.byref(size), C.byref(codec))
        if st == L.MBK_ERR_INVALID and size.value > cap:
            self._ser_buf = np.empty(size.value, np.uint8)
            st = self._lib.mbk_serialize_last(self._h, self._ser_buf.ctypes.data, size.value, C.byref(size),
                                              C.byref(codec))
        self._check(st)
        return self._ser_buf[:size.value].tobytes(), int(codec.value)

    def submit_datachunk(self, slot: int, level: int, mrd: int, index_real: int, index_imag: int,
                         out_bytes: np.ndarray, lazy_uniform: bool = False) -> None:
        assert out_bytes.dtype == np.uint8 and out_bytes.size == L.MBK_CHUNK_BYTES and out_bytes.flags.c_contiguous
        self._check(self._lib.mbk_datachunk_submit_ex(self._h, slot, level, mrd, index_real, index_imag,
                                                      out_bytes.ctypes.data, None,
                                                      L.MBK_LAZY_UNIFORM if lazy_uniform else 0))

    def submit_view(self, slot: int, view: View, mrd: int, *, window=None, out_counts: Optional[np.ndarray] = None,
                    out_bytes: Optional[np.ndarray] = None, kernel: str = "default", precision: str = "f64") -> None:
        cv = self._cview(view, window)
        flags, p_counts, p_bytes = _wanted((cv.nrows, cv.ncols), out_counts, out_bytes)
        self._check(self._lib.mbk_view_submit(self._h, slot, C.byref(cv), mrd, L.KERNELS[kernel] | L.PRECISIONS[precision] | flags,
                                              p_counts, p_bytes))

    def wait(self, slot: int) -> TileStats:
        st = L.mbk_stats()
        self._check(self._lib.mbk_wait(self._h, slot, C.byref(st)))
        return _stats(st)

    def launch_view(self, view: View, mrd: int, *, d_counts: int = 0, d_bytes: int = 0,
                    stream: int = 0, window=None, kernel: str = "default", precision: str = "f64") -> None:
        cv = self._cview(view, window)
        flags = (L.KERNELS[kernel] | L.PRECISIONS[precision] | (L.MBK_WANT_COUNTS if d_counts else 0)
                 | (L.MBK_WANT_BYTES if d_bytes else 0))
        self._check(self._lib.mbk_view_launch(self._h, C.byref(cv), mrd, flags,
                                              d_counts or None, d_bytes or None, stream or None))

    @staticmethod
    def _cdeep(view: Union[DeepView, WideDeepView], window):
        col0, row0, ncols, nrows = window if window is not None else (0, 0, view.width, view.height)
        if isinstance(view, WideDeepView):
            return L.mbk_deep_xview(view.range_r, view.range_i, view.exp2, view.width, view.height, col0, row0, ncols, nrows)
        return L.mbk_deep_view(view.span_r, view.span_i, view.width, view.height, col0, row0, ncols, nrows)

    def _deep_fn(self, view, name: str, bla: bool = False, source: Optional[str] = None, xbla: bool = False):
        if isinstance(view, WideDeepView):
            if bla:
# ... 379 lines not shown
```

include/mbk.h:

```cpp
#ifndef MBK_H
#define MBK_H

#include <stdint.h>

#ifdef __cplusplus
extern "C" {
#endif

#define MBK_ABI_VERSION 5

#define MBK_CHUNK_DEFINITION 4096u
#define MBK_CHUNK_BYTES (4096u * 4096u)

enum mbk_status {
    MBK_OK = 0,
    MBK_ERR_INVALID = 1,
    MBK_ERR_NO_DEVICE = 2,
    MBK_ERR_HIP = 3,
    MBK_ERR_NOMEM = 4,
    MBK_ERR_NET = 5
};

#define MBK_WANT_COUNTS 0x1u
#define MBK_WANT_BYTES 0x2u
// ... 231 lines not shown
                                          uint32_t flags, const mbk_render_spec *spec, const double *h_lut, uint32_t lut_len,
                                          uint8_t *d_rgba, void *hip_stream);
int mbk_deep_view_render_equalized_compute(mbk_ctx *ctx, const mbk_deep_orbit *orbit, const mbk_deep_view *view, uint32_t mrd,
                                           uint32_t flags, const mbk_render_spec *spec, const double *h_lut, uint32_t lut_len,
                                           uint8_t *h_rgba, mbk_stats *stats);
int mbk_deep_xview_render_equalized_launch(mbk_ctx *ctx, const mbk_deep_orbit *orbit, const mbk_deep_xview *view, uint32_t mrd,
                                           uint32_t flags, const mbk_render_spec *spec, const double *h_lut, uint32_t lut_len,
                                           uint8_t *d_rgba, void *hip_stream);
int mbk_deep_xview_render_equalized_compute(mbk_ctx *ctx, const mbk_deep_orbit *orbit, const mbk_deep_xview *view, uint32_t mrd,
                                            uint32_t flags, const mbk_render_spec *spec, const double *h_lut, uint32_t lut_len,
                                            uint8_t *h_rgba, mbk_stats *stats);
int mbk_render_resolve_equalized_host(const mbk_render_spec *spec, const double *h_lut, uint32_t lut_len, uint32_t width,
                                      uint32_t height, const int32_t *counts, const double *smooth, uint8_t *rgba);

int mbk_julia_view_launch(mbk_ctx *ctx, const mbk_view *view, double c_r, double c_i, uint32_t mrd, uint32_t flags,
                          int32_t *d_counts, uint8_t *d_bytes, double *d_smooth, void *hip_stream);
int mbk_julia_view_compute(mbk_ctx *ctx, const mbk_view *view, double c_r, double c_i, uint32_t mrd, uint32_t flags,
                           int32_t *h_counts, uint8_t *h_bytes, double *h_smooth, mbk_stats *stats);
int mbk_julia_view_submit(mbk_ctx *ctx, int slot, const mbk_view *view, double c_r, double c_i, uint32_t mrd, uint32_t flags,
                          int32_t *h_counts, uint8_t *h_bytes);
int mbk_julia_view_render_launch(mbk_ctx *ctx, const mbk_view *view, double c_r, double c_i, uint32_t mrd, uint32_t flags,
                                 const mbk_render_spec *spec, uint8_t *d_rgba, void *hip_stream);
int mbk_julia_view_render_compute(mbk_ctx *ctx, const mbk_view *view, double c_r, double c_i, uint32_t mrd, uint32_t flags,
                                  const mbk_render_spec *spec, uint8_t *h_rgba, mbk_stats *stats);
int mbk_julia_view_render_equalized_launch(mbk_ctx *ctx, const mbk_view *view, double c_r, double c_i, uint32_t mrd,
                                           uint32_t flags, const mbk_render_spec *spec, const double *h_lut, uint32_t lut_len,
                                           uint8_t *d_rgba, void *hip_stream);
int mbk_julia_view_render_equalized_compute(mbk_ctx *ctx, const mbk_view *view, double c_r, double c_i, uint32_t mrd,
                                            uint32_t flags, const mbk_render_spec *spec, const double *h_lut, uint32_t lut_len,
                                            uint8_t *h_rgba, mbk_stats *stats);
int mbk_julia_view_histogram_launch(mbk_ctx *ctx, const mbk_view *view, double c_r, double c_i, uint32_t mrd, uint32_t flags,
                                    uint64_t *d_hist, void *hip_stream);
int mbk_julia_view_histogram_compute(mbk_ctx *ctx, const mbk_view *view, double c_r, double c_i, uint32_t mrd, uint32_t flags,
                                     uint64_t *h_hist, mbk_stats *stats);
int mbk_julia_count_host(double z_r, double z_i, double c_r, double c_i, uint32_t mrd, int32_t *count, double *mag);

#define MBK_DENSITY_MAX_CELLS (1u << 28)
#define MBK_DENSITY_LINEAR 0u
#define MBK_DENSITY_SQRT 1u
typedef struct mbk_density_target {
    double start_r, start_i;
    double range_r, range_i;
    uint32_t width, height;
} mbk_density_target;
typedef struct mbk_density_stats {
    uint64_t deposits;
    uint64_t dropped;
} mbk_density_stats;
typedef struct mbk_density_render_spec {
    uint32_t mode;
    uint32_t factor;
    const uint8_t *palette;
    uint32_t palette_len;
    double scale, offset;
} mbk_density_render_spec;
int mbk_view_density_launch(mbk_ctx *ctx, const mbk_view *view, const mbk_density_target *target, uint32_t mrd, uint32_t min_count,
                            uint32_t max_count, uint32_t flags, uint32_t *d_density, void *hip_stream);
int mbk_view_density_compute(mbk_ctx *ctx, const mbk_view *view, const mbk_density_target *target, uint32_t mrd, uint32_t min_count,
                             uint32_t max_count, uint32_t flags, uint32_t *h_density, mbk_stats *stats, mbk_density_stats *dstats);
int mbk_density_max(mbk_ctx *ctx, const uint32_t *d_density, uint64_t n, uint32_t *max, uint64_t *total, void *hip_stream);
int mbk_density_render_launch(mbk_ctx *ctx, const uint32_t *d_density, uint32_t width, uint32_t height,
                              const mbk_density_render_spec *spec, uint8_t *d_rgba, void *hip_stream);
int mbk_density_render_compute(mbk_ctx *ctx, const uint32_t *h_density, uint32_t width, uint32_t height,
                               const mbk_density_render_spec *spec, uint8_t *h_rgba, mbk_stats *stats);
int mbk_density_cell_host(const mbk_density_target *target, double z_r, double z_i, uint32_t *cell_x, uint32_t *cell_y, int *inside);
int mbk_density_accumulate_host(const mbk_view *view, const mbk_density_target *target, uint32_t mrd, uint32_t min_count,
                                uint32_t max_count, uint32_t *density, mbk_density_stats *dstats);
int mbk_density_resolve_host(const mbk_density_render_spec *spec, uint32_t width, uint32_t height, const uint32_t *density,
                             uint8_t *rgba);
int mbk_density_build_info(void);

typedef struct mbk_interior_render_spec {
    uint32_t supersample;
    const uint8_t *palette;
    uint32_t palette_len;
    uint8_t unknown[4];
    uint8_t outside[4];
    double scale;
    uint32_t max_band_rows;
} mbk_interior_render_spec;
int mbk_view_interior_launch(mbk_ctx *ctx, const mbk_view *view, uint32_t mrd, uint32_t flags, int32_t *d_counts,
                             int32_t *d_period, double *d_distance, void *hip_stream);
int mbk_view_interior_compute(mbk_ctx *ctx, const mbk_view *view, uint32_t mrd, uint32_t flags, int32_t *h_counts,
                              int32_t *h_period, double *h_distance, mbk_stats *stats);
int mbk_interior_host(double c_r, double c_i, uint32_t mrd, int32_t *count, int32_t *period, int32_t *cycle_len, double *de);
int mbk_view_interior_render_launch(mbk_ctx *ctx, const mbk_view *view, uint32_t mrd, uint32_t flags,
                                    const mbk_interior_render_spec *spec, uint8_t *d_rgba, void *hip_stream);
int mbk_view_interior_render_compute(mbk_ctx *ctx, const mbk_view *view, uint32_t mrd, uint32_t flags,
                                     const mbk_interior_render_spec *spec, uint8_t *h_rgba, mbk_stats *stats);
int mbk_interior_resolve_host(const mbk_interior_render_spec *spec, uint32_t width, uint32_t height, const int32_t *counts,
                              const int32_t *period, const double *de, uint8_t *rgba);

#define MBK_CODEC_RAW 0x00u
#define MBK_CODEC_RLE 0x01u

int mbk_serialize_last(mbk_ctx *ctx, uint8_t *h_out, uint64_t cap, uint64_t *size, uint32_t *codec);

#define MBK_STREAM_OK 0u
#define MBK_STREAM_BAD_CODEC 1u
#define MBK_STREAM_BAD_SIZE 2u
#define MBK_STREAM_ZERO_RUN 3u
#define MBK_STREAM_TOO_LONG 4u
#define MBK_STREAM_TOO_SHORT 5u

typedef struct mbk_chunk_spec {
    const uint8_t *palette;
    uint32_t scale;
} mbk_chunk_spec;

int mbk_chunk_stream_check(const uint8_t *stream, uint64_t size, uint64_t n, uint32_t *codec, uint64_t *runs, uint32_t *reason);
int mbk_chunk_decode_host(const uint8_t *stream, uint64_t size, uint64_t n, uint8_t *bytes);
int mbk_chunk_resolve_host(const mbk_chunk_spec *spec, const uint8_t *bytes, uint8_t *rgba, uint64_t pitch_px);
int mbk_chunk_decode_launch(mbk_ctx *ctx, const uint8_t *h_stream, uint64_t size, uint64_t n, uint8_t *d_bytes,
                            uint32_t *d_status, void *hip_stream);
int mbk_chunk_render_launch(mbk_ctx *ctx, const uint8_t *h_stream, uint64_t size, const mbk_chunk_spec *spec, uint8_t *d_rgba,
                            uint64_t pitch_px, uint32_t *d_status, void *hip_stream);
int mbk_chunk_decode_compute(mbk_ctx *ctx, const uint8_t *h_stream, uint64_t size, uint64_t n, uint8_t *h_bytes,
                             mbk_stats *stats);
int mbk_chunk_render_compute(mbk_ctx *ctx, const uint8_t *h_stream, uint64_t size, const mbk_chunk_spec *spec, uint8_t *h_rgba,
                             uint64_t pitch_px, mbk_stats *stats);

enum mbk_option {
    MBK_OPT_ORDER = 0,
    MBK_OPT_WAVES_PER_WG,
    MBK_OPT_GROUP_STEPS,
    MBK_OPT_EXACT_STEPS,
    MBK_OPT_PROBE_STEPS,
    MBK_OPT_SCAN_WAVES,
    MBK_OPT_SCAN_XCD_MAP,
    MBK_OPT_SCAN_COL_PERIOD,
    MBK_OPT_HEAVY_SHARE,
    MBK_OPT_RF_LIVEMIN,
    MBK_OPT_RF_PATIENCE,
    MBK_OPT_RF_BATCH,
    MBK_OPT_RF_WAVES,
    MBK_OPT_CYCLE_DETECT,
    MBK_OPT_PROBE_MID,
    MBK_OPT_PREPASS_OVERLAP,
    MBK_OPT_EXACT_LONG,
    MBK_OPT_SCAN_INLINE,
    MBK_OPT_WAVE_LIMIT,
    MBK_OPT_UNITS_MIN_LIGHT,
    MBK_OPT_XCD_BALANCE,
    MBK_OPT_M_LATE,
    MBK_OPT_H_SETTLED,
    MBK_OPT_CLASSIFY_WG,
    MBK_OPT_SCAN_STRIP,
    MBK_OPT_CYCLE_WINDOW,
    MBK_OPT_SPILL_FIRST,
    MBK_OPT_SPILL_LANES,
    MBK_OPT_SPILL_MIN_MRD,
    MBK_OPT_SPILL_MIN_BLOCKS,
    MBK_OPT_SPILL_CYC_SHIFT,
    MBK_OPT_COUNT_
};
#define MBK_INFO_SCAN_WG_PER_CU 100
#define MBK_INFO_XCD_SHARE 110
#define MBK_INFO_SPILL 130
int mbk_set_option(mbk_ctx *ctx, int option, uint32_t value);
int mbk_get_option(mbk_ctx *ctx, int option, uint32_t *value);

int mbk_units_plan(uint32_t n_h, uint32_t n_v, uint32_t n_m, const double *fractions, uint32_t *plan);
int mbk_units_lookup(const uint32_t *plan, uint32_t id, uint32_t *list, uint32_t *index);

int mbk_quantise_counts(mbk_ctx *ctx, const int32_t *h_counts, uint64_t n, uint32_t mrd, uint8_t *h_bytes);

int mbk_reduce_counts(mbk_ctx *ctx, const int32_t *d_counts, uint64_t n, uint32_t mrd,
                      void *hip_stream, mbk_stats *stats);

typedef struct mbk_worker_report {
    uint64_t leased;
    uint64_t accepted;
    uint64_t rejected;
    uint64_t resets;
    uint64_t uniform_tiles;
    uint64_t pixel_iterations;
    double kernel_ms_sum;
    double seconds;
    uint64_t net_retries;
} mbk_worker_report;
int mbk_worker_run(mbk_ctx *ctx, const char *addr, uint16_t port, uint64_t max_tiles, uint32_t senders,
                   mbk_worker_report *report);

enum mbk_net_option {
    MBK_NET_MAX_CONNECTIONS = 0,
    MBK_NET_CONNECT_TIMEOUT_MS = 1,
    MBK_NET_IO_TIMEOUT_MS = 2,
    MBK_NET_RETRIES = 3,
    MBK_NET_BACKOFF_MS = 4,
    MBK_NET_STOP = 5,
    MBK_NET_PEAK_CONNECTIONS = 6,
    MBK_NET_FEEDER_SLOTS = 7,
    MBK_NET_OPT_COUNT_
};
int mbk_net_set_option(int option, uint32_t value);
int mbk_net_get_option(int option, uint32_t *value);

typedef struct mbk_feeder_ops {
    void *user;
    int (*submit)(void *user, int slot, uint32_t level, uint32_t mrd, uint32_t index_real, uint32_t index_imag, uint8_t *h_bytes);
    int (*wait)(void *user, int slot, mbk_stats *stats);
    void *(*alloc)(void *user, uint64_t bytes);
    void (*release)(void *user, void *ptr);
    void (*on_tile)(void *user, const uint32_t workload[4], const mbk_stats *stats, int status);
} mbk_feeder_ops;
int mbk_feeder_run(const mbk_feeder_ops *ops, const char *addr, uint16_t port, uint64_t max_tiles, uint32_t senders,
                   mbk_worker_report *report);

#ifdef __cplusplus
}
#endif
#endif
```

Measured before the change: 5297.

## Add opt-in paired-block interior iteration and trim cycle-check compare

Adds an h_pair option that classifies pairs of vertically adjacent provably-interior 8x8 blocks and iterates both orbits interleaved in one wave via a dual-orbit asm loop, raising instruction-level parallelism for fp64 dependency chains. The classifier and units plan are extended to place paired blocks, and an info query reports pair counts. Separately, the cycle-detection check now tests only the real part inline and defers the imaginary compare to the out-of-line path, shortening the hot loop. The pairing is off by default and adds register pressure and complexity.

```diff
diff --git a/distributedmandelbrot_amd/_lib.py b/distributedmandelbrot_amd/_lib.py
--- a/distributedmandelbrot_amd/_lib.py
+++ b/distributedmandelbrot_amd/_lib.py
@@ -21,7 +21,7 @@
            "refill": MBK_KERNEL_REFILL, "group": MBK_KERNEL_GROUP, "scan": MBK_KERNEL_SCAN}
 OPTIONS = {name: i for i, name in enumerate(
     ["order", "waves_per_wg", "group_steps", "exact_steps", "probe_steps", "scan_waves", "scan_xcd_map", "scan_col_period", "heavy_share",
-     "rf_livemin", "rf_patience", "rf_batch", "rf_waves", "cycle_detect", "probe_mid", "prepass_overlap", "exact_long", "scan_inline", "wave_limit", "units_min_light", "xcd_balance", "m_late", "h_settled", "classify_wg", "scan_strip", "cycle_window", "spill_first", "spill_lanes", "spill_min_mrd", "spill_min_blocks", "spill_cyc_shift"])}
+     "rf_livemin", "rf_patience", "rf_batch", "rf_waves", "cycle_detect", "probe_mid", "prepass_overlap", "exact_long", "scan_inline", "wave_limit", "units_min_light", "xcd_balance", "m_late", "h_settled", "classify_wg", "scan_strip", "cycle_window", "spill_first", "spill_lanes", "spill_min_mrd", "spill_min_blocks", "spill_cyc_shift", "h_pair"])}
 MBK_PRECISION_F32 = 0x1000
 MBK_LAZY_UNIFORM = 0x2000
 MBK_DEEP_BLA = 0x8000
@@ -32,6 +32,7 @@
 MBK_INFO_SCAN_WG_PER_CU = 100
 MBK_INFO_XCD_SHARE = 110
 MBK_INFO_SPILL = 130
+MBK_INFO_H_PAIR = 140
 MBK_CODEC_RAW = 0x00
 MBK_CODEC_RLE = 0x01
 MBK_CHUNK_DEFINITION = 4096
diff --git a/distributedmandelbrot_amd/csrc/mbk_api.hip b/distributedmandelbrot_amd/csrc/mbk_api.hip
--- a/distributedmandelbrot_amd/csrc/mbk_api.hip
+++ b/distributedmandelbrot_amd/csrc/mbk_api.hip
@@ -175,6 +175,9 @@
     uint32_t wave_limit_lds[8] = {0, 0, 0, 0, 0, 0, 0, 0};
     uint32_t spill_launches = 0;
     hipStream_t last_spill_stream = nullptr;
+    uint32_t pair_launches = 0;
+    const uint32_t *last_units_plan = nullptr;
+    hipStream_t last_units_stream = nullptr;
     struct ProbeKey { Axis re, im; uint32_t col0, row0, ncols, nrows; } probe_key = {};
     double probe_share = 0.0;
     bool probe_valid = false;
@@ -462,6 +465,7 @@
     dim3 grid, block;
     uint32_t order_mode, probe_steps;
     bool cyc, units, ordered;
+    bool pair;
     double unit_share;
 };
 
@@ -479,16 +483,19 @@
     p.probe_steps = ctx->opt[MBK_OPT_PROBE_STEPS];
     a.perm_mul = p.order_mode == 1 ? coprime_multiplier(p.grid.x) : 1u;
     a.order = nullptr;
+    const bool small = ctx->opt[MBK_OPT_H_PAIR] == 2u;
+    const bool worth = small ? (uint32_t)a.mrd > p.probe_steps : p.grid.x >= 16384u && (uint32_t)a.mrd > 2u * p.probe_steps;
     p.units = p.order_mode == 3 && p.wpw == 1u && kernel == MBK_KERNEL_GROUP && !safe && a.smooth == nullptr &&
               (a.counts || a.bytes) && !(a.bytes && a.quant_wide) && a.blocks_x % 8u == 0u && a.blocks_x <= 2048u &&
               a.fast_bx_end > 0u && a.fast_by_end > 0u && (f32 || ctx->opt[MBK_OPT_GROUP_STEPS] == 16u) &&
-              p.grid.x >= 16384u && (uint32_t)a.mrd > 2u * p.probe_steps && p.by <= 0xffffu;
+              worth && p.by <= 0xffffu;
     p.unit_share = 0.0;
     if (p.units) {
         p.unit_share = window_heavy_share(ctx, a);
         p.units = (1.0 - p.unit_share) * 65536.0 >= (double)ctx->opt[MBK_OPT_UNITS_MIN_LIGHT];
     }
-    p.ordered = p.order_mode >= 2 && p.grid.x >= 16384u && (uint32_t)a.mrd > 2u * p.probe_steps && a.blocks_x <= 0xffffu && p.by <= 0xffffu;
+    p.ordered = p.order_mode >= 2 && (p.units || (p.grid.x >= 16384u && (uint32_t)a.mrd > 2u * p.probe_steps)) && a.blocks_x <= 0xffffu && p.by <= 0xffffu;
+    p.pair = p.units && ctx->opt[MBK_OPT_H_PAIR] != 0u && !p.cyc;
     return p;
 }
 
@@ -542,6 +549,7 @@
         MBK_HIP(ctx, hipStreamSynchronize(stream));
         if (ring.aux) MBK_HIP(ctx, hipStreamSynchronize(ring.aux));
         ring.drop_lists();
+        ctx->last_units_plan = nullptr;
         for (int k = 0; k < kOrderRing; ++k)
             MBK_HIP(ctx, hipMalloc((void **)&ring.d_order[k], mbk::units_list_words(nblocks) * sizeof(uint32_t)));
         ring.order_cap = nblocks;
@@ -597,9 +605,13 @@
     a.stamps = balance == 1u ? sc->h_stamps + (size_t)(seq % kStampSlots) * mbk::kStampWords : nullptr;
     a.stamp_tag = seq & 0xffffu;
     const uint32_t cwg = ctx->opt[MBK_OPT_CLASSIFY_WG];
-    hipLaunchKernelGGL(mbk::classify_units_kernel, dim3((p.grid.x + cwg - 1u) / cwg), dim3(cwg), 0, ol.pre, a, p.grid.x,
+    const uint32_t cthreads = p.pair ? a.blocks_x * ((p.by + 1u) & ~1u) : p.grid.x;
+    hipLaunchKernelGGL(mbk::classify_units_kernel, dim3((cthreads + cwg - 1u) / cwg), dim3(cwg), 0, ol.pre, a, p.grid.x,
                        (int32_t)p.probe_steps, ol.list, ctl, (int32_t)ctx->opt[MBK_OPT_M_LATE], settle_thr, ctl + 3, (uint32_t *)a.plan, w,
-                       a.stamps ? 1u : 0u);
+                       a.stamps ? 1u : 0u, p.pair ? 1u : 0u);
+    ctx->last_units_plan = p.pair ? a.plan : nullptr;
+    ctx->last_units_stream = stream;
+    if (p.pair) ++ctx->pair_launches;
     return MBK_OK;
 }
 
@@ -667,8 +679,15 @@
 typedef void (*BlockKernel)(TileArgs);
 typedef void (*SpillKernel)(TileArgs, const uint32_t *, const unsigned long long *, uint32_t);
 
-static UnitsKernel pick_units_kernel(bool f32, bool cyc, bool stats, bool counts, bool bytes)
-{
+static UnitsKernel pick_units_kernel(bool f32, bool cyc, bool stats, bool counts, bool bytes, bool pair)
+{
+    static const UnitsKernel pair_forms[2][4] = {
+        {mbk::tile_units_kernel<float, 8, false, false, true, true, true>, mbk::tile_units_kernel<float, 8, false, true, true, false, true>,
+         mbk::tile_units_kernel<float, 8, false, false, true, false, true>, mbk::tile_units_kernel<float, 8, false, true, false, false, true>},
+        {mbk::tile_units_kernel<double, 16, false, false, true, true, true>, mbk::tile_units_kernel<double, 16, false, true, true, false, true>,
+         mbk::tile_units_kernel<double, 16, false, false, true, false, true>, mbk::tile_units_kernel<double, 16, false, true, false, false, true>},
+    };
+    if (pair && !cyc) return pair_forms[f32 ? 0 : 1][stats ? 0 : (counts && bytes) ? 1 : bytes ? 2 : 3];
     static const UnitsKernel forms[4][4] = {
         {mbk::tile_units_kernel<float, 8, true, false, true, true>, mbk::tile_units_kernel<float, 8, true, true, true>,
          mbk::tile_units_kernel<float, 8, true, false, true>, mbk::tile_units_kernel<float, 8, true, true, false>},
@@ -723,7 +742,7 @@
         a.counts = nullptr;
         fuse->fused = true;
     }
-    hipLaunchKernelGGL(pick_units_kernel(f32, p.cyc, stats, a.counts != nullptr, a.bytes != nullptr), dim3(g), dim3(64), lds, stream, a,
+    hipLaunchKernelGGL(pick_units_kernel(f32, p.cyc, stats, a.counts != nullptr, a.bytes != nullptr, p.pair), dim3(g), dim3(64), lds, stream, a,
                        quant_table4(a.mrd, a.bytes != nullptr));
 }
 
@@ -747,6 +766,7 @@
 {
     const BlockLaunchPlan p = block_launch_plan(ctx, a, kernel, safe, f32);
     OrderList ol;
+    if (!p.pair) ctx->last_units_plan = nullptr;
     if (p.ordered) {
         int rc = acquire_order_list(ctx, stream, p.grid.x, &ol);
         if (rc != MBK_OK) return rc;
@@ -1526,7 +1546,8 @@
          48u,  256u,  1u,  8u,  1u,
          65537u,  1u,  0u,  1u,  0u,
          32768u,  0u,  8u,  6u,  1024u,
-         1u,  32u,  256u,  16u,  2048u,  19u,  5u};
+         1u,  32u,  256u,  16u,  2048u,  19u,  5u,
+         0u};
     std::memcpy(ctx->opt, kDefaults, sizeof(kDefaults));
 #define MBK_CREATE_HIP(call)                                                        \
     do {                                                                            \
@@ -2161,6 +2182,7 @@
         case MBK_OPT_SPILL_MIN_MRD: ok = true; break;
         case MBK_OPT_SPILL_MIN_BLOCKS: ok = value <= 31u; break;
         case MBK_OPT_SPILL_CYC_SHIFT: ok = value <= 31u; break;
+        case MBK_OPT_H_PAIR: ok = value <= 2u; break;
         default: return fail(ctx, MBK_ERR_INVALID, "unknown MBK_OPT_* selector");
     }
     if (!ok) return fail(ctx, MBK_ERR_INVALID, "option value out of range");
@@ -2196,6 +2218,20 @@
                     MBK_HIP(ctx, hipMemcpy(&t, sc.spill.d_total, sizeof(t), hipMemcpyDeviceToHost));
                     *value = (uint32_t)std::min<unsigned long long>(t, 0xffffffffull);
                 }
+        }
+        return MBK_OK;
+    }
+    if (option == MBK_INFO_H_PAIR || option == MBK_INFO_H_PAIR + 1) {
+        *value = ctx->pair_launches;
+        if (option == MBK_INFO_H_PAIR) {
+            *value = 0u;
+            if (ctx->last_units_plan) {
+                uint32_t w[2] = {0u, 0u};
+                MBK_HIP(ctx, hipSetDevice(ctx->device));
+                MBK_HIP(ctx, hipStreamSynchronize(ctx->last_units_stream));
+                MBK_HIP(ctx, hipMemcpy(w, ctx->last_units_plan + 6, sizeof(w), hipMemcpyDeviceToHost));
+                *value = w[1] - w[0];
+            }
         }
         return MBK_OK;
     }
diff --git a/distributedmandelbrot_amd/csrc/mbk_kernels.h b/distributedmandelbrot_amd/csrc/mbk_kernels.h
--- a/distributedmandelbrot_amd/csrc/mbk_kernels.h
+++ b/distributedmandelbrot_amd/csrc/mbk_kernels.h
@@ -204,6 +204,45 @@
     if (p.bytes) (p.bytes + ubase)[loff] = quantise(count, p);
     if (p.smooth) (p.smooth + ubase)[loff] = smooth_value(count, (double)m);
     return count;
+}
+
+template <typename T, int kGroup>
+__device__ __forceinline__ void block_pair(const TileArgs &p, uint32_t ucol, uint32_t urow, uint32_t lx, uint32_t ly, int32_t &c0, int32_t &c1)
+{
+    const uint32_t lc = ucol + lx, lr = urow + ly;
+    const T cr = (T)((double)(p.col0 + lc) * p.re.step + p.re.start);
+    const T ci0 = (T)((double)(p.row0 + lr) * p.im.step + p.im.start);
+    const T ci1 = (T)((double)(p.row0 + lr + 8u) * p.im.step + p.im.start);
+    T zr = cr, zi = ci0, yr = cr, yi = ci1, m = 0;
+    int32_t cnt0 = 0, cnt1 = 0;
+    const uint32_t total = p.mrd > 1 ? (uint32_t)p.mrd - 1u : 0u;
+    const uint32_t ex = kGroup >= 16 ? p.exact_steps_long : p.exact_steps;
+    const uint32_t first = total < ex ? total : ex;
+    uint32_t n = first;
+    bool whole = true;
+    if (first != 0u) {
+        T a = zr * zr, b = zi * zi;
+        escape_steps_asm<true>(cr, ci0, zr, zi, a, b, m, cnt0, 0u, first);
+        a = yr * yr;
+        b = yi * yi;
+        escape_steps_asm<true>(cr, ci1, yr, yi, a, b, m, cnt1, 0u, first);
+        whole = __ballot((cnt0 | cnt1) != 0) == 0ull;
+    }
+    const uint32_t limit = first + ((total - first) & ~31u);
+    if (whole && limit > first) n = escape_steps_pair(cr, ci0, ci1, zr, zi, yr, yi, first, limit);
+    const size_t ubase = (size_t)(urow + p.out_row0) * p.out_pitch + ucol + p.out_col0;
+    const uint32_t loff = ly * p.out_pitch + lx;
+#pragma nounroll
+    for (uint32_t k = 0; k < 2u; ++k) {
+        const T ci = k ? ci1 : ci0;
+        T wr = k ? yr : zr, wi = k ? yi : zi, a = wr * wr, b = wi * wi;
+        int32_t cnt = k ? cnt1 : cnt0;
+        if (cnt == 0 && total > n) escape_steps_tail<kGroup, false>(cr, ci, wr, wi, a, b, m, cnt, n, total);
+        const size_t base = ubase + (size_t)(8u * k) * p.out_pitch;
+        if (p.counts) (p.counts + base)[loff] = cnt;
+        if (p.bytes) (p.bytes + base)[loff] = quantise(cnt, p);
+        if (k) c1 = cnt; else c0 = cnt;
+    }
 }
 
 template <typename T> struct SpillPair;
diff --git a/distributedmandelbrot_amd/csrc/mbk_loops.inc b/distributedmandelbrot_amd/csrc/mbk_loops.inc
--- a/distributedmandelbrot_amd/csrc/mbk_loops.inc
+++ b/distributedmandelbrot_amd/csrc/mbk_loops.inc
@@ -310,8 +310,6 @@
     "s_mov_b32 %[win], %[win0]\n"
 #define MBK_G_CYC(ZR, ZI, ID)                              \
     "v_cmp_eq_" MBK_CYC_BITS " vcc, " ZR ", %[szr]\n"      \
-    "v_cmp_eq_" MBK_CYC_BITS "_e64 %[tmp2], " ZI ", %[szi]\n" \
-    "s_and_b64 vcc, vcc, %[tmp2]\n"                        \
     "s_cbranch_vccnz .Lcyc" ID "_%=\n"                     \
     ".Lcyccont" ID "_%=:\n"                                \
     "s_add_u32 %[tc], %[tc], 1\n"                          \
@@ -320,6 +318,9 @@
     ".Lcycsaved" ID "_%=:\n"
 #define MBK_G_CYC_OOL(ZR, ZI, ID)                          \
     ".Lcyc" ID "_%=:\n"                                    \
+    "v_cmp_eq_" MBK_CYC_BITS "_e64 %[tmp2], " ZI ", %[szi]\n" \
+    "s_and_b64 vcc, vcc, %[tmp2]\n"                        \
+    "s_cbranch_vccz .Lcyccont" ID "_%=\n"                  \
     "s_and_saveexec_b64 %[tmp], vcc\n"                     \
     "v_mov_b32 %[cnt], -1\n"                               \
     "s_andn2_b64 exec, %[tmp], vcc\n"                      \
@@ -502,6 +503,64 @@
     return kCycle && cnt < 0 ? 0 : cnt;
 }
 
+#define MBK_P_STEP(ZRS, ZIS, ZRD, ZID, YRS, YIS, YRD, YID)    \
+    "v_add_" MBK_F " %[t], %[a], -%[b]\n"                    \
+    "v_add_" MBK_F " %[yt], %[ya], -%[yb]\n"                 \
+    "v_mul_" MBK_F " %[p], " ZRS ", " ZIS "\n"               \
+    "v_mul_" MBK_F " %[yp], " YRS ", " YIS "\n"              \
+    "v_add_" MBK_F " " ZRD ", %[t], %[cr]\n"                 \
+    "v_add_" MBK_F " " YRD ", %[yt], %[cr]\n"                \
+    "v_fma_" MBK_F " " ZID ", %[p], 2.0, %[ci]\n"            \
+    "v_fma_" MBK_F " " YID ", %[yp], 2.0, %[di]\n"           \
+    "v_mul_" MBK_F " %[a], " ZRD ", " ZRD "\n"               \
+    "v_mul_" MBK_F " %[ya], " YRD ", " YRD "\n"              \
+    "v_mul_" MBK_F " %[b], " ZID ", " ZID "\n"               \
+    "v_mul_" MBK_F " %[yb], " YID ", " YID "\n"
+#define MBK_P_0TO1 MBK_P_STEP("%[zr]", "%[zi]", "%[zr2]", "%[zi2]", "%[yr]", "%[yi]", "%[yr2]", "%[yi2]")
+#define MBK_P_1TO0 MBK_P_STEP("%[zr2]", "%[zi2]", "%[zr]", "%[zi]", "%[yr2]", "%[yi2]", "%[yr]", "%[yi]")
+#define MBK_P_0TO0 MBK_P_STEP("%[zr]", "%[zi]", "%[zr]", "%[zi]", "%[yr]", "%[yi]", "%[yr]", "%[yi]")
+#define MBK_P_1TO1 MBK_P_STEP("%[zr2]", "%[zi2]", "%[zr2]", "%[zi2]", "%[yr2]", "%[yi2]", "%[yr2]", "%[yi2]")
+#define MBK_P_GROUP(FIRST, REST, ID)                       \
+    FIRST REST REST REST REST REST REST REST REST REST REST REST REST REST REST REST \
+    "v_add_" MBK_F " %[t], %[a], %[b]\n"                   \
+    "v_add_" MBK_F " %[yt], %[ya], %[yb]\n"                \
+    "v_cmp_ngt_" MBK_F " vcc, 4.0, %[t]\n"                 \
+    "v_cmp_ngt_" MBK_F "_e64 %[tmp2], 4.0, %[yt]\n"        \
+    "s_or_b64 vcc, vcc, %[tmp2]\n"                         \
+    "s_cbranch_vccnz .Lptrip" ID "_%=\n"
+#define MBK_P_LOOP                                         \
+    "s_mov_b32 %[n], %[n0]\n"                              \
+    ".Lpmain_%=:\n"                                        \
+    MBK_P_GROUP(MBK_P_0TO1, MBK_P_1TO1, "1")               \
+    MBK_P_GROUP(MBK_P_1TO0, MBK_P_0TO0, "2")               \
+    "s_add_u32 %[n], %[n], 32\n"                           \
+    "s_cmp_lt_u32 %[n], %[limit]\n"                        \
+    "s_cbranch_scc1 .Lpmain_%=\n"                          \
+    "s_branch .Lptrip1_%=\n"                               \
+    ".Lptrip2_%=:\n"    \
+    "v_mov_" MBK_CYC_MOV " %[zr], %[zr2]\n"                \
+    "v_mov_" MBK_CYC_MOV " %[zi], %[zi2]\n"                \
+    "v_mov_" MBK_CYC_MOV " %[yr], %[yr2]\n"                \
+    "v_mov_" MBK_CYC_MOV " %[yi], %[yi2]\n"                \
+    "s_add_u32 %[n], %[n], 16\n"                           \
+    ".Lptrip1_%=:\n"
+
+__device__ __forceinline__ uint32_t escape_steps_pair(MBK_T cr, MBK_T ci, MBK_T di, MBK_T &zr, MBK_T &zi, MBK_T &yr, MBK_T &yi,
+                                                      uint32_t n0, uint32_t limit)
+{
+    MBK_T a = zr * zr, b = zi * zi, ya = yr * yr, yb = yi * yi;
+    MBK_T zr2, zi2, yr2, yi2, t, p, yt, yp;
+    uint32_t n;
+    unsigned long long tmp2;
+    asm volatile(MBK_P_LOOP
+                 : [zr] "+&v"(zr), [zi] "+&v"(zi), [yr] "+&v"(yr), [yi] "+&v"(yi), [a] "+&v"(a), [b] "+&v"(b), [ya] "+&v"(ya), [yb] "+&v"(yb),
+                   [zr2] "=&v"(zr2), [zi2] "=&v"(zi2), [yr2] "=&v"(yr2), [yi2] "=&v"(yi2), [t] "=&v"(t), [p] "=&v"(p), [yt] "=&v"(yt),
+                   [yp] "=&v"(yp), [n] "=&s"(n), [tmp2] "=&s"(tmp2)
+                 : [cr] "v"(cr), [ci] "v"(ci), [di] "v"(di), [limit] "s"(limit), [n0] "s"(n0)
+                 : "vcc", "scc");
+    return (uint32_t)__builtin_amdgcn_readfirstlane((int)n);
+}
+
 template <bool kFmaDouble>
 __device__ __forceinline__ int32_t escape_count_asm_from(MBK_T z0r, MBK_T z0i, MBK_T cr, MBK_T ci, int32_t mrd, MBK_T *m_out = nullptr)
 {
diff --git a/distributedmandelbrot_amd/csrc/mbk_units.h b/distributedmandelbrot_amd/csrc/mbk_units.h
--- a/distributedmandelbrot_amd/csrc/mbk_units.h
+++ b/distributedmandelbrot_amd/csrc/mbk_units.h
@@ -47,18 +47,26 @@
 
 __global__ __launch_bounds__(1024) void classify_units_kernel(TileArgs p, uint32_t nregions, int32_t probe_steps,
                                                               uint32_t *order, uint32_t *counters, int32_t m_late, double settle_thr,
-                                                              uint32_t *extra, uint32_t *plan, XcdShares shares, uint32_t stamps)
+                                                              uint32_t *extra, uint32_t *plan, XcdShares shares, uint32_t stamps, uint32_t pair)
 {
     __shared__ uint32_t s_last;
     __shared__ uint32_t s_cnt[5][16], s_base[5];
     const uint32_t r = blockIdx.x * blockDim.x + threadIdx.x;
     const uint32_t lane = threadIdx.x & 63u, wave = threadIdx.x >> 6;
-    const bool valid = r < nregions;
+    bool valid = r < nregions;
     uint32_t cls = 5u;
     uint32_t by = 0, bx = 0;
-    if (valid) {
+    bool pairable = false;
+    if (pair) {
+        const uint32_t g = r >> 4, w = r & 15u, gpr = p.blocks_x >> 3, k = g / gpr;
+        by = 2u * k + (w >> 3);
+        bx = 8u * (g - k * gpr) + (w & 7u);
+        valid = by < nregions / p.blocks_x;
+    } else if (valid) {
         by = r / p.blocks_x;
         bx = r - by * p.blocks_x;
+    }
+    if (valid) {
         uint32_t lc = bx * 8u + 4u, lr = by * 8u + 4u;
         lc = lc < p.ncols ? lc : p.ncols - 1u;
         lr = lr < p.nrows ? lr : p.nrows - 1u;
@@ -68,6 +76,12 @@
         const int32_t cnt = cap > 1 ? (settle_thr > 0.0 ? probe_settling(cr, ci, cap, &delta) : escape_count<true>(cr, ci, cap)) : 1;
         const bool regular = bx < p.fast_bx_end && by < p.fast_by_end;
         cls = cnt == 0 ? (delta <= settle_thr ? 4u : 0u) : (cnt <= 3 && regular ? 1u : (m_late > 0 && cnt >= m_late ? 3u : 2u));
+        const double fr = __builtin_fabs(cr) + 4.5 * __builtin_fabs(p.re.step), fi = __builtin_fabs(ci) + 4.5 * __builtin_fabs(p.im.step);
+        pairable = cls == 0u && regular && fr * fr + fi * fi < 4.0 - 2e-3;
+    }
+    if (pair) {
+        const unsigned long long hm = __ballot(pairable);
+        if (((hm >> (lane & ~8u)) & (hm >> (lane | 8u)) & 1ull) != 0ull) cls = (lane & 8u) ? 5u : 4u;
     }
     const unsigned long long vmask = __ballot(cls == 1u);
     const uint32_t seg = (uint32_t)(vmask >> (lane & ~7u)) & 0xffu;
@@ -109,6 +123,7 @@
         const uint32_t n_ml = atomicExch(&extra[0], 0u), n_hs = atomicExch(&extra[1], 0u);
         atomicExch(&extra[2], 0u);
         units_plan(n_h + n_ml + n_hs, n_v, n_m, shares.cum, stamps, plan, n_ml, n_hs);
+        if (pair) plan[7] = plan[6] + n_hs;
     }
 }
 
@@ -195,7 +210,7 @@
         reinterpret_cast<unsigned long long *>(base)[slot] = (wall_clock64() & 0xffffffffffffull) | ((unsigned long long)tag << 48);
 }
 
-template <typename T, int kGroup, bool kCycle, bool kCounts, bool kBytes, bool kStats = false>
+template <typename T, int kGroup, bool kCycle, bool kCounts, bool kBytes, bool kStats = false, bool kPair = false>
 __global__ __launch_bounds__(64) __attribute__((amdgpu_waves_per_eu(8, 8))) void tile_units_kernel(TileArgs args, uint32_t qtab)
 {
     static_assert(!kStats || (!kCounts && kBytes), "fused statistics exist for the bytes-only instantiation");
@@ -228,7 +243,17 @@
         if (!units_lookup(u, hmin, lmin, h_x, l_x, hbase_x, lbase_x, is_h, i)) break;
         if (is_h || i < n_m) {
             const bool late = is_h && i < n_ml;
-            const uint32_t e = scalar_load_u32(p.order, is_h ? (late ? 2u * n + 2u - i : (i < hs0 ? i - n_ml : (uint32_t)units_settled_base(n) + (i - hs0)))
+            if (kPair && is_h && !late && i < hs0) {
+                const uint32_t e = scalar_load_u32(p.order, (uint32_t)units_settled_base(n) + (i - n_ml));
+                const uint32_t by = e >> 16, bx = e & 0xffffu;
+                int32_t c0, c1;
+                block_pair<T, kGroup>(p, bx * 8u, by * 8u, lx, ly, c0, c1);
+                if (kStats) heavy += (c0 > 0 ? (unsigned long long)(uint32_t)c0 : (1ull << 47) + never_cap) +
+                                     (c1 > 0 ? (unsigned long long)(uint32_t)c1 : (1ull << 47) + never_cap);
+                continue;
+            }
+            const uint32_t e = scalar_load_u32(p.order, kPair ? (is_h ? (late ? 2u * n + 2u - i : i - hs0) : n + 3u + i)
+                                                              : is_h ? (late ? 2u * n + 2u - i : (i < hs0 ? i - n_ml : (uint32_t)units_settled_base(n) + (i - hs0)))
                                                               : n + 3u + i);
             const uint32_t by = e >> 16, bx = e & 0xffffu;
             const int32_t c = block_pixel<T, true, kGroup, kCycle>(p, bx * 8u, by * 8u, lx, ly, kGroup >= 16 && is_h && !late,
diff --git a/distributedmandelbrot_amd/device.py b/distributedmandelbrot_amd/device.py
--- a/distributedmandelbrot_amd/device.py
+++ b/distributedmandelbrot_amd/device.py
@@ -506,6 +506,12 @@
         self._check(self._lib.mbk_get_option(self._h, L.MBK_INFO_SPILL + 1, C.byref(b)))
         return {"lanes_last_launch": int(a.value), "launches": int(b.value)}
 
+    def h_pair_info(self) -> dict:
+        a, b = C.c_uint32(0), C.c_uint32(0)
+        self._check(self._lib.mbk_get_option(self._h, L.MBK_INFO_H_PAIR, C.byref(a)))
+        self._check(self._lib.mbk_get_option(self._h, L.MBK_INFO_H_PAIR + 1, C.byref(b)))
+        return {"pairs_last_launch": int(a.value), "launches": int(b.value)}
+
     def quantise_counts(self, counts: np.ndarray, mrd: int) -> np.ndarray:
         counts = np.ascontiguousarray(counts, dtype=np.int32)
         out = np.empty(counts.shape, np.uint8)
diff --git a/include/mbk.h b/include/mbk.h
--- a/include/mbk.h
+++ b/include/mbk.h
@@ -407,11 +407,13 @@
     MBK_OPT_SPILL_MIN_MRD,
     MBK_OPT_SPILL_MIN_BLOCKS,
     MBK_OPT_SPILL_CYC_SHIFT,
+    MBK_OPT_H_PAIR,
     MBK_OPT_COUNT_
 };
 #define MBK_INFO_SCAN_WG_PER_CU 100
 #define MBK_INFO_XCD_SHARE 110
 #define MBK_INFO_SPILL 130
+#define MBK_INFO_H_PAIR 140
 int mbk_set_option(mbk_ctx *ctx, int option, uint32_t value);
 int mbk_get_option(mbk_ctx *ctx, int option, uint32_t *value);
 
```

Measured after the change: 5298 (median of 5 runs). Within noise of the previous version (+0.0%).
